# fzi-forschungszentrum-informatik/muvo

Measured on AMD Instinct MI355X. Metric: world-model training samples/sec (seq_len=10), higher is better.
Workload: dtype f32 storage/accumulate; large contractions (convolutions, transformer Linear) as bf16x3 split products

## Files before the change

### include/muvo_hip.h

```cpp
#ifndef MUVO_HIP_H
#define MUVO_HIP_H
#include <stdint.h>

#ifdef __cplusplus
extern "C" {
#endif

#define MUVO_OK 0
#define MUVO_ERR_INVALID_ARG (-1)
#define MUVO_ERR_HIP (-2)

#define MUVO_ACT_NONE 0
#define MUVO_ACT_RELU 1
#define MUVO_ACT_LEAKY 2
#define MUVO_ACT_ELU 3
#define MUVO_ACT_TANH 4
#define MUVO_ACT_SIGMOID 5

const char* muvo_last_error(void);
int muvo_abi_version(void);
int muvo_selftest_mfma(void* stream);
int muvo_set_deterministic(int on);
int muvo_reset_accumulators(void);
int muvo_get_deterministic(void);

typedef struct muvo_conv_desc {
  int32_t nd;
  int32_t transposed;
  int32_t N, Cin, Cout;
  int32_t in_sz[3], out_sz[3];
  int32_t ksz[3], stride[3], pad[3], dil[3];
} muvo_conv_desc;

#define MUVO_CONV_F32 0
#define MUVO_CONV_BF16X3 1
#define MUVO_CONV_MODE_DEFAULT MUVO_CONV_BF16X3
int muvo_conv_set_products(int n);
int muvo_conv_get_products(void);
int muvo_conv_set_mode(int mode);
int muvo_conv_get_mode(void);
int muvo_conv_set_bf16x3_min_gflop(double gflop_per_item);
int muvo_linear_bf16x3_pack_floats(int in_f, int out_f, int64_t* fwd_floats, int64_t* dgrad_floats);
int muvo_linear_bf16x3_pack(int in_f, int out_f, const float* w, float* wp_fwd, float* wp_dgrad, void* stream);
int64_t muvo_linear_bf16x3_workspace_bytes(int64_t rows, int features);
int muvo_linear_bf16x3_split(const float* x, int64_t rows, int features, void* ws, void* stream);
int muvo_linear_bf16x3_forward(int64_t rows, int in_f, int out_f, const void* ws_x, const float* wp_fwd, const float* bias,
                               float* y, int act, float slope, void* stream);
int muvo_linear_bf16x3_dgrad(int64_t rows, int in_f, int out_f, const void* ws_dz, const float* wp_dgrad, float* dx,
                             void* stream);
int muvo_linear_bf16x3_wgrad(int64_t rows, int in_f, int out_f, const void* ws_x, const void* ws_dz, float* scratch,
                             float* dw, void* stream);
int64_t muvo_pack_table_item_bytes(void);
int muvo_conv_pack_table_add(void* host_items, int capacity, int* n_items, int64_t* n_blocks, const muvo_conv_desc* d,
                             const float* w, float* wp_fwd, float* wp_dgrad);
int muvo_linear_bf16x3_pack_table_add(void* host_items, int capacity, int* n_items, int64_t* n_blocks, int in_f, int out_f,
                                      const float* w, float* wp_fwd, float* wp_dgrad);
int muvo_pack_table_run(const void* dev_items, int n_items, int64_t n_blocks, void* stream);
int muvo_conv_pack_sizes(const muvo_conv_desc* d, int64_t* fwd_floats, int64_t* dgrad_floats);
int muvo_conv_pack_weights(const muvo_conv_desc* d, const float* w, float* wp_fwd, float* wp_dgrad, void* stream);
int64_t muvo_conv_workspace_bytes(const muvo_conv_desc* d, int op);
int muvo_conv_kernel_family(const muvo_conv_desc* d, int op);
int muvo_conv_kernel_variant(const muvo_conv_desc* d, int op);
int muvo_conv_forward(const muvo_conv_desc* d, const float* x, const float* wp_fwd, const float* bias, float* y, int act,
                      float slope, void* ws, void* stream);
int muvo_conv_dgrad(const muvo_conv_desc* d, const float* dy, const float* wp_dgrad, float* dx, void* ws, int ws_valid,
                    void* stream);
int muvo_conv_forward_head_supported(const muvo_conv_desc* d, int CO);
int muvo_conv_forward_head(const muvo_conv_desc* d, const float* x, const float* wp_fwd, const float* bias, float* y, int act,
                           float slope, void* ws, const float* head_w, const float* head_b, int CO, float* logits, void* stream);
int muvo_conv_forward_moments_supported(const muvo_conv_desc* d);
int muvo_conv_forward_moments(const muvo_conv_desc* d, const float* x, const float* wp_fwd, const float* bias, float* y, int act,
                              float slope, double* moments, void* stream);
int muvo_adain_fwd_moments(const float* x, const float* style, float* y, float* save_mean, float* save_rstd, double* moments,
                           int N, int C, int64_t S, float eps, void* stream);
int muvo_adain_affine(const float* style, double* moments, float* save_mean, float* save_rstd, float* aff, int N, int C, int64_t S,
                      float eps, void* stream);
int muvo_conv_affine_supported(const muvo_conv_desc* d);
int muvo_conv_forward_affine(const muvo_conv_desc* d, const float* x, const float* aff, const float* wp_fwd, const float* bias,
                             float* y, int act, float slope, double* moments, void* stream);
int muvo_conv_wgrad_affine(const muvo_conv_desc* d, const float* x, const float* aff, const float* dy, float* dw, float* dbias,
                           void* stream);
int muvo_grouped_linear_fwd(const float* x, int M, int K, int L, const float* const* W, const float* const* b, float* const* Y,
                            const int* N, void* stream);
int muvo_grouped_linear_bwd(const float* x, int M, int K, int L, const float* const* W, float* const* dY, float* dx,
                            float* const* dW, float* const* db, const int* N, void* stream);
int muvo_bf3_loop_clock(double* shader_mhz, double* us_per_k_step);
int muvo_adain_head_supported(int C, int CO, int64_t S);
int muvo_adain_head_fwd(const float* x, const float* style, float* save_mean, float* save_rstd, double* moments, const float* head_w,
                        const float* head_b, float* logits, int N, int C, int CO, int64_t S, float eps, void* stream);
int muvo_adain_head_bwd(const float* x, const float* style, const float* save_mean, const float* save_rstd, const float* head_w,
                        const float* dlogits, float* dx, float* dstyle, float* dhead_w, float* dhead_b, double* ws, int N, int C,
                        int CO, int64_t S, int act, float slope, void* stream);
int muvo_conv_dgrad_accumulate(const muvo_conv_desc* d, const float* dy, const float* wp_dgrad, float* dx, void* stream);
int muvo_conv_prepare_dy(const muvo_conv_desc* d, const float* y, const float* dy, int act, float slope, void* ws_dy,
                         float* dbias, void* stream);
int muvo_conv_prepare_dy_head_supported(const muvo_conv_desc* d, int CO);
int muvo_conv_prepare_dy_head(const muvo_conv_desc* d, const float* y, const float* dy, const float* dhead, const float* head_w,
                              int CO, int act, float slope, void* ws_dy, float* dbias, float* dhead_w, float* dhead_b, void* stream);
int64_t muvo_split_planes_bytes(int N, int C, int64_t S);
int muvo_split_planes(const float* x, void* ws, int N, int C, int64_t S, const float* y, int act, float slope, float* dbias,
                      void* stream);
int muvo_conv_wgrad(const muvo_conv_desc* d, const float* x, const float* dy, float* dwp_scratch, float* dw, float* dbias,
                    void* ws_x, void* ws_dy, int flags, void* stream);

int muvo_bias_grad_nchw(const float* dy, float* db, int N, int M, int64_t S, void* stream);

typedef struct muvo_gemm_desc {
  int32_t M, N, K;
  int64_t sam, sak, sbk, sbn, scm;
  int32_t B1, B2;
  int64_t a_b1, a_b2, b_b1, b_b2, c_b1, c_b2;
  float alpha;
  int32_t bias_div;
  int32_t act;
  float slope;
  int32_t mode;
} muvo_gemm_desc;
int muvo_gemm(const muvo_gemm_desc* d, const float* A, const float* B, float* C, const float* bias, void* stream);

int muvo_bn_train_fwd(const float* x, const float* gamma, const float* beta, const float* residual, float* y,
                      float* save_mean, float* save_rstd, float* running_mean, float* running_var, double* ws, int N, int C,
                      int64_t S, float eps, float momentum, int res_mode, int relu, void* stream);
int muvo_bn_train_bwd(const float* x, const float* y, const float* dy, const float* gamma, const float* beta,
                      const float* save_mean, const float* save_rstd, float* dx, float* dres, float* dgamma, float* dbeta,
                      double* ws, int N, int C, int64_t S, int mask_mode, void* stream);
int muvo_adain_fwd(const float* x, const float* style, float* y, float* save_mean, float* save_rstd, double* ws, int N,
                   int C, int64_t S, int64_t x_batch_stride, float eps, void* stream);
int muvo_adain_bwd(const float* x, const float* style, const float* dy, const float* save_mean, const float* save_rstd,
                   float* dx, float* dstyle, double* ws, int N, int C, int64_t S, int64_t x_batch_stride, int act,
                   float slope, void* stream);
int muvo_add_dropout_layernorm_fwd(const float* x, const float* a, const float* gamma, const float* beta, float* y,
                                   float* z, float* mean, float* rstd, int rows, int E, float eps, float p, uint64_t seed,
                                   void* stream);
int muvo_add_dropout_layernorm_bwd(const float* dy, const float* z, const float* mean, const float* rstd,
                                   const float* gamma, float* dx, float* da, float* dgamma, float* dbeta, int rows, int E,
                                   float p, uint64_t seed, void* stream);

int muvo_act_fwd(const float* x, float* y, int64_t n, int act, float slope, void* stream);
int muvo_act_bwd(const float* y, const float* dy, float* dx, int64_t n, int act, float slope, void* stream);
int muvo_dropout(const float* x, float* y, int64_t n, float p, uint64_t seed, void* stream);
int muvo_axpby(const float* a, const float* b, float* out, int64_t n, float alpha, float beta, void* stream);
int muvo_copy2d(const float* src, float* dst, int64_t rows, int64_t cols, int64_t ld_src, int64_t ld_dst, int accumulate,
                void* stream);
int muvo_colsum_acc(const float* x, float* out, int64_t rows, int64_t cols, int64_t ld, void* stream);
int muvo_batchsum(const float* x, float* out, int N, int64_t inner, int accumulate, void* stream);
int muvo_nchw_to_tokens(const float* x, const float* pos, const float* temb, int temb_stride, float* tokens, int N, int C,
                        int L, int l0, void* stream);
int muvo_tokens_to_nchw(const float* tokens, float* x, int N, int C, int L, int l0, void* stream);
int muvo_maxpool2d_fwd(const float* x, float* y, uint8_t* idx, int64_t NC, int H, int W, int OH, int OW, int k, int s, int p,
                       void* stream);
int muvo_maxpool2d_bwd(const float* dy, const uint8_t* idx, float* dx, int64_t NC, int H, int W, int OH, int OW, int k, int s,
                       int p, void* stream);
int muvo_avgpool_fwd(const float* x, float* y, int64_t G, int64_t S, void* stream);
int muvo_avgpool_bwd(const float* dy, float* dx, int64_t G, int64_t S, void* stream);
int muvo_upsample3d_x2_fwd(const float* x, float* y, int64_t NC, int D, int H, int W, void* stream);
int muvo_upsample3d_x2_bwd(const float* dy, float* dx, int64_t NC, int D, int H, int W, void* stream);
int muvo_preprocess_image(const uint8_t* img, float* label, float* norm, int64_t NC, int C, int H, int W, int top, int left,
                          int CH, int CW, const float* mean3, const float* std3, void* stream);
int muvo_preprocess_route(const uint8_t* img, float* norm, int64_t NC, int C, int H, int W, int OH, int OW,
                          const float* mean3, const float* std3, void* stream);
int muvo_attention_supported(int L, int DH);
int muvo_attention_fwd(const float* qkv, float* out, float* lse, int L, int N, int H, int DH, float p, uint64_t seed,
                       void* stream);
int muvo_attention_bwd(const float* qkv, const float* out, const float* dout, const float* lse, float* dqkv, int L, int N, int H,
                       int DH, float p, uint64_t seed, void* stream);
int muvo_attention_stream_supported(int L, int DH);
int muvo_attention_stream_blocks(int* bq, int* bk);
int muvo_attention_stream_fwd(const float* qkv, float* out, float* lse, int L, int N, int H, int DH, float p, uint64_t seed,
                              void* stream);
int muvo_attention_stream_bwd(const float* qkv, const float* out, const float* dout, const float* lse, float* dqkv, float* dws,
                              int L, int N, int H, int DH, float p, uint64_t seed, void* stream);
int muvo_rssm_supported(int B, int T, int H, int S, int E, int A, int AD);
int64_t muvo_rssm_transposed_floats(int H, int S, int E, int A);
int64_t muvo_rssm_scratch_floats(int B, int H, int S, int E, int A);
int muvo_rssm_forward(int B, int T, int H, int S, int E, int A, int AD, const float* const* weights, const float* emb,
                      const float* act, const float* noise, uint64_t use_prior_mask, float* const* out7, float* const* keep12,
                      uint32_t* barrier_word, float min_std, void* stream);
int muvo_rssm_backward(int B, int T, int H, int S, int E, int A, int AD, const float* const* weights, float* wt_scratch,
                       const float* noise, uint64_t use_prior_mask, const float* const* kept5, const float* const* upstream7,
                       float* const* grads10, float* scratch, uint32_t* barrier_word, void* stream);
#define MUVO_PIXAUG_STRIDE 16
#define MUVO_ROUTEAUG_STRIDE 8
int muvo_pixel_augment(float* img, float* norm, float* tmp, const float* params, double* gray_sum, int64_t frames, int H, int W,
                       const float* mean3, const float* std3, void* stream);
int muvo_preprocess_route_aug(const uint8_t* img, float* out, const float* params, int B, int S, int C, int H, int W, int OH,
                              int OW, const float* mean3, const float* std3, void* stream);
int muvo_divide_scalar(const float* x, float* y, int64_t n, float divisor, void* stream);
int muvo_resize_bilinear(const float* x, float* y, int64_t NC, int H, int W, int OH, int OW, void* stream);
int muvo_resize_nearest_f32(const float* x, float* y, int64_t NC, int D, int H, int W, int OD, int OH, int OW, void* stream);
int muvo_resize_nearest_u8(const uint8_t* x, uint8_t* y, int64_t NC, int D, int H, int W, int OD, int OH, int OW,
                           void* stream);
int muvo_softmax_dropout_fwd(const float* S, float* P, float* Pd, int64_t rows, int cols, float p, uint64_t seed, void* stream);
int muvo_softmax_dropout_bwd(const float* P, const float* dPd, float* dS, int64_t rows, int cols, float p, uint64_t seed,
                             void* stream);
int muvo_gru_fwd(const float* gi, const float* gh, const float* h, float* hnew, int B, int H, void* stream);
int muvo_gru_bwd(const float* gi, const float* gh, const float* h, const float* dhnew, float* dgi, float* dgh, float* dh,
                 int B, int H, void* stream);
int muvo_rssm_sample_fwd(const float* mu_logsigma, const float* eps, int64_t eps_ld, float* mu, float* sigma, float* sample,
                         int B, int S, float min_std, void* stream);
int muvo_rssm_sample_bwd(const float* mu_logsigma, const float* eps, int64_t eps_ld, const float* dmu, const float* dsigma,
                         const float* dsample, float* dmls, int B, int S, void* stream);

int muvo_spatial_loss_fwd(const float* pred, const float* target, int64_t F, int Ct, int64_t HW, int c0, int c1, int norm,
                          float ignore, float weight, double* stats2, float* loss, void* stream);
int muvo_spatial_loss_bwd(const float* pred, const float* target, float* dpred, int64_t F, int Ct, int64_t HW, int c0, int c1,
                          int norm, float ignore, float weight, const double* stats2, const float* gout, void* stream);
int muvo_spatial_loss_masked_fwd(const float* pred, const float* target, const uint8_t* mask, int64_t F, int Ct, int64_t HW, int c0,
                                 int c1, int norm, float ignore, float weight, double* stats2, float* loss, void* stream);
int muvo_spatial_loss_masked_bwd(const float* pred, const float* target, const uint8_t* mask, float* dpred, int64_t F, int Ct,
                                 int64_t HW, int c0, int c1, int norm, float ignore, float weight, const double* stats2,
                                 const float* gout, void* stream);
int muvo_voxel_loss_stats_doubles(int C);
int muvo_voxel_loss_coef_floats(int C);
int muvo_voxel_loss_fwd(const float* logits, const uint8_t* target, int64_t F, int C, int64_t V, const float* class_w,
                        float weight, double* stats, float* coef, float* loss3, void* stream);
int muvo_voxel_loss_bwd(const float* logits, const uint8_t* target, float* dlogits, int64_t F, int C, int64_t V,
                        const float* class_w, float weight, const float* coef, const float* gout3, void* stream);
int muvo_seg_ce_fwd(const float* logits, const uint8_t* target, const float* class_w, float* loss, int64_t N, int C, int64_t HW,
                    void* stream);
int muvo_seg_ce_bwd(const float* logits, const uint8_t* target, const float* class_w, const float* gloss, float* dlogits, int64_t N,
                    int C, int64_t HW, void* stream);
int muvo_l1_rows_fwd(const float* p, const float* t, int64_t rows, int cols, float weight, float* loss, void* stream);
int muvo_l1_rows_bwd(const float* p, const float* t, float* dp, int64_t rows, int cols, float weight, const float* gout,
                     void* stream);
int muvo_kl_loss_fwd(const float* prior_mu, const float* prior_sigma, const float* post_mu, const float* post_sigma, int B,
                     int T, int S, float weight, float* loss, void* stream);
int muvo_kl_loss_bwd(const float* prior_mu, const float* prior_sigma, const float* post_mu, const float* post_sigma,
                     float* d_prior_mu, float* d_prior_sigma, float* d_post_mu, float* d_post_sigma, int B, int T, int S,
                     float weight, float alpha, const float* gout, void* stream);
int muvo_adamw_step(float* p, const float* g, float* m, float* v, int64_t n, float lr, float beta1, float beta2, float eps,
                    float weight_decay, int step, float grad_scale, void* stream);

int64_t muvo_chamfer_loss_ws_doubles(int64_t F, int64_t n);
int muvo_chamfer_loss_fwd(const float* pred, const float* target, int64_t F, int Cp, int Ct, int64_t n, float weight, double* ws,
                          int32_t* idx_pt, int32_t* idx_tp, float* loss, void* stream);
int muvo_chamfer_loss_bwd(const float* pred, const float* target, const int32_t* idx_pt, const int32_t* idx_tp, float* dpred, int64_t F,
                          int Cp, int Ct, int64_t n, float weight, const float* gout, void* stream);

int muvo_ssim_frames(const float* pred, const float* target, const float* window, double* sums, int N, int C, int H, int W,
                     float c1, float c2, void* stream);
int muvo_ssim_maps(const float* pred, const float* target, const float* window, double* sums, float* dA, float* dB, float* dC, int N,
                   int C, int H, int W, float c1, float c2, void* stream);
int muvo_ssim_bwd(const float* pred, const float* target, const float* window, const float* dA, const float* dB, const float* dC,
                  float* dpred, int N, int C, int H, int W, float scale, void* stream);
int muvo_sqdiff_frames(const float* pred, const float* target, double* sums, int N, int64_t L, void* stream);
int muvo_chamfer_sums(const float* a, const float* b, double* sums, int N, int P, int Q, void* stream);
// ... 120 lines not shown
```

### muvo_amd/csrc/conv_gemm.hip

```cpp
#include "common.h"
#include "conv_vox.h"
#include "conv_pw.h"
#include "conv_plan.h"
#include "conv_bf3.h"

typedef __bf16 wg_bf16x8 __attribute__((ext_vector_type(8)));
__device__ __forceinline__ void wg_split8(const float (&v)[8], wg_bf16x8& hi, wg_bf16x8& lo) {
  typedef __bf16 b2 __attribute__((ext_vector_type(2)));
  typedef float f2 __attribute__((ext_vector_type(2)));
  unsigned h[4], l[4];
#pragma unroll
  for (int p = 0; p < 4; ++p) {
    const b2 hh = __builtin_convertvector((f2){v[2 * p], v[2 * p + 1]}, b2);
    h[p] = __builtin_bit_cast(unsigned, hh);
    const float h0 = __uint_as_float(h[p] << 16), h1 = __uint_as_float(h[p] & 0xffff0000u);
    const b2 ll = __builtin_convertvector((f2){v[2 * p] - h0, v[2 * p + 1] - h1}, b2);
    l[p] = __builtin_bit_cast(unsigned, ll);
  }
  typedef unsigned u4 __attribute__((ext_vector_type(4)));
  hi = __builtin_bit_cast(wg_bf16x8, (u4){h[0], h[1], h[2], h[3]});
  lo = __builtin_bit_cast(wg_bf16x8, (u4){l[0], l[1], l[2], l[3]});
}

template <int BM, int BN, int WM, int WN, int RUN>
// ... 835 lines not shown
    }
    return pl.nfwd > 0 && bf3_wgrad_uses_pp(pl.fwd[0]) ? 1 : 0;
  }
  if (build_plan(d, &pl)) return 0;
  const ConvPhase* ph = op == 0 ? pl.fwd : pl.dgr;
  const int nph = op == 0 ? pl.nfwd : pl.ndgr;
  return nph > 0 && bf3_fwd_uses_pp(ph[0]) ? 1 : 0;
}

static int run_phases(const ConvPhase* ph, int nph, const float* in, const float* wp, const float* bias, float* out, int act,
                      float slope, void* ws, hipStream_t st, bool ws_valid = false) {
  bool split_done = ws_valid;
  static const int any_rule = getenv("MUVO_KSPLIT_ANY") ? atoi(getenv("MUVO_KSPLIT_ANY")) : 1;
  bool use_ksplit = nph > 0 && !any_rule, any_ks = false;
  for (int i = 0; i < nph; ++i) {
    use_ksplit = use_ksplit && phase_ksplit(ph[i]) > 1;
    any_ks = any_ks || phase_ksplit(ph[i]) > 1;
  }
  if (any_rule) use_ksplit = any_ks;
  const long out_total = nph > 0 ? (long)ph[0].N * ph[0].out_sN : 0;
  if (use_ksplit && hipMemsetAsync(out, 0, sizeof(float) * out_total, st) != hipSuccess) {
    muvo_set_error("conv: memset of the split-K output failed");
    return MUVO_ERR_HIP;
  }
  for (int i = 0; i < nph; ++i) {
    if (ph[i].bf3 && !split_done) {
      MUVO_CHECK_ARG(ws != nullptr, "conv: this shape runs on the bf16x3 kernel and needs muvo_conv_workspace_bytes() of workspace");
      int rc = bf3_split_input(in, ws, ph[i].N, ph[i].C, (long)ph[i].ID * ph[i].IH * ph[i].IW, st);
      if (rc) return rc;
      split_done = true;
    }
    const int ks_i = phase_ksplit(ph[i]);
    int rc = launch_fwd_phase(ph[i], in, wp, bias, out, act, slope, st, ws, use_ksplit ? (ks_i > 1 ? ks_i : 2) : 1);
    if (rc) return rc;
  }
  if (use_ksplit && (bias != nullptr || act != MUVO_ACT_NONE)) {
    hipLaunchKernelGGL(bias_act_kernel, dim3(ew_grid(out_total)), dim3(256), 0, st, out, bias, ph[0].Msub, (long)ph[0].out_sC,
                       out_total, act, slope);
    MUVO_CHECK_LAUNCH("bias_act_kernel");
  }
  return MUVO_OK;
}

int muvo_conv_forward(const muvo_conv_desc* d, const float* x, const float* wp_fwd, const float* bias, float* y,
                      int act, float slope, void* ws, void* stream) {
  ConvPlan pl;
  int rc = build_plan(d, &pl);
  if (rc) return rc;
  MUVO_CHECK_ARG(x && wp_fwd && y, "conv_forward: null pointer");
  if (pw_applicable(d)) return pw_forward(d, x, wp_fwd, bias, y, act, slope, (hipStream_t)stream);
  if (vox_fwd_ok(d)) return vox_forward(d, x, wp_fwd, bias, y, act, slope, (hipStream_t)stream, vox_uses_bf3(d, 0));
  return run_phases(pl.fwd, pl.nfwd, x, wp_fwd, bias, y, act, slope, ws, (hipStream_t)stream);
}

int muvo_conv_forward_planes(const muvo_conv_desc* d, const float* x, const float* wp_fwd, const float* bias, float* y, int act,
                             float slope, void* ws, int ws_valid, void* stream) {
  if (!ws_valid) return muvo_conv_forward(d, x, wp_fwd, bias, y, act, slope, ws, stream);
  ConvPlan pl;
  int rc = build_plan(d, &pl);
  if (rc) return rc;
  MUVO_CHECK_ARG(wp_fwd && y && ws, "conv_forward_planes: null pointer");
  MUVO_CHECK_ARG(!pw_applicable(d) && !vox_fwd_ok(d), "conv_forward_planes: this shape does not read split planes");
  bool all_bf3 = pl.nfwd > 0;
  for (int i = 0; i < pl.nfwd; ++i) all_bf3 = all_bf3 && pl.fwd[i].bf3;
  MUVO_CHECK_ARG(all_bf3, "conv_forward_planes: ws_valid needs every phase on the bf16x3 kernels (muvo_conv_kernel_family == 1)");
  return run_phases(pl.fwd, pl.nfwd, x, wp_fwd, bias, y, act, slope, ws, (hipStream_t)stream, true);
}

int muvo_conv_forward_head_supported(const muvo_conv_desc* d, int CO) {
  if (check_desc(d) || CO < 1 || CO > 4) return 0;
  static const int on = getenv("MUVO_CONV_HEAD_FWD") ? atoi(getenv("MUVO_CONV_HEAD_FWD")) : 1;
  if (!on || muvo_det() || conv_mode() != 1 || pw_applicable(d) || vox_fwd_ok(d)) return 0;
  ConvPlan pl;
  if (build_plan(d, &pl) != MUVO_OK || pl.nfwd < 1) return 0;
  for (int i = 0; i < pl.nfwd; ++i) {
    const ConvPhase& g = pl.fwd[i];
    if (!g.bf3 || !bf3_fwd_uses_pp(g) || phase_ksplit(g) > 1) return 0;
    if (g.Msub != d->Cout || g.Msub % 64 != 0 || g.M % 64 != 0 || (long)CO * g.Msub > 1024) return 0;
    if ((long)g.N * g.out_sN * 4 >= 0x7fffff00L) return 0;
  }
  return 1;
}
int muvo_conv_forward_head(const muvo_conv_desc* d, const float* x, const float* wp_fwd, const float* bias, float* y, int act,
                           float slope, void* ws, const float* head_w, const float* head_b, int CO, float* logits, void* stream) {
  ConvPlan pl;
  int rc = build_plan(d, &pl);
  if (rc) return rc;
  MUVO_CHECK_ARG(x && wp_fwd && y && head_w && logits, "conv_forward_head: null pointer");
  MUVO_CHECK_ARG(muvo_conv_forward_head_supported(d, CO), "conv_forward_head: shape not served by the eight-wave bf16x3 tiles");
  hipStream_t st = (hipStream_t)stream;
  if (d->Cout > 64) {
    const long S_out = (long)d->out_sz[0] * d->out_sz[1] * d->out_sz[2];
    if (hipMemsetAsync(logits, 0, sizeof(float) * (size_t)d->N * CO * S_out, st) != hipSuccess) {
      muvo_set_error("conv_forward_head: memset of the logits failed");
      return MUVO_ERR_HIP;
    }
  }
  bf3_set_fused_head(head_w, head_b, logits, CO);
  rc = run_phases(pl.fwd, pl.nfwd, x, wp_fwd, bias, y, act, slope, ws, st);
  bf3_set_fused_head(nullptr, nullptr, nullptr, 0);
  return rc;
}

int muvo_conv_forward_moments_supported(const muvo_conv_desc* d) {
  if (check_desc(d)) return 0;
  if (muvo_det()) return 0;
  return (!pw_applicable(d) && vox_fwd_ok(d) && vox_uses_bf3(d, 0)) ? 1 : 0;
}
int muvo_conv_forward_moments(const muvo_conv_desc* d, const float* x, const float* wp_fwd, const float* bias, float* y, int act,
                              float slope, double* moments, void* stream) {
  ConvPlan pl;
  int rc = build_plan(d, &pl);
  if (rc) return rc;
  MUVO_CHECK_ARG(x && wp_fwd && y && moments, "conv_forward_moments: null pointer");
  MUVO_CHECK_ARG(muvo_conv_forward_moments_supported(d), "conv_forward_moments: only the bf16x3 voxel kernels produce output moments");
  return vox_forward(d, x, wp_fwd, bias, y, act, slope, (hipStream_t)stream, true, moments);
}

int muvo_conv_affine_supported(const muvo_conv_desc* d) {
  if (check_desc(d)) return 0;
  return (conv_mode() == 1 && !pw_applicable(d) && vox_fwd_ok(d) && vox_uses_bf3(d, 0) && vox_wgrad_applicable(d) &&
          vox_wgrad_uses_bf3(d) && vox_affine_ok(d)) ? 1 : 0;
}
int muvo_conv_forward_affine(const muvo_conv_desc* d, const float* x, const float* aff, const float* wp_fwd, const float* bias,
                             float* y, int act, float slope, double* moments, void* stream) {
  ConvPlan pl;
  int rc = build_plan(d, &pl);
  if (rc) return rc;
  MUVO_CHECK_ARG(x && aff && wp_fwd && y, "conv_forward_affine: null pointer");
  MUVO_CHECK_ARG(muvo_conv_affine_supported(d), "conv_forward_affine: shape not served by the bf16x3 voxel kernels");
  return vox_forward(d, x, wp_fwd, bias, y, act, slope, (hipStream_t)stream, true, moments, aff);
}
int muvo_conv_wgrad_affine(const muvo_conv_desc* d, const float* x, const float* aff, const float* dy, float* dw, float* dbias,
                           void* stream) {
  ConvPlan pl;
  int rc = build_plan(d, &pl, 0, false);
  if (rc) return rc;
  MUVO_CHECK_ARG(x && aff && dy && dw, "conv_wgrad_affine: null pointer");
  MUVO_CHECK_ARG(muvo_conv_affine_supported(d), "conv_wgrad_affine: shape not served by the bf16x3 voxel kernels");
  return vox_wgrad(d, x, dy, dw, dbias, (hipStream_t)stream, true, aff);
}

int muvo_conv_dgrad(const muvo_conv_desc* d, const float* dy, const float* wp_dgrad, float* dx, void* ws, int ws_valid,
                    void* stream) {
  ConvPlan pl;
  int rc = build_plan(d, &pl);
  if (rc) return rc;
  MUVO_CHECK_ARG(dy && wp_dgrad && dx, "conv_dgrad: null pointer");
  if (pw_applicable(d)) return pw_dgrad(d, dy, wp_dgrad, dx, (hipStream_t)stream);
  if (vox_dgrad_ok(d)) return vox_dgrad(d, dy, wp_dgrad, dx, (hipStream_t)stream, vox_uses_bf3(d, 1));
  return run_phases(pl.dgr, pl.ndgr, dy, wp_dgrad, nullptr, dx, MUVO_ACT_NONE, 0.f, ws, (hipStream_t)stream, ws_valid != 0);
}

int muvo_conv_dgrad_accumulate(const muvo_conv_desc* d, const float* dy, const float* wp_dgrad, float* dx, void* stream) {
  int rc = check_desc(d);
  if (rc) return rc;
  MUVO_CHECK_ARG(dy && wp_dgrad && dx, "conv_dgrad_accumulate: null pointer");
  MUVO_CHECK_ARG(pw_applicable(d), "conv_dgrad_accumulate: only the 1x1 head kernels (muvo_conv_kernel_family == 3) accumulate");
  return pw_dgrad_acc(d, dy, wp_dgrad, dx, (hipStream_t)stream);
}

int muvo_conv_prepare_dy(const muvo_conv_desc* d, const float* y, const float* dy, int act, float slope, void* ws_dy,
                         float* dbias, void* stream) {
  int rc = check_desc(d);
  if (rc) return rc;
  MUVO_CHECK_ARG(dy && ws_dy && (y || act == MUVO_ACT_NONE), "conv_prepare_dy: null pointer");
  const long S_out = (long)d->out_sz[0] * d->out_sz[1] * d->out_sz[2];
  return bf3_split_input(dy, ws_dy, d->N, d->Cout, S_out, (hipStream_t)stream, act == MUVO_ACT_NONE ? nullptr : y, act, slope,
                         dbias);
}

int muvo_conv_prepare_dy_head(const muvo_conv_desc* d, const float* y, const float* dy, const float* dhead, const float* head_w,
                              int CO, int act, float slope, void* ws_dy, float* dbias, float* dhead_w, float* dhead_b, void* stream) {
  int rc = check_desc(d);
  if (rc) return rc;
  MUVO_CHECK_ARG(dhead && head_w && ws_dy && CO >= 1 && CO <= 4 && (y || act == MUVO_ACT_NONE), "conv_prepare_dy_head: bad args");
  const long S_out = (long)d->out_sz[0] * d->out_sz[1] * d->out_sz[2];
  MUVO_CHECK_ARG(dhead_w == nullptr || (y != nullptr && act != MUVO_ACT_NONE),
                 "conv_prepare_dy_head: the fused head weight gradient needs the activation output y");
  return bf3_split_input(dy, ws_dy, d->N, d->Cout, S_out, (hipStream_t)stream, act == MUVO_ACT_NONE ? nullptr : y, act, slope,
                         dbias, dhead, head_w, CO, dhead_w, dhead_b);
}
int muvo_conv_prepare_dy_head_supported(const muvo_conv_desc* d, int CO) {
  if (check_desc(d)) return 0;
  const long S_out = (long)d->out_sz[0] * d->out_sz[1] * d->out_sz[2];
  return CO >= 1 && CO <= 4 && S_out % 4 == 0 && S_out >= 1024;
}

static double bf3_wgrad_min_gflop() {
  static const char* e = getenv("MUVO_BF16X3_WGRAD_MIN_GFLOP");
  static const double env_v = e ? atof(e) : -1.0;
  if (env_v >= 0.0) return env_v;
  if (bf3_default_policy()) return 0.05;
  return bf3_min_gflop() < 0.5 ? bf3_min_gflop() : 0.5;
}

static const int g_bf3_wgrad_min_m = getenv("MUVO_BF3_WGRAD_MIN_M") ? atoi(getenv("MUVO_BF3_WGRAD_MIN_M")) : 32;
static bool wgrad_uses_bf3(const ConvPlan& pf) {
  if (conv_mode() != 1) return false;
  const bool dflt = bf3_default_policy() && !getenv("MUVO_BF16X3_WGRAD_MIN_GFLOP");
  double total = 0.0;
  int taps = 0;
  for (int i = 0; i < pf.nfwd; ++i) {
    const ConvPhase& g = pf.fwd[i];
    const double gflop = 2.0 * g.Msub * g.T * g.C * (double)g.SD * g.SH * g.SW * 1e-9;
    if (g.Msub < g_bf3_wgrad_min_m || g.C < 32 || g.Msub % 16 != 0 && g.nmerge > 1) return false;
    static const int allow32 = getenv("MUVO_BF3_WGRAD_32X32") ? atoi(getenv("MUVO_BF3_WGRAD_32X32")) : 1;
    if (g.Msub <= 32 && g.C < 64 && !allow32) return false;
    if (!dflt && gflop < bf3_wgrad_min_gflop()) return false;
    total += gflop * g.nmerge;
    taps += g.T * g.nmerge;
  }
  if (dflt && (total < bf3_wgrad_min_gflop() || taps <= 1)) return false;
  return pf.nfwd > 0;
}

int muvo_conv_wgrad(const muvo_conv_desc* d, const float* x, const float* dy, float* dwp_scratch, float* dw, float* dbias,
                    void* ws_x, void* ws_dy, int flags, void* stream) {
  ConvPlan pl;
  int rc = build_plan(d, &pl, 0, false);
  if (rc) return rc;
  MUVO_CHECK_ARG(x && dy && dwp_scratch && dw, "conv_wgrad: null pointer");
  hipStream_t st = (hipStream_t)stream;
  if (pw_applicable(d)) return pw_wgrad(d, x, dy, dw, dbias, st);
  if (vox_wgrad_ok(d)) return vox_wgrad(d, x, dy, dw, dbias, st, vox_wgrad_uses_bf3(d));
  const long S_out = (long)d->out_sz[0] * d->out_sz[1] * d->out_sz[2];
  if (wgrad_uses_bf3(pl)) {
    ConvPlan pm;
    if (build_plan(d, &pm, 0, true) == MUVO_OK && wgrad_uses_bf3(pm)) pl = pm;
    MUVO_CHECK_ARG(ws_x && ws_dy, "conv_wgrad: this shape runs on the bf16x3 kernel and needs both workspaces");
    const long S_in = (long)d->in_sz[0] * d->in_sz[1] * d->in_sz[2];
    if (!(flags & 1)) { rc = bf3_split_input(x, ws_x, d->N, d->Cin, S_in, st); if (rc) return rc; }
    if (!(flags & 2)) { rc = bf3_split_input(dy, ws_dy, d->N, d->Cout, S_out, st); if (rc) return rc; }
    long off = 0;
    for (int i = 0; i < pl.nfwd; ++i) off += (long)pl.fwd[i].T * pl.fwd[i].M * pl.fwd[i].C;
    off = 0;
    for (int i = 0; i < pl.nfwd; ++i) {
      ConvPhase g = pl.fwd[i];
      g.wp_off = off;
      off += (long)g.T * g.M * g.C;
      rc = bf3_wgrad_phase(g, ws_x, d->Cin, ws_dy, d->Cout, dwp_scratch, dw, st);
      if (rc) return rc;
    }
  } else {
    for (int i = 0; i < pl.nfwd; ++i) {
      rc = launch_wgrad_phase(pl.fwd[i], x, dy, dwp_scratch, st);
      if (rc) return rc;
    }
    for (int i = 0; i < pl.nfwd; ++i) {
      const long total = (long)pl.fwd[i].M * pl.fwd[i].C * pl.fwd[i].T;
      if (total == 0) continue;
      hipLaunchKernelGGL(unpack_wgrad_kernel, dim3(ew_grid(total)), dim3(256), 0, st, pl.fwd[i], dwp_scratch, dw);
    }
    MUVO_CHECK_LAUNCH("unpack_wgrad_kernel");
  }
  if (dbias) {
    int chunks = cdiv((long)d->N * S_out, 65536);
    if (chunks > 64) chunks = 64;
    if (muvo_det()) chunks = 1;
    hipLaunchKernelGGL(bias_grad_kernel, dim3(d->Cout, chunks), dim3(256), 0, st, dy, dbias, d->N, d->Cout, S_out);
    MUVO_CHECK_LAUNCH("bias_grad_kernel");
  }
  return MUVO_OK;
}

int64_t muvo_split_planes_bytes(int N, int C, int64_t S) { return bf3_workspace_bytes(N, C, (long)S); }
int muvo_split_planes(const float* x, void* ws, int N, int C, int64_t S, const float* y, int act, float slope, float* dbias,
                      void* stream) {
  MUVO_CHECK_ARG(x && ws && N > 0 && C > 0 && S > 0, "split_planes: bad args");
  return bf3_split_input(x, ws, N, C, (long)S, (hipStream_t)stream, act == MUVO_ACT_NONE ? nullptr : y, act, slope, dbias);
}
int muvo_bias_grad_nchw(const float* dy, float* db, int N, int M, int64_t S, void* stream) {
  MUVO_CHECK_ARG(dy && db && N > 0 && M > 0 && S > 0, "bias_grad_nchw: bad args");
  int chunks = cdiv((long)N * S, 65536);
  if (chunks > 64) chunks = 64;
  if (muvo_det()) chunks = 1;
  hipLaunchKernelGGL(bias_grad_kernel, dim3(M, chunks), dim3(256), 0, (hipStream_t)stream, dy, db, N, M, (long)S);
  MUVO_CHECK_LAUNCH("bias_grad_kernel");
  return MUVO_OK;
}

static int linear_phase(int rows, int c, int m, long wsm, long wsc, bool token_major_out, ConvPhase* ph) {
  MUVO_CHECK_ARG(rows > 0 && c >= 32 && m > 32 && c % 8 == 0 && m % 4 == 0,
                 "linear_bf16x3: needs in/out features >= 32, reduction features %% 8 == 0, produced features %% 4 == 0");
  muvo_conv_desc d;
  memset(&d, 0, sizeof(d));
  d.nd = 2; d.N = 1; d.Cin = c; d.Cout = m;
  for (int a = 0; a < 3; ++a) { d.in_sz[a] = d.out_sz[a] = d.ksz[a] = d.stride[a] = d.dil[a] = 1; d.pad[a] = 0; }
  d.in_sz[2] = d.out_sz[2] = rows;
  t_plan_mode = 1;
  t_allow_merge = false;
  t_force_family = 1;
  const int rc = build_conv_form(&d, d.in_sz, d.out_sz, c, m, wsm, wsc, ph);
  t_force_family = 0;
  if (rc) return rc;
  ph->wp_off = 0;
  if (token_major_out) { ph->os[2] = m; ph->out_sC = 1; }
  return MUVO_OK;
}

int muvo_linear_bf16x3_pack_floats(int in_f, int out_f, int64_t* fwd_floats, int64_t* dgrad_floats) {
  ConvPhase f, b;
  int rc = linear_phase(1, in_f, out_f, in_f, 1, true, &f);
  if (rc) return rc;
  rc = linear_phase(1, out_f, in_f, 1, in_f, true, &b);
  if (rc) return rc;
// ... 121 lines not shown
```

### muvo_amd/csrc/conv_vox.h

```cpp
#pragma once
#include "common.h"

bool vox_fwd_applicable(const muvo_conv_desc* d);
bool vox_dgrad_applicable(const muvo_conv_desc* d);
bool vox_wgrad_applicable(const muvo_conv_desc* d);
long vox_pack_floats(const muvo_conv_desc* d);
bool vox_bf3_shape_ok(const muvo_conv_desc* d, int dgrad);
int vox_pack(const muvo_conv_desc* d, const float* w, float* wp, int dgrad, hipStream_t st, bool bf3);
int vox_forward(const muvo_conv_desc* d, const float* x, const float* wp, const float* bias, float* y, int act, float slope,
                hipStream_t st, bool bf3, double* moments = nullptr, const float* aff = nullptr);
bool vox_affine_ok(const muvo_conv_desc* d);
int vox_dgrad(const muvo_conv_desc* d, const float* dy, const float* wp, float* dx, hipStream_t st, bool bf3);
bool vox_bf3_wgrad_shape_ok(const muvo_conv_desc* d);
bool vox_wgrad_ps_only(const muvo_conv_desc* d);
int vox_wgrad(const muvo_conv_desc* d, const float* x, const float* dz, float* dw, float* dbias, hipStream_t st, bool bf3,
              const float* aff = nullptr);
```

### muvo_amd/csrc/conv_vox.hip

```cpp
#include "common.h"
#include "conv_vox.h"
#include <type_traits>

struct VoxArgs {
  int N, Cin, Cout, X, Y;
  int ytiles, xgroups;
  int XYZ;
  long sN_in, sN_out;
  double* moments;
  int xcd_order;
  const float* aff;
  unsigned* ticket;
};
static int vox_xcd_order() {
  static const int v = getenv("MUVO_VOX_XCD") ? atoi(getenv("MUVO_VOX_XCD")) : 1;
  return v;
}

__device__ __forceinline__ float dpp_wave_shr1(float v) {
  return __int_as_float(__builtin_amdgcn_update_dpp(0, __float_as_int(v), 0x138, 0xf, 0xf, true));
}
__device__ __forceinline__ float dpp_wave_shl1(float v) {
  return __int_as_float(__builtin_amdgcn_update_dpp(0, __float_as_int(v), 0x130, 0xf, 0xf, true));
}
// ... 170 lines not shown
    }
  };
  auto fetch_dz = [&](int xx) {
#pragma unroll
    for (int k = 0; k < NDZ; ++k) {
      const int item = tid + k * NT;
      const int i = item & 3, zz = (item >> 2) % Z, r = (item >> 2) / Z;
      const int y = y0 + r;
      const bool ok = xx < xb && r < TYB && y < a.Y;
      const int off = xx * YZ + y * Z + zz;
#pragma unroll
      for (int e = 0; e < CQB; ++e) pdz[k][e] = ok ? dzn[(size_t)(4 * e + i) * a.XYZ + off] : 0.f;
    }
  };
  auto store_dz = [&](int buf) {
    float* S = D + buf * DBUF;
#pragma unroll
    for (int k = 0; k < NDZ; ++k) {
      const int item = tid + k * NT;
      const int i = item & 3, zz = (item >> 2) % Z, r = (item >> 2) / Z;
      if (r < TYB) {
#pragma unroll
        for (int e = 0; e < CQB; ++e) S[e * DPL + (r * Z + zz) * 4 + i] = pdz[k][e];
      }
    }
  };
  auto slot_of = [](int xx) { return (xx + 3) % 3; };

  f32x4 acc[CQR][9];
#pragma unroll
  for (int q = 0; q < CQR; ++q)
#pragma unroll
    for (int t = 0; t < 9; ++t) acc[q][t] = (f32x4){0.f, 0.f, 0.f, 0.f};
  float db[CQR];
#pragma unroll
  for (int q = 0; q < CQR; ++q) db[q] = 0.f;

  fetch_in(xa - 1); store_in(slot_of(xa - 1));
  fetch_in(xa);     store_in(slot_of(xa));
  fetch_in(xa + 1); store_in(slot_of(xa + 1));
  fetch_dz(xa);     store_dz(xa & 1);
  __syncthreads();

  const int b = lane >> 2, lj = lane & 3;
  const bool bias_role = tx == 1 && rr == 0;
  for (int x = xa; x < xb; ++x) {
    const bool more = x + 1 < xb;
    if (more) { fetch_in(x + 2); fetch_dz(x + 1); }
    const float* S = P + slot_of(x + tx - 1) * SLOT + rr * PLANE;
    const float* Dz = D + (x & 1) * DBUF + (qg * CQR) * DPL;
#pragma unroll 1
    for (int row = 0; row < TYB; ++row) {
#pragma unroll
      for (int zs = 0; zs < ZS; ++zs) {
        const int zz = zs * 16 + b;
        float av[CQR];
#pragma unroll
        for (int q = 0; q < CQR; ++q) av[q] = Dz[q * DPL + (row * Z + zz) * 4 + lj];
        float bv[9];
#pragma unroll
        for (int ty = 0; ty < 3; ++ty)
#pragma unroll
          for (int tz = 0; tz < 3; ++tz) bv[ty * 3 + tz] = S[((row + ty) * ZP + zz + tz) * 4 + lj];
#pragma unroll
        for (int t = 0; t < 9; ++t)
#pragma unroll
          for (int q = 0; q < CQR; ++q) acc[q][t] = __builtin_amdgcn_mfma_f32_4x4x1f32(av[q], bv[t], acc[q][t], 0, 0, 0);
        if (bias_role) {
#pragma unroll
          for (int q = 0; q < CQR; ++q) db[q] += av[q];
        }
      }
    }
    __syncthreads();
    if (more) { store_in(slot_of(x + 2)); store_dz((x + 1) & 1); }
    __syncthreads();
  }

  det_turn_wait(a.ticket);
#pragma unroll
  for (int q = 0; q < CQR; ++q)
#pragma unroll
    for (int t = 0; t < 9; ++t)
#pragma unroll
      for (int i = 0; i < 4; ++i) {
        float v = acc[q][t][i];
        v += __shfl_xor(v, 4, 64);
        v += __shfl_xor(v, 8, 64);
        v += __shfl_xor(v, 16, 64);
        v += __shfl_xor(v, 32, 64);
        if (lane < 4) {
          const int co = (qc * CQB + qg * CQR + q) * 4 + i, ci = (rc * RQB + rr) * 4 + lane;
          atomicAdd(dw + ((size_t)co * a.Cin + ci) * 27 + tx * 9 + t, v);
        }
      }
  if (bias_role && rc == 0 && dbias != nullptr) {
#pragma unroll
    for (int q = 0; q < CQR; ++q) {
      float v = db[q];
      v += __shfl_xor(v, 4, 64);
      v += __shfl_xor(v, 8, 64);
      v += __shfl_xor(v, 16, 64);
      v += __shfl_xor(v, 32, 64);
      if (lane < 4) atomicAdd(dbias + (qc * CQB + qg * CQR + q) * 4 + lane, v);
    }
  }
  det_turn_done(a.ticket);
}

__global__ void __launch_bounds__(256) vox_pack_kernel(const float* __restrict__ w, float* __restrict__ wp, int Cin, int Cout,
                                                       int dgrad) {
  const int total = 27 * Cin * Cout;
  for (int idx = blockIdx.x * 256 + threadIdx.x; idx < total; idx += gridDim.x * 256) {
    const int ci_k = dgrad ? Cout : Cin;
    const int co_k = dgrad ? Cin : Cout;
    const int cq = co_k / 4;
    const int q = idx % cq;
    int r = idx / cq;
    const int i = r & 3; r >>= 2;
    const int ck = r % ci_k, tap = r / ci_k;
    const int cp = 4 * q + i;
    float v;
    if (!dgrad) v = w[((size_t)cp * Cin + ck) * 27 + tap];
    else v = w[((size_t)ck * Cin + cp) * 27 + (26 - tap)];
    wp[idx] = v;
  }
}

typedef __bf16 vbf16x8 __attribute__((ext_vector_type(8)));
typedef float vf32x4 __attribute__((ext_vector_type(4)));
typedef unsigned vu32x4 __attribute__((ext_vector_type(4)));

__device__ __forceinline__ float vox_act_simple(float v, int act, float slope) {
  const float neg = act == MUVO_ACT_RELU ? 0.f : v * slope;
  return (act == MUVO_ACT_NONE || v > 0.f) ? v : neg;
}

template <int N>
__device__ __forceinline__ void vox_dummy_stores(__amdgpu_buffer_rsrc_t rs) {
#pragma unroll
  for (int k = 0; k < N; ++k) __builtin_amdgcn_raw_buffer_store_b32(0u, rs, 0x7fffff00u + 32u * k, 0, 0);
}

__device__ __forceinline__ void vox_split2(float a, float b, unsigned& hi, unsigned& lo) {
  typedef __bf16 vbf16x2 __attribute__((ext_vector_type(2)));
  typedef float vf32x2 __attribute__((ext_vector_type(2)));
  const vbf16x2 h = __builtin_convertvector((vf32x2){a, b}, vbf16x2);
  hi = __builtin_bit_cast(unsigned, h);
  const float h0 = __uint_as_float(hi << 16), h1 = __uint_as_float(hi & 0xffff0000u);
  const vbf16x2 l = __builtin_convertvector((vf32x2){a - h0, b - h1}, vbf16x2);
  lo = __builtin_bit_cast(unsigned, l);
}

template <int CK, int Z, int TY, bool GENERIC>
__global__ void __launch_bounds__(64 * TY)
vox_bf3_kernel(const VoxArgs a, const float* __restrict__ in, const vu32x4* __restrict__ wp, const float* __restrict__ bias,
               float* __restrict__ out, int act, float slope, int xseg, int accum) {
  static_assert(CK == 8 && TY == 8, "8 reduction channels (one channel group), 8 rows per workgroup");
  constexpr int CG = 1, TPS = 4, NSTEP = (27 + TPS - 1) / TPS, ZT = Z / 16;
  constexpr int ROWS = TY + 2, COLS = Z + 2;
  constexpr int PLANE = 2 * CG * ROWS * COLS;
  constexpr int NTASK = CG * ROWS * Z, TPT = (NTASK + 64 * TY - 1) / (64 * TY);
  extern __shared__ vu32x4 vsm[];
  const int tid = threadIdx.x, lane = tid & 63, wave = tid >> 6;
  const int nseg = (a.X + xseg - 1) / xseg;
  int bid = a.xcd_order ? xcd_swizzle(blockIdx.x, gridDim.x) : (int)blockIdx.x;
  const int seg = bid % nseg; bid /= nseg;
  const int ytile = bid % a.ytiles, n = bid / a.ytiles;
  const int y0 = ytile * TY, xs = seg * xseg, xe = xs + xseg < a.X ? xs + xseg : a.X;
  const long YZ = (long)a.Y * Z;
  const float* inb = in + (long)n * a.sN_in;
  const int co0 = blockIdx.y * 16;

  vbf16x8 wh[NSTEP], wl[NSTEP];
  const vu32x4* wpb = wp + (size_t)blockIdx.y * NSTEP * 2 * 64;
#pragma unroll
  for (int s = 0; s < NSTEP; ++s) {
    wh[s] = __builtin_bit_cast(vbf16x8, wpb[(s * 2) * 64 + lane]);
    wl[s] = __builtin_bit_cast(vbf16x8, wpb[(s * 2 + 1) * 64 + lane]);
  }
  for (int i = tid; i < 3 * PLANE; i += 64 * TY) vsm[i] = vu32x4{0u, 0u, 0u, 0u};
  __syncthreads();

  float stg[TPT][8];
  unsigned stg_ok = 0u;
  float afs[8], afb[8];
  if (a.aff) {
#pragma unroll
    for (int e = 0; e < 8; ++e) {
      afs[e] = a.aff[((long)n * a.Cin + e) * 2];
      afb[e] = a.aff[((long)n * a.Cin + e) * 2 + 1];
    }
  }
  const __amdgpu_buffer_rsrc_t rs_in = __builtin_amdgcn_make_buffer_rsrc((void*)inb, 0, (int)((long)CK * a.XYZ * 4), 0x00020000);
  const unsigned xyz4 = (unsigned)a.XYZ * 4u;
  auto stage_load = [&](int x) {
#pragma unroll
    for (int k = 0; k < TPT; ++k) {
      const int t = tid + k * 64 * TY;
      const int z = t % Z, r = (t / Z) % ROWS, cg = t / (Z * ROWS);
      const int gy = y0 - 1 + r;
      const bool ok = t < NTASK && x >= 0 && x < a.X && gy >= 0 && gy < a.Y;
      stg_ok = k == 0 ? (unsigned)ok : stg_ok | ((unsigned)ok << k);
      const unsigned off = ok ? (unsigned)(((long)(cg * 8) * a.XYZ + (long)x * YZ + (long)gy * Z + z) * 4) : 0x7fffff00u;
#pragma unroll
      for (int e = 0; e < 8; ++e)
        stg[k][e] = __uint_as_float(__builtin_amdgcn_raw_buffer_load_b32(rs_in, off + (unsigned)e * xyz4, 0, 0));
    }
  };
  auto stage_store = [&](int slot) {
    vu32x4* P = vsm + slot * PLANE;
#pragma unroll
    for (int k = 0; k < TPT; ++k) {
      const int t = tid + k * 64 * TY;
      if (t >= NTASK) continue;
      const int z = t % Z, r = (t / Z) % ROWS, cg = t / (Z * ROWS);
      if (a.aff) {
        const bool ok = (stg_ok >> k) & 1u;
#pragma unroll
        for (int e = 0; e < 8; ++e) stg[k][e] = ok ? stg[k][e] * afs[e] + afb[e] : 0.f;
      }
      unsigned h[4], l[4];
#pragma unroll
      for (int q = 0; q < 4; ++q) vox_split2(stg[k][2 * q], stg[k][2 * q + 1], h[q], l[q]);
      P[(cg * ROWS + r) * COLS + z + 1] = vu32x4{h[0], h[1], h[2], h[3]};
      P[((CG + cg) * ROWS + r) * COLS + z + 1] = vu32x4{l[0], l[1], l[2], l[3]};
    }
  };

  const int v = lane & 15, g = lane >> 4;
  float msum[4] = {0.f, 0.f, 0.f, 0.f}, msq[4] = {0.f, 0.f, 0.f, 0.f};
  float bv[4];
#pragma unroll
  for (int i = 0; i < 4; ++i) bv[i] = (bias != nullptr && co0 + 4 * g + i < a.Cout) ? bias[co0 + 4 * g + i] : 0.f;
  const __amdgpu_buffer_rsrc_t rs_out = __builtin_amdgcn_make_buffer_rsrc((void*)(out + (long)n * a.sN_out), 0,
                                                                          (int)((long)a.Cout * a.XYZ * 4), 0x00020000);

  int fdx[NSTEP], foff[NSTEP];
#pragma unroll
  for (int s = 0; s < NSTEP; ++s) {
    int tap = s * TPS + g;
    if (tap > 26) tap = 26;
    const int dx = tap / 9 - 1, dy = (tap / 3) % 3 - 1, dz = tap % 3 - 1;
    fdx[s] = dx;
    foff[s] = (wave + 1 + dy) * COLS + (v + 1 + dz);
  }

  stage_load(xs - 1); stage_store((xs - 1 + 3) % 3);
  stage_load(xs); stage_store(xs % 3);
  stage_load(xs + 1);
  vox_dummy_stores<4 * ZT>(rs_out);
  __syncthreads();
  for (int x = xs; x < xe; ++x) {
    stage_store((x + 1) % 3);
    __syncthreads();
    if (x + 1 < xe) stage_load(x + 2);
    const vu32x4* P[3] = {vsm + ((x - 1 + 3) % 3) * PLANE, vsm + (x % 3) * PLANE, vsm + ((x + 1) % 3) * PLANE};
    const vu32x4* fb[NSTEP];
#pragma unroll
    for (int s = 0; s < NSTEP; ++s) fb[s] = (fdx[s] < 0 ? P[0] : (fdx[s] == 0 ? P[1] : P[2])) + foff[s];
    const int gy = y0 + wave;
#pragma unroll
    for (int zt = 0; zt < ZT; ++zt) {
      vf32x4 acc = {0.f, 0.f, 0.f, 0.f};
#pragma unroll
      for (int s = 0; s < NSTEP; ++s) {
        const vbf16x8 bh = __builtin_bit_cast(vbf16x8, fb[s][zt * 16]);
        const vbf16x8 bl = __builtin_bit_cast(vbf16x8, fb[s][zt * 16 + CG * ROWS * COLS]);
        acc = __builtin_amdgcn_mfma_f32_16x16x32_bf16(wl[s], bh, acc, 0, 0, 0);
        acc = __builtin_amdgcn_mfma_f32_16x16x32_bf16(wh[s], bl, acc, 0, 0, 0);
        acc = __builtin_amdgcn_mfma_f32_16x16x32_bf16(wh[s], bh, acc, 0, 0, 0);
      }
      const unsigned ooff = (unsigned)(((long)x * YZ + (long)gy * Z + zt * 16 + v) * 4);
#pragma unroll
      for (int i = 0; i < 4; ++i) {
        const int co = co0 + 4 * g + i;
        const bool ok = gy < a.Y && co < a.Cout;
        const unsigned off = ok ? ooff + (unsigned)co * xyz4 : 0x7fffff00u;
        float r = acc[i] + bv[i];
        if constexpr (GENERIC) {
          if (accum) r += __uint_as_float(__builtin_amdgcn_raw_buffer_load_b32(rs_out, off, 0, 0));
          r = act_apply(r, act, slope);
        } else {
          r = vox_act_simple(r, act, slope);
        }
        __builtin_amdgcn_raw_buffer_store_b32(__float_as_uint(r), rs_out, off, 0, 0);
        r = ok ? r : 0.f;
        msum[i] += r;
        msq[i] += r * r;
      }
    }
    __syncthreads();
  }
  if (a.moments) {
#pragma unroll
    for (int i = 0; i < 4; ++i)
#pragma unroll
      for (int o = 1; o < 16; o <<= 1) { msum[i] += __shfl_xor(msum[i], o, 64); msq[i] += __shfl_xor(msq[i], o, 64); }
    float* red = (float*)vsm;
    if (v == 0)
#pragma unroll
      for (int i = 0; i < 4; ++i) { red[((wave * 4 + g) * 4 + i) * 2] = msum[i]; red[((wave * 4 + g) * 4 + i) * 2 + 1] = msq[i]; }
    __syncthreads();
    if (tid < 32) {
      const int c = tid >> 1, k = tid & 1;
      double t = 0.0;
      for (int w = 0; w < TY; ++w) t += (double)red[((w * 4 + (c >> 2)) * 4 + (c & 3)) * 2 + k];
      if (co0 + c < a.Cout) atomicAdd(&a.moments[((long)n * a.Cout + co0 + c) * 2 + k], t);
    }
  }
}

constexpr int VOX_PS_TY = 8;
template <int Z, int TY, bool CO8, bool GENERIC>
__global__ void __launch_bounds__(64 * TY, 1)
vox_bf3_ps_kernel(const VoxArgs a, const float* __restrict__ in, const vu32x4* __restrict__ wp, const float* __restrict__ bias,
                  float* __restrict__ out, int act, float slope, int xseg, int accum) {
  static_assert(TY == VOX_PS_TY, "one workgroup of eight waves per CU");
  constexpr int CK = 16, CG = 2, PSTEPS = 5, ZT = Z / 16, NF = CO8 ? 2 * PSTEPS : 3 * PSTEPS, NACC = CO8 ? 2 : 3;
  constexpr int ROWS = TY + 2, COLS = Z + 2;
  constexpr int PLANE = 2 * CG * ROWS * COLS;
  constexpr int NTASK = CG * ROWS * Z, TPT = (NTASK + 64 * TY - 1) / (64 * TY);
  extern __shared__ vu32x4 vsm[];
  const int tid = threadIdx.x, lane = tid & 63, wave = tid >> 6;
  const int nseg = (a.X + xseg - 1) / xseg;
  int bid = a.xcd_order ? xcd_swizzle(blockIdx.x, gridDim.x) : (int)blockIdx.x;
  const int seg = bid % nseg; bid /= nseg;
  const int ytile = bid % a.ytiles, n = bid / a.ytiles;
  const int y0 = ytile * TY, xs = seg * xseg, xe = xs + xseg < a.X ? xs + xseg : a.X;
  const long YZ = (long)a.Y * Z;
  const float* inb = in + (long)n * a.sN_in;
  const int co0 = blockIdx.y * 16;

  vbf16x8 wh[NF], wl[NF];
  const vu32x4* wpb = wp + (size_t)blockIdx.y * NF * 2 * 64;
#pragma unroll
  for (int f = 0; f < NF; ++f) {
    wh[f] = __builtin_bit_cast(vbf16x8, wpb[(f * 2) * 64 + lane]);
    wl[f] = __builtin_bit_cast(vbf16x8, wpb[(f * 2 + 1) * 64 + lane]);
  }
  for (int i = tid; i < 2 * PLANE; i += 64 * TY) vsm[i] = vu32x4{0u, 0u, 0u, 0u};
  __syncthreads();

  float stg[TPT][8];
  unsigned stg_ok = 0u;
  __shared__ float s_aff[2 * CK];
  if (a.aff) {
    if (tid < 2 * CK) s_aff[tid] = a.aff[(long)n * a.Cin * 2 + tid];
    __syncthreads();
  }
  const __amdgpu_buffer_rsrc_t rs_in = __builtin_amdgcn_make_buffer_rsrc((void*)inb, 0, (int)((long)CK * a.XYZ * 4), 0x00020000);
  const unsigned xyz4 = (unsigned)a.XYZ * 4u;
  auto stage_load_task = [&](int k, int x) {
    const int t = tid + k * 64 * TY;
    const int z = t % Z, r = (t / Z) % ROWS, cg = t / (Z * ROWS);
    const int gy = y0 - 1 + r;
    const bool ok = t < NTASK && x >= 0 && x < a.X && gy >= 0 && gy < a.Y;
    stg_ok = (stg_ok & ~(1u << k)) | ((unsigned)ok << k);
    const unsigned off = ok ? (unsigned)(((long)(cg * 8) * a.XYZ + (long)x * YZ + (long)gy * Z + z) * 4) : 0x7fffff00u;
#pragma unroll
    for (int e = 0; e < 8; ++e)
      stg[k][e] = __uint_as_float(__builtin_amdgcn_raw_buffer_load_b32(rs_in, off + (unsigned)e * xyz4, 0, 0));
  };
  auto stage_load = [&](int x) {
#pragma unroll
    for (int k = 0; k < TPT; ++k) stage_load_task(k, x);
  };
  auto stage_store_task = [&](int k, int slot) {
    vu32x4* P = vsm + slot * PLANE;
    {
      const int t = tid + k * 64 * TY;
      if (t >= NTASK) return;
      const int z = t % Z, r = (t / Z) % ROWS, cg = t / (Z * ROWS);
      if (a.aff) {
        const bool ok = (stg_ok >> k) & 1u;
#pragma unroll
        for (int e = 0; e < 8; ++e) {
          const float sc = s_aff[(cg * 8 + e) * 2], sh = s_aff[(cg * 8 + e) * 2 + 1];
          stg[k][e] = ok ? stg[k][e] * sc + sh : 0.f;
        }
      }
      unsigned h[4], l[4];
#pragma unroll
      for (int q = 0; q < 4; ++q) vox_split2(stg[k][2 * q], stg[k][2 * q + 1], h[q], l[q]);
      P[(cg * ROWS + r) * COLS + z + 1] = vu32x4{h[0], h[1], h[2], h[3]};
      P[((CG + cg) * ROWS + r) * COLS + z + 1] = vu32x4{l[0], l[1], l[2], l[3]};
    }
  };
  auto stage_store = [&](int slot) {
#pragma unroll
    for (int k = 0; k < TPT; ++k) stage_store_task(k, slot);
  };

  const int v = lane & 15, g = lane >> 4;
  float msum[4] = {0.f, 0.f, 0.f, 0.f}, msq[4] = {0.f, 0.f, 0.f, 0.f};
  float bv[4];
#pragma unroll
  for (int i = 0; i < 4; ++i) bv[i] = (bias != nullptr && co0 + 4 * g + i < a.Cout) ? bias[co0 + 4 * g + i] : 0.f;
  const __amdgpu_buffer_rsrc_t rs_out = __builtin_amdgcn_make_buffer_rsrc((void*)(out + (long)n * a.sN_out), 0,
                                                                          (int)((long)a.Cout * a.XYZ * 4), 0x00020000);
  int foff[PSTEPS];
#pragma unroll
  for (int s = 0; s < PSTEPS; ++s) {
    int tp = s * 2 + (g >> 1);
    if (tp > 8) tp = 8;
    const int dy = tp / 3 - 1, dz = tp % 3 - 1;
    foff[s] = ((g & 1) * ROWS + (wave + 1 + dy)) * COLS + (v + 1 + dz);
  }
  vf32x4 acc[NACC][ZT];
#pragma unroll
  for (int j = 0; j < NACC; ++j)
#pragma unroll
    for (int zt = 0; zt < ZT; ++zt) acc[j][zt] = vf32x4{0.f, 0.f, 0.f, 0.f};

  stage_load(xs - 1); stage_store((xs - 1) & 1);
  stage_load(xs);
  vox_dummy_stores<4 * ZT>(rs_out);
  __syncthreads();
  const int gy = y0 + wave;
  for (int p = xs - 1; p <= xe; ++p) {
    constexpr bool ACC_PRE = GENERIC && (CO8 || Z <= 32);
    float accv[ZT][4];
    if constexpr (ACC_PRE) {
      if (accum) {
        const int xo = p - 1;
        const bool xok = xo >= xs && xo < xe;
#pragma unroll
        for (int zt = 0; zt < ZT; ++zt) {
          const unsigned ooff = (unsigned)(((long)xo * YZ + (long)gy * Z + zt * 16 + v) * 4);
#pragma unroll
          for (int i = 0; i < 4; ++i) {
            const int co = co0 + 4 * g + i;
            const bool ok = xok && gy < a.Y && co < a.Cout && (!CO8 || g < 2);
            accv[zt][i] = __uint_as_float(__builtin_amdgcn_raw_buffer_load_b32(rs_out, ok ? ooff + (unsigned)co * xyz4 : 0x7fffff00u, 0, 0));
          }
        }
      }
    }
    constexpr bool PIPE = CO8 || Z <= 32;
    if constexpr (!PIPE) {
      stage_store((p + 1) & 1);
      if (p + 2 <= xe) stage_load(p + 2);
    }
    const vu32x4* P = vsm + (p & 1) * PLANE;
#pragma unroll
    for (int zt = 0; zt < ZT; ++zt) {
#pragma unroll
      for (int s = 0; s < PSTEPS; ++s) {
        const vbf16x8 bh = __builtin_bit_cast(vbf16x8, P[foff[s] + zt * 16]);
        const vbf16x8 bl = __builtin_bit_cast(vbf16x8, P[foff[s] + zt * 16 + CG * ROWS * COLS]);
        if constexpr (CO8) {
          acc[1][zt] = __builtin_amdgcn_mfma_f32_16x16x32_bf16(wl[s], bh, acc[1][zt], 0, 0, 0);
          acc[1][zt] = __builtin_amdgcn_mfma_f32_16x16x32_bf16(wh[s], bl, acc[1][zt], 0, 0, 0);
          acc[1][zt] = __builtin_amdgcn_mfma_f32_16x16x32_bf16(wh[s], bh, acc[1][zt], 0, 0, 0);
          acc[0][zt] = __builtin_amdgcn_mfma_f32_16x16x32_bf16(wl[PSTEPS + s], bh, acc[0][zt], 0, 0, 0);
          acc[0][zt] = __builtin_amdgcn_mfma_f32_16x16x32_bf16(wh[PSTEPS + s], bl, acc[0][zt], 0, 0, 0);
          acc[0][zt] = __builtin_amdgcn_mfma_f32_16x16x32_bf16(wh[PSTEPS + s], bh, acc[0][zt], 0, 0, 0);
        } else {
#pragma unroll
          for (int dxi = 0; dxi < 3; ++dxi) {
            const int f = dxi * PSTEPS + s, j = 2 - dxi;
            acc[j][zt] = __builtin_amdgcn_mfma_f32_16x16x32_bf16(wl[f], bh, acc[j][zt], 0, 0, 0);
            acc[j][zt] = __builtin_amdgcn_mfma_f32_16x16x32_bf16(wh[f], bl, acc[j][zt], 0, 0, 0);
            acc[j][zt] = __builtin_amdgcn_mfma_f32_16x16x32_bf16(wh[f], bh, acc[j][zt], 0, 0, 0);
          }
        }
      }
      if constexpr (PIPE) {
#pragma unroll
        for (int k = 0; k < TPT; ++k)
          if ((k < ZT ? k : ZT - 1) == zt) {
            stage_store_task(k, (p + 1) & 1);
            if (p + 2 <= xe) stage_load_task(k, p + 2);
          }
        __builtin_amdgcn_sched_barrier(0);
      }
    }
    const int xo = p - 1;
    const bool xok = xo >= xs && xo < xe;
#pragma unroll
    for (int zt = 0; zt < ZT; ++zt) {
      const unsigned ooff = (unsigned)(((long)xo * YZ + (long)gy * Z + zt * 16 + v) * 4);
#pragma unroll
      for (int i = 0; i < 4; ++i) {
        const int co = co0 + 4 * g + i;
        const bool ok = xok && gy < a.Y && co < a.Cout && (!CO8 || g < 2);
        const unsigned off = ok ? ooff + (unsigned)co * xyz4 : 0x7fffff00u;
        float r = acc[0][zt][i] + bv[i];
        if constexpr (GENERIC) {
          if constexpr (ACC_PRE) { if (accum) r += accv[zt][i]; }
          else if (accum) r += __uint_as_float(__builtin_amdgcn_raw_buffer_load_b32(rs_out, off, 0, 0));
          r = act_apply(r, act, slope);
        } else {
          r = vox_act_simple(r, act, slope);
        }
        __builtin_amdgcn_raw_buffer_store_b32(__float_as_uint(r), rs_out, off, 0, 0);
        r = ok ? r : 0.f;
        msum[i] += r;
        msq[i] += r * r;
      }
    }
#pragma unroll
    for (int zt = 0; zt < ZT; ++zt) {
      if constexpr (CO8) {
        acc[0][zt] = acc[1][zt];
#pragma unroll
        for (int i = 0; i < 4; ++i) {
          const float up = __shfl(acc[1][zt][i], (lane + 32) & 63, 64);
          acc[1][zt][i] = lane < 32 ? up : 0.f;
        }
      } else {
        acc[0][zt] = acc[1][zt];
        acc[1][zt] = acc[2][zt];
        acc[2][zt] = vf32x4{0.f, 0.f, 0.f, 0.f};
      }
    }
    __syncthreads();
  }
  if (a.moments) {
#pragma unroll
    for (int i = 0; i < 4; ++i)
#pragma unroll
      for (int o = 1; o < 16; o <<= 1) { msum[i] += __shfl_xor(msum[i], o, 64); msq[i] += __shfl_xor(msq[i], o, 64); }
    float* red = (float*)vsm;
    if (v == 0)
#pragma unroll
      for (int i = 0; i < 4; ++i) { red[((wave * 4 + g) * 4 + i) * 2] = msum[i]; red[((wave * 4 + g) * 4 + i) * 2 + 1] = msq[i]; }
    __syncthreads();
    if (tid < 32) {
      const int c = tid >> 1, k = tid & 1;
      double t = 0.0;
      for (int w = 0; w < TY; ++w) t += (double)red[((w * 4 + (c >> 2)) * 4 + (c & 3)) * 2 + k];
      if (co0 + c < a.Cout) atomicAdd(&a.moments[((long)n * a.Cout + co0 + c) * 2 + k], t);
    }
  }
}

template <int Z, int CI, bool CO8>
__global__ void __launch_bounds__(512)
vox_bf3_wgrad_kernel(const VoxArgs a, const float* __restrict__ x, const float* __restrict__ dz, float* __restrict__ dw,
                     float* __restrict__ dbias, int xseg) {
  static_assert(CI == 8 && !CO8, "8 input channels, 16 produced channels");
  constexpr int ZH = Z / 32, WROWS = 8 / ZH, ROWS = WROWS + 2;
  constexpr int XROW = (Z + 16) * 2;
  constexpr int XCI = ROWS * XROW + 16;
  constexpr int XHL = CI * XCI, XSLOT = 2 * XHL;
  constexpr int DCH = 16;
  constexpr int DROW = Z * 2, DCO = WROWS * DROW + 16, DHL = DCH * DCO, DBUF = 2 * DHL;
  constexpr int XT = CI * ROWS * (Z / 8), DT = DCH * WROWS * (Z / 8);
  constexpr int NCOMB = 5, TPC = 3;
  constexpr int NT = NCOMB * TPC;
  constexpr int XPT = (XT + 511) / 512, DPT = (DT + 511) / 512;
  extern __shared__ char wsm[];
  char* xring = wsm;
  char* dzb = wsm + 4 * XSLOT;
  float* dbsum = (float*)(dzb + 2 * DBUF);
  const int tid = threadIdx.x, lane = tid & 63, wave = tid >> 6;
  const int nseg = (a.X + xseg - 1) / xseg;
  int bid = a.xcd_order ? xcd_swizzle(blockIdx.x, gridDim.x) : (int)blockIdx.x;
  const int seg = bid % nseg; bid /= nseg;
  const int ytile = bid % a.ytiles, n = bid / a.ytiles;
  const int y0 = ytile * WROWS, xs = seg * xseg, xe = xs + xseg < a.X ? xs + xseg : a.X;
  const int ci0 = blockIdx.y * CI;
  const long YZ = (long)a.Y * Z;
  const float* xb = x + (long)n * a.sN_in + (long)ci0 * a.XYZ;
  const float* db = dz + (long)n * a.sN_out;
  for (int i = tid; i < (4 * XSLOT + 2 * DBUF + 64) / 16; i += 512) ((uint4*)wsm)[i] = uint4{0u, 0u, 0u, 0u};
  __syncthreads();

  float xst[XPT][8], dst[DPT][8];
  unsigned xok = 0u;
  float xas[XPT], xab[XPT];
#pragma unroll
  for (int k = 0; k < XPT; ++k) {
    const int t = tid + k * 512;
    const int ci = t < XT ? t / ((Z / 8) * ROWS) : 0;
    const bool have = a.aff != nullptr && ci0 + ci < a.Cin;
    xas[k] = have ? a.aff[((long)n * a.Cin + ci0 + ci) * 2] : 1.f;
    xab[k] = have ? a.aff[((long)n * a.Cin + ci0 + ci) * 2 + 1] : 0.f;
  }
  auto split_store = [&](const float (&v)[8], char* hi_addr, int hl_stride) {
    unsigned h[4], l[4];
#pragma unroll
    for (int q = 0; q < 4; ++q) vox_split2(v[2 * q], v[2 * q + 1], h[q], l[q]);
    *(vu32x4*)hi_addr = vu32x4{h[0], h[1], h[2], h[3]};
    *(vu32x4*)(hi_addr + hl_stride) = vu32x4{l[0], l[1], l[2], l[3]};
  };
  constexpr unsigned OOB = 0x7fffff00u;
  auto load8b = [&](const __amdgpu_buffer_rsrc_t& rs, unsigned off, float (&v)[8]) {
    const vu32x4 u0 = __builtin_amdgcn_raw_buffer_load_b128(rs, off, 0, 0);
    const vu32x4 u1 = __builtin_amdgcn_raw_buffer_load_b128(rs, off + 16u, 0, 0);
    v[0] = __uint_as_float(u0.x); v[1] = __uint_as_float(u0.y); v[2] = __uint_as_float(u0.z); v[3] = __uint_as_float(u0.w);
    v[4] = __uint_as_float(u1.x); v[5] = __uint_as_float(u1.y); v[6] = __uint_as_float(u1.z); v[7] = __uint_as_float(u1.w);
  };
  const int nci = a.Cin - ci0 < CI ? a.Cin - ci0 : CI;
  const __amdgpu_buffer_rsrc_t rs_x = __builtin_amdgcn_make_buffer_rsrc((void*)xb, 0, (int)((long)nci * a.XYZ * 4), 0x00020000);
  const __amdgpu_buffer_rsrc_t rs_d = __builtin_amdgcn_make_buffer_rsrc((void*)db, 0, (int)((long)a.Cout * a.XYZ * 4), 0x00020000);
  auto xload = [&](int px) {
#pragma unroll
    for (int k = 0; k < XPT; ++k) {
      const int t = tid + k * 512;
      const int z8 = t % (Z / 8), rr = (t / (Z / 8)) % ROWS, ci = t / ((Z / 8) * ROWS);
      const int gy = y0 - 1 + rr;
      const bool ok = t < XT && px >= 0 && px < a.X && gy >= 0 && gy < a.Y;
      xok = k == 0 ? (unsigned)ok : xok | ((unsigned)ok << k);
      const long eoff = (long)ci * a.XYZ + (long)px * YZ + (long)gy * Z + z8 * 8;
      load8b(rs_x, ok ? (unsigned)(eoff * 4) : OOB, xst[k]);
    }
  };
  auto xstore_task = [&](int k, int slot) {
    const int t = tid + k * 512;
    if (t >= XT) return;
    const int z8 = t % (Z / 8), rr = (t / (Z / 8)) % ROWS, ci = t / ((Z / 8) * ROWS);
    if (a.aff) {
      const bool ok = (xok >> k) & 1u;
#pragma unroll
      for (int e = 0; e < 8; ++e) xst[k][e] = ok ? xst[k][e] * xas[k] + xab[k] : 0.f;
    }
    split_store(xst[k], xring + slot * XSLOT + ci * XCI + rr * XROW + 16 + z8 * 16, XHL);
  };
  auto xstore = [&](int slot) {
#pragma unroll
    for (int k = 0; k < XPT; ++k) xstore_task(k, slot);
  };
  auto dload = [&](int px) {
#pragma unroll
    for (int k = 0; k < DPT; ++k) {
      const int t = tid + k * 512;
      const int z8 = t % (Z / 8), r = (t / (Z / 8)) % WROWS, co = t / ((Z / 8) * WROWS);
      const int gy = y0 + r;
      const bool ok = t < DT && px < xe && gy < a.Y && co < a.Cout;
      const long eoff = (long)co * a.XYZ + (long)px * YZ + (long)gy * Z + z8 * 8;
      load8b(rs_d, ok ? (unsigned)(eoff * 4) : OOB, dst[k]);
    }
  };
  auto dstore_task = [&](int k, int buf) {
    const int t = tid + k * 512;
    if (t >= DT) return;
    const int z8 = t % (Z / 8), r = (t / (Z / 8)) % WROWS, co = t / ((Z / 8) * WROWS);
    split_store(dst[k], dzb + buf * DBUF + co * DCO + r * DROW + z8 * 16, DHL);
    if (blockIdx.y == 0 && dbias) {
      float sdz = 0.f;
#pragma unroll
      for (int e = 0; e < 8; ++e) sdz += dst[k][e];
      if (sdz != 0.f) atomicAdd(dbsum + co, sdz);
    }
  };
  auto dstore = [&](int buf) {
#pragma unroll
    for (int k = 0; k < DPT; ++k) dstore_task(k, buf);
  };

  vf32x4 acc[NT];
#pragma unroll
  for (int t = 0; t < NT; ++t) acc[t] = vf32x4{0.f, 0.f, 0.f, 0.f};
  const int row = wave / ZH, z0 = (wave % ZH) * 32;
  const int j = lane & 15, kg = lane >> 4;
  const int a_off = j * DCO + row * DROW + (z0 + kg * 8) * 2;
  const int b_off = (j & (CI - 1)) * XCI + 16 + (z0 + kg * 8) * 2;
  const int sel = j >> 3;

  xload(xs - 1); xstore((xs - 1 + 4) & 3);
  xload(xs); xstore(xs & 3);
  xload(xs + 1); xstore((xs + 1) & 3);
  dload(xs); dstore(xs & 1);
  xload(xs + 2);
  dload(xs + 1);
  __syncthreads();
  for (int px = xs; px < xe; ++px) {
    const char* A = dzb + (px & 1) * DBUF + a_off;
// ... 618 lines not shown
  a.sN_in = (long)(cin_total ? cin_total : Cin) * a.XYZ; a.sN_out = (long)Cout * a.XYZ;
  return a;
}

static int vox_blocks_target(int wgrad) {
  static const int f = getenv("MUVO_VOX_BLOCKS") ? atoi(getenv("MUVO_VOX_BLOCKS")) : 128;
  static const int w = getenv("MUVO_VOX_WGRAD_BLOCKS") ? atoi(getenv("MUVO_VOX_WGRAD_BLOCKS")) : 128;
  return wgrad ? w : f;
}
static int vox_xseg(const VoxArgs& a, int factor, int wgrad) {
  int xseg = a.X;
  while ((long)a.N * a.ytiles * cdiv(a.X, xseg) * factor < vox_blocks_target(wgrad) && xseg > 12) xseg = cdiv(xseg, 2);
  return xseg;
}

template <class... K>
static int vox_raise_lds(bool& done, const char* what, size_t lds, K... kernels) {
  if (done) return MUVO_OK;
  if (((hipFuncSetAttribute((const void*)kernels, hipFuncAttributeMaxDynamicSharedMemorySize, (int)lds) != hipSuccess) || ...)) {
    muvo_set_error("%s: cannot raise the dynamic LDS limit to %zu bytes", what, lds);
    return MUVO_ERR_HIP;
  }
  done = true;
  return MUVO_OK;
}

template <bool Z16 = false, class F>
static int vox_with_z(int Z, F&& f) {
  if (Z == 64) return f(std::integral_constant<int, 64>{});
  if (Z == 32) return f(std::integral_constant<int, 32>{});
  if constexpr (Z16) {
    if (Z == 16) return f(std::integral_constant<int, 16>{});
  }
  muvo_set_error("vox_conv: no kernel for z lines of %d voxels", Z);
  return MUVO_ERR_INVALID_ARG;
}
template <class F>
static int vox_with_bool(bool b, F&& f) { return b ? f(std::true_type{}) : f(std::false_type{}); }

template <int CQ, int TY, int Z>
static int launch_vox_conv(const muvo_conv_desc* d, int Cin, int Cout, const float* in, const float* wp, const float* bias,
                           float* out, int act, float slope, hipStream_t st) {
  VoxArgs a = vox_args(d, Cin, Cout, TY, Z, 0, nullptr);
  a.xgroups = cdiv(a.X, 64 / Z);
  const long nwaves = (long)a.N * a.xgroups * a.ytiles;
  const size_t lds = (size_t)27 * Cin * Cout * sizeof(float);
  hipLaunchKernelGGL((vox_conv_kernel<CQ, TY, Z>), dim3(cdiv(nwaves, 4)), dim3(256), lds, st, a, in, wp, bias, out, act, slope);
  MUVO_CHECK_LAUNCH("vox_conv_kernel");
  return MUVO_OK;
}

template <int Z>
static int launch_vox_bf3(const muvo_conv_desc* d, int Cout, const float* in, const float* wp, const float* bias, float* out, int act,
                          float slope, hipStream_t st, double* moments, const float* aff) {
  constexpr int CK = 8, TY = 8;
  VoxArgs a = vox_args(d, CK, Cout, TY, Z, 0, aff);
  a.moments = moments;
  const int xseg = vox_xseg(a, 1, 0);
  constexpr size_t lds = (size_t)3 * 2 * (TY + 2) * (Z + 2) * 16;
  static bool lds_raised = false;
  if (int rc = vox_raise_lds(lds_raised, "vox_bf3", lds, vox_bf3_kernel<CK, Z, TY, false>, vox_bf3_kernel<CK, Z, TY, true>)) return rc;
  const dim3 grid((unsigned)((long)a.N * a.ytiles * cdiv(a.X, xseg)), cdiv(Cout, 16));
  return vox_with_bool(act > MUVO_ACT_LEAKY, [&](auto generic) -> int {
    hipLaunchKernelGGL((vox_bf3_kernel<CK, Z, TY, decltype(generic)::value>), grid, dim3(64 * TY), lds, st, a, in, (const vu32x4*)wp, bias, out,
                       act, slope, xseg,  0);
    MUVO_CHECK_LAUNCH("vox_bf3_kernel");
    return MUVO_OK;
  });
}

template <int Z>
static int launch_vox_bf3_2row(const muvo_conv_desc* d, const float* in, const float* wp, const float* bias, float* out, int act,
                               float slope, hipStream_t st, double* moments, const float* aff) {
  constexpr int CK = 8, TY = 16;
  VoxArgs a = vox_args(d, CK, 8, TY, Z, 0, aff);
  a.moments = moments;
  const int xseg = vox_xseg(a, 1, 0);
  constexpr size_t lds = (size_t)3 * 2 * (TY + 2) * (Z + 2) * 16;
  static_assert(lds <= 160 * 1024, "LDS budget");
  static bool lds_raised = false;
  if (int rc = vox_raise_lds(lds_raised, "vox_bf3_2row", lds, vox_bf3_2row_kernel<Z, CK, false>, vox_bf3_2row_kernel<Z, CK, true>)) return rc;
  const dim3 grid((unsigned)((long)a.N * a.ytiles * cdiv(a.X, xseg)));
  return vox_with_bool(act > MUVO_ACT_LEAKY, [&](auto generic) -> int {
    hipLaunchKernelGGL((vox_bf3_2row_kernel<Z, CK, decltype(generic)::value>), grid, dim3(32 * TY), lds, st, a, in, (const vu32x4*)wp, bias, out,
                       act, slope, xseg);
    MUVO_CHECK_LAUNCH("vox_bf3_2row_kernel");
    return MUVO_OK;
  });
}

template <int Z, bool CO8>
static int launch_vox_bf3_ps(const muvo_conv_desc* d, int Cout, const float* in, const float* wp, const float* bias, float* out, int act,
                             float slope, hipStream_t st, int cin_total, int accum, double* moments, const float* aff) {
  constexpr int TY = VOX_PS_TY;
  VoxArgs a = vox_args(d, 16, Cout, TY, Z, cin_total, aff);
  a.moments = moments;
  const int xseg = vox_xseg(a, 1, 0);
  constexpr size_t lds = (size_t)2 * 2 * 2 * (TY + 2) * (Z + 2) * 16;
  static bool lds_raised = false;
  if (int rc = vox_raise_lds(lds_raised, "vox_bf3_ps", lds, vox_bf3_ps_kernel<Z, TY, CO8, false>, vox_bf3_ps_kernel<Z, TY, CO8, true>)) return rc;
  const dim3 grid((unsigned)((long)a.N * a.ytiles * cdiv(a.X, xseg)), cdiv(Cout, 16));
  return vox_with_bool(accum || act > MUVO_ACT_LEAKY, [&](auto generic) -> int {
    hipLaunchKernelGGL((vox_bf3_ps_kernel<Z, TY, CO8, decltype(generic)::value>), grid, dim3(64 * TY), lds, st, a, in, (const vu32x4*)wp, bias, out,
                       act, slope, xseg, accum);
    MUVO_CHECK_LAUNCH("vox_bf3_ps_kernel");
    return MUVO_OK;
  });
}

static int vox_conv_dispatch(const muvo_conv_desc* d, int Cin, int Cout, const float* in, const float* wp, const float* bias,
                             float* out, int act, float slope, hipStream_t st, bool bf3, double* moments, const float* aff) {
  if (moments && !bf3) { muvo_set_error("vox_conv: output moments need the bf16x3 kernels"); return MUVO_ERR_INVALID_ARG; }
  const int Z = d->in_sz[2];
  if (bf3 && vox_bf3_ps(Cin, Cout)) {
    const long XYZ = (long)d->in_sz[0] * d->in_sz[1] * Z;
    const size_t wstep = (size_t)cdiv(Cout, 16) * (Cout <= 8 ? 10 : 15) * 2 * 64 * 4;
    const int npass = Cin / 16, cin_total = npass > 1 ? Cin : 0;
    return vox_with_z<true>(Z, [&](auto z) -> int {
      constexpr int ZC = decltype(z)::value;
      return vox_with_bool(Cout <= 8, [&](auto co8) -> int {
        for (int ps = 0; ps < npass; ++ps) {
          const bool last = ps == npass - 1;
          const int rc = launch_vox_bf3_ps<ZC, decltype(co8)::value>(d, Cout, in + (size_t)ps * 16 * XYZ, wp + ps * wstep, last ? bias : nullptr, out,
                                                                     last ? act : MUVO_ACT_NONE, last ? slope : 0.f, st, cin_total, ps > 0,
                                                                     last ? moments : nullptr, aff);
          if (rc) return rc;
        }
        return MUVO_OK;
      });
    });
  }
  if (bf3 && vox_bf3_two_rows(Cin, Cout))
    return vox_with_z(Z, [&](auto z) -> int { return launch_vox_bf3_2row<decltype(z)::value>(d, in, wp, bias, out, act, slope, st, moments, aff); });
  if (bf3 && Cin == 8)
    return vox_with_z(Z, [&](auto z) -> int { return launch_vox_bf3<decltype(z)::value>(d, Cout, in, wp, bias, out, act, slope, st, moments, aff); });
  if (Cout == 8) return vox_with_z(Z, [&](auto z) -> int { return launch_vox_conv<2, 6, decltype(z)::value>(d, Cin, Cout, in, wp, bias, out, act, slope, st); });
  if (Cout == 16) return vox_with_z(Z, [&](auto z) -> int { return launch_vox_conv<4, 4, decltype(z)::value>(d, Cin, Cout, in, wp, bias, out, act, slope, st); });
  muvo_set_error("vox_conv: unsupported shape Cout=%d Z=%d", Cout, Z);
  return MUVO_ERR_INVALID_ARG;
}

int vox_forward(const muvo_conv_desc* d, const float* x, const float* wp, const float* bias, float* y, int act, float slope,
                hipStream_t st, bool bf3, double* moments, const float* aff) {
  if (aff && !vox_affine_ok(d)) { muvo_set_error("vox_forward: no affine staging for this shape"); return MUVO_ERR_INVALID_ARG; }
  return vox_conv_dispatch(d, d->Cin, d->Cout, x, wp, bias, y, act, slope, st, bf3 || aff != nullptr, moments, aff);
}
bool vox_affine_ok(const muvo_conv_desc* d) {
  return vox_fwd_applicable(d) && vox_bf3_shape_ok(d, 0) && vox_bf3_wgrad_shape_ok(d) && (d->Cin == 8 || d->Cin == 16);
}
int vox_dgrad(const muvo_conv_desc* d, const float* dy, const float* wp, float* dx, hipStream_t st, bool bf3) {
  return vox_conv_dispatch(d, d->Cout, d->Cin, dy, wp, nullptr, dx, MUVO_ACT_NONE, 0.f, st, bf3, nullptr, nullptr);
}

template <int RQB, int CQR, int Z, int TYB>
static int launch_vox_wgrad(const muvo_conv_desc* d, const float* x, const float* dz, float* dw, float* dbias,
                            hipStream_t st) {
  constexpr int CQB = 2;
  VoxArgs a = vox_args(d, d->Cin, d->Cout, TYB, Z, 0, nullptr);
  const int nqc = d->Cout / (4 * CQB), nrc = d->Cin / (4 * RQB);
  int xsplit = 1;
  while ((long)a.N * a.ytiles * xsplit * nqc * nrc < 1536 && a.X / (xsplit * 2) >= 8) xsplit *= 2;
  constexpr size_t lds = sizeof(float) * (3 * RQB * (TYB + 2) * (Z + 2) * 4 + 2 * CQB * TYB * Z * 4);
  static bool lds_raised = false;
  if (int rc = vox_raise_lds(lds_raised, "vox_wgrad", lds, vox_wgrad_kernel<RQB, CQR, Z, TYB>)) return rc;
  dim3 grid(a.N * a.ytiles * xsplit, nqc * nrc);
  a.ticket = muvo_det_ticket(st);
  hipLaunchKernelGGL((vox_wgrad_kernel<RQB, CQR, Z, TYB>), grid, dim3(768), lds, st, a, x, dz, dw, dbias, xsplit, nqc);
  MUVO_CHECK_LAUNCH("vox_wgrad_kernel");
  return MUVO_OK;
}

bool vox_wgrad_ps_only(const muvo_conv_desc* d) {
  return vox_geometry_ok(d, true) && (d->in_sz[2] == 16 || d->Cout == 32) && d->Cin % 16 == 0 && d->Cin <= 64 &&
         (d->Cout == 8 || d->Cout == 16 || d->Cout == 32);
}
bool vox_bf3_wgrad_shape_ok(const muvo_conv_desc* d) {
  if (vox_wgrad_ps_only(d)) return true;
  return vox_wgrad_applicable(d) && (d->Cin == 8 || d->Cin % 16 == 0) && d->Cin <= 64 && (d->Cout == 8 || d->Cout == 16);
}

template <int Z>
static int launch_vox_bf3_wgrad(const muvo_conv_desc* d, const float* x, const float* dz, float* dw, float* dbias, hipStream_t st,
                                const float* aff) {
  constexpr int CI = 8;
  constexpr int ZH = Z / 32, WROWS = 8 / ZH, ROWS = WROWS + 2;
  constexpr size_t lds = (size_t)4 * 2 * CI * (ROWS * (Z + 16) * 2 + 16) + (size_t)2 * 2 * 16 * (WROWS * Z * 2 + 16) + 64;
  static_assert(lds <= 160 * 1024, "LDS budget");
  static_assert(lds >= 15 * 256 * 4 + 64, "the reduction reuses the rings");
  const VoxArgs a = vox_args(d, d->Cin, d->Cout, WROWS, Z, 0, aff);
  const int xseg = vox_xseg(a, a.Cin / CI, 1);
  static bool lds_raised = false;
  if (int rc = vox_raise_lds(lds_raised, "vox_bf3_wgrad", lds, vox_bf3_wgrad_kernel<Z, CI, false>)) return rc;
  dim3 grid((unsigned)((long)a.N * a.ytiles * cdiv(a.X, xseg)), a.Cin / CI);
  hipLaunchKernelGGL((vox_bf3_wgrad_kernel<Z, CI, false>), grid, dim3(512), lds, st, a, x, dz, dw, dbias, xseg);
  MUVO_CHECK_LAUNCH("vox_bf3_wgrad_kernel");
  return MUVO_OK;
}

template <int Z, int CI, bool CO8>
static int launch_vox_bf3_wgrad_ps(const muvo_conv_desc* d, const float* x, const float* dz, float* dw, float* dbias, hipStream_t st,
                                   const float* aff) {
  constexpr int SW = (CI == 16 && CO8) ? VOX_WGPS_SW : 0;
  constexpr int ZH = Z >= 32 ? Z / 32 : 1, RW = Z >= 32 ? 1 : 32 / Z, WROWS = 8 / ZH * RW, ROWS = WROWS + 2;
  constexpr size_t lds = (size_t)2 * 2 * CI * (ROWS * (Z + 16) * 2 + 16) + 64;
  const VoxArgs a = vox_args(d, d->Cin, d->Cout, WROWS, Z, 0, aff);
  const int xseg = vox_xseg(a, (a.Cin / CI) * cdiv(a.Cout, 16), 1);
  static bool lds_raised = false;
  if (int rc = vox_raise_lds(lds_raised, "vox_bf3_wgrad_ps", lds, vox_bf3_wgrad_ps_kernel<Z, CI, CO8, SW>)) return rc;
  dim3 grid((unsigned)((long)a.N * a.ytiles * cdiv(a.X, xseg)), a.Cin / CI, cdiv(a.Cout, 16));
  hipLaunchKernelGGL((vox_bf3_wgrad_ps_kernel<Z, CI, CO8, SW>), grid, dim3(512 + 64 * SW), lds, st, a, x, dz, dw, dbias, xseg);
  MUVO_CHECK_LAUNCH("vox_bf3_wgrad_ps_kernel");
  return MUVO_OK;
}

int vox_wgrad(const muvo_conv_desc* d, const float* x, const float* dz, float* dw, float* dbias, hipStream_t st, bool bf3,
              const float* aff) {
  if (aff && !vox_affine_ok(d)) { muvo_set_error("vox_wgrad: no affine staging for this shape"); return MUVO_ERR_INVALID_ARG; }
  if (aff) bf3 = true;
  const int Z = d->in_sz[2];
  if (bf3) {
    if (Z == 16 && !vox_wgrad_ps_only(d)) { muvo_set_error("vox_wgrad: 16-voxel z lines need the plane-streaming kernel"); return MUVO_ERR_INVALID_ARG; }
    const bool co8 = d->Cout <= 8;
    if (d->Cin != 8)
      return vox_with_z<true>(Z, [&](auto z) -> int {
        constexpr int ZC = decltype(z)::value;
        return vox_with_bool(co8, [&](auto c) -> int { return launch_vox_bf3_wgrad_ps<ZC, 16, decltype(c)::value>(d, x, dz, dw, dbias, st, aff); });
      });
    if (co8) return vox_with_z(Z, [&](auto z) -> int { return launch_vox_bf3_wgrad_ps<decltype(z)::value, 8, true>(d, x, dz, dw, dbias, st, aff); });
    return vox_with_z(Z, [&](auto z) -> int { return launch_vox_bf3_wgrad<decltype(z)::value>(d, x, dz, dw, dbias, st, aff); });
  }
  const bool r4 = d->Cin % 16 == 0;
  return vox_with_z(Z, [&](auto z) -> int {
    constexpr int ZC = decltype(z)::value, TYB = ZC == 64 ? 4 : 8;
    return r4 ? launch_vox_wgrad<4, 2, ZC, TYB>(d, x, dz, dw, dbias, st) : launch_vox_wgrad<2, 1, ZC, TYB>(d, x, dz, dw, dbias, st);
  });
}
```

### muvo_amd/models/common.py

```python
import math

import torch
import torch.nn as nn

from muvo_amd import nn as hnn
from muvo_amd import ops
from muvo_amd.models.resnet import ResNet18Features


class RouteEncode(nn.Module):
    def __init__(self, out_channels, backbone='resnet18'):
        super().__init__()
        assert backbone == 'resnet18'
        self.backbone = ResNet18Features(in_chans=3, out_indices=(4,))
        self.out_channels = out_channels
        self.fc = hnn.Linear(512, out_channels)

    def forward(self, route):
        x = self.backbone(route)[0]
        return self.fc(ops.global_avg_pool(x))


class Policy(nn.Module):
    def __init__(self, in_channels):
        super().__init__()
        c = in_channels
        self.fc = nn.Sequential(hnn.Linear(c, c), hnn.Placeholder(), hnn.Linear(c, c), hnn.Placeholder(),
                                hnn.Linear(c, c // 2), hnn.Placeholder(), hnn.Linear(c // 2, 2), hnn.Placeholder())

    def forward(self, x):
        x = self.fc[0](x, act=ops.ACT_RELU)
        x = self.fc[2](x, act=ops.ACT_RELU)
        x = self.fc[4](x, act=ops.ACT_RELU)
        return self.fc[6](x, act=ops.ACT_TANH)


def _conv_bn_relu(cin, cout):
    return nn.Sequential(hnn.Conv2d(cin, cout, 3, 1, 1, bias=False), hnn.BatchNorm2d(cout), hnn.Placeholder())


class DecoderDS(nn.Module):
    def __init__(self, feature_info, out_channels):
        super().__init__()
        self.conv1 = _conv_bn_relu(feature_info[0]['num_chs'], out_channels)
        self.downsample_skip_convs = nn.ModuleList(
            _conv_bn_relu(feature_info[i]['num_chs'], out_channels) for i in range(1, len(feature_info)))
        self.out_channels = out_channels

    def feat_consumers(self):
        return [(self.conv1[0],)] + [(c[0],) for c in self.downsample_skip_convs]

    def forward(self, xs):
        x = self.conv1[1](self.conv1[0](xs[0]), relu=True, from_conv=True)
        for i, conv in enumerate(self.downsample_skip_convs):
            stride = xs[i].shape[-1] // xs[i + 1].shape[-1]
            pooled = ops.max_pool2d(x, stride)
            x = conv[1](conv[0](xs[i + 1]), residual=pooled, res_mode=2, relu=True, from_conv=True)
        return x


class Decoder(nn.Module):

    def __init__(self, feature_info, out_channels):
        super().__init__()
        n_upsample_skip_convs = len(feature_info) - 1
        self.conv1 = _conv_bn_relu(feature_info[-1]['num_chs'], out_channels)
        self.upsample_skip_convs = nn.ModuleList(
            _conv_bn_relu(feature_info[-i]['num_chs'], out_channels) for i in range(2, n_upsample_skip_convs + 2))
        self.out_channels = out_channels

    def forward(self, xs):
        x = self.conv1[1](self.conv1[0](xs[-1]), relu=True)
        for i, conv in enumerate(self.upsample_skip_convs):
            up = ops.interpolate_bilinear(x, xs[-(i + 2)].shape[-2:])
            x = conv[1](conv[0](xs[-(i + 2)]), residual=up, res_mode=2, relu=True)
        return x


class StyleBank:

    def __init__(self, latent, modules, styles):
        self.latent = latent
        self.shape = latent.shape
        self._styles = {id(m): s for m, s in zip(modules, styles)}

    def style_of(self, norm):
        return self._styles[id(norm)]

    @staticmethod
    def build(decoder, w):
        if isinstance(w, StyleBank):
            return w
        norms = decoder.__dict__.get('_adain_layers')
        if norms is None:
            norms = [m for m in decoder.modules() if isinstance(m, (AdaptiveInstanceNorm3d, AdaptiveInstanceNorm))]
            decoder.__dict__['_adain_layers'] = norms
        linears = [m.latent_affine for m in norms]
        if not norms or not ops.grouped_linear_supported(w, linears):
            return w
        return StyleBank(w, norms, ops.grouped_linear(w, linears))


def _style(norm, style):
    return style.style_of(norm) if isinstance(style, StyleBank) else norm.latent_affine(style)


class AdaptiveInstanceNorm3d(nn.Module):
    def __init__(self, latent_n_channels, out_channels, epsilon=1e-8):
        super().__init__()
        self.out_channels = out_channels
        self.epsilon = epsilon
        self.latent_affine = hnn.Linear(latent_n_channels, 2 * out_channels)

    def forward(self, x, style, pre_act=ops.ACT_NONE, pre_slope=0.0, moments=None):
        return ops.adain(x, _style(self, style), self.epsilon, style.shape[0], pre_act, pre_slope, moments)


class ConvInstanceNorm3d(nn.Module):
    def __init__(self, in_channels, out_channels, latent_n_channels):
        super().__init__()
        self.conv_act = nn.Sequential(hnn.Conv3d(in_channels, out_channels, 3, 1, 1), hnn.Placeholder())
        self.adaptive_norm = AdaptiveInstanceNorm3d(latent_n_channels, out_channels)

    def forward(self, x, w, lazy=None, next_conv=None):
        moments = ops.conv_moments_buffer(x, self.conv_act[0].geom)
        x = self.conv_act[0](x, act=ops.ACT_LEAKY, slope=0.2, act_bwd_fused=True, moments=moments, lazy=lazy)
        if next_conv is not None and ops.conv_affine_supported(x, next_conv.geom, moments):
            an = self.adaptive_norm
            y, raw, aff = ops.adain_lazy(x, _style(an, w), an.epsilon, ops.ACT_LEAKY, 0.2, moments)
            return y, (raw, aff)
        y = self.adaptive_norm(x, w, pre_act=ops.ACT_LEAKY, pre_slope=0.2, moments=moments)
        return y if next_conv is None else (y, None)

    def forward_with_head(self, x, w, head_conv, lazy=None):
        moments = ops.conv_moments_buffer(x, self.conv_act[0].geom)
        x = self.conv_act[0](x, act=ops.ACT_LEAKY, slope=0.2, act_bwd_fused=True, moments=moments, lazy=lazy)
        if ops.adain_head_supported(x, head_conv.weight, moments):
            an = self.adaptive_norm
            return ops.adain_head(x, _style(an, w), head_conv.weight, head_conv.bias, an.epsilon, moments, ops.ACT_LEAKY, 0.2)
        return head_conv(self.adaptive_norm(x, w, pre_act=ops.ACT_LEAKY, pre_slope=0.2, moments=moments))


class AdaptiveInstanceNorm(nn.Module):

    def __init__(self, latent_n_channels, out_channels, epsilon=1e-8):
        super().__init__()
        self.out_channels = out_channels
        self.epsilon = epsilon
        self.latent_affine = hnn.Linear(latent_n_channels, 2 * out_channels)

    def forward(self, x, style, pre_act=ops.ACT_NONE, pre_slope=0.0):
        x5 = x.unsqueeze(-3)
        y = ops.adain(x5, _style(self, style), self.epsilon, style.shape[0], pre_act, pre_slope)
        return y.squeeze(2)


class ConvInstanceNorm(nn.Module):

    def __init__(self, in_channels, out_channels, latent_n_channels):
        super().__init__()
        self.conv_act = nn.Sequential(hnn.Conv2d(in_channels, out_channels, 3, 1, 1), hnn.Placeholder())
        self.adaptive_norm = AdaptiveInstanceNorm(latent_n_channels, out_channels)

    def forward(self, x, w):
        x = self.conv_act[0](x, act=ops.ACT_LEAKY, slope=0.2, act_bwd_fused=True)
        return self.adaptive_norm(x, w, pre_act=ops.ACT_LEAKY, pre_slope=0.2)


class DecoderBlock(nn.Module):

    def __init__(self, in_channels, out_channels, latent_n_channels, upsample=False):
        super().__init__()
        self.upsample = upsample
        self.conv1 = ConvInstanceNorm(in_channels, out_channels, latent_n_channels)
        self.conv2 = ConvInstanceNorm(out_channels, out_channels, latent_n_channels)

    def forward(self, x, w):
        if self.upsample:
            x = ops.interpolate_bilinear(x, (2 * x.shape[-2], 2 * x.shape[-1]))
        return self.conv2(self.conv1(x, w), w)


class SegmentationHead(nn.Module):

    def __init__(self, in_channels, n_classes, downsample_factor):
        super().__init__()
        self.downsample_factor = downsample_factor
        self.segmentation_head = nn.Sequential(hnn.Conv2d(in_channels, n_classes, 1, 1, 0))
        self.instance_offset_head = nn.Sequential(hnn.Conv2d(in_channels, 2, 1, 1, 0))
        self.instance_center_head = nn.Sequential(hnn.Conv2d(in_channels, 1, 1, 1, 0), hnn.Placeholder())

    def forward(self, x):
        f = self.downsample_factor
        return {f'bev_segmentation_{f}': self.segmentation_head[0](x),
                f'bev_instance_offset_{f}': self.instance_offset_head[0](x),
                f'bev_instance_center_{f}': self.instance_center_head[0](x, act=ops.ACT_SIGMOID)}


class BevDecoder(nn.Module):

    def __init__(self, latent_n_channels, semantic_n_channels, constant_size=(3, 3), head='bev'):
        super().__init__()
        assert head == 'bev'
        n = 512
        self.constant_tensor = nn.Parameter(torch.randn((n, *constant_size), dtype=torch.float32))
        self.first_norm = AdaptiveInstanceNorm(latent_n_channels, out_channels=n)
        self.first_conv = ConvInstanceNorm(n, n, latent_n_channels)
        self.middle_conv = nn.ModuleList(DecoderBlock(n, n, latent_n_channels, upsample=True) for _ in range(3))
        self.conv1 = DecoderBlock(n, 256, latent_n_channels, upsample=True)
        self.head_4 = SegmentationHead(256, semantic_n_channels, downsample_factor=4)
        self.conv2 = DecoderBlock(256, 128, latent_n_channels, upsample=True)
        self.head_2 = SegmentationHead(128, semantic_n_channels, downsample_factor=2)
        self.conv3 = DecoderBlock(128, 64, latent_n_channels, upsample=True)
        self.head_1 = SegmentationHead(64, semantic_n_channels, downsample_factor=1)

    def forward(self, w):
        w = StyleBank.build(self, w)
        x = self.first_norm(self.constant_tensor, w)
        x = self.first_conv(x, w)
        for module in self.middle_conv:
            x = module(x, w)
        x = self.conv1(x, w)
        output_4 = self.head_4(x)
        x = self.conv2(x, w)
        output_2 = self.head_2(x)
        x = self.conv3(x, w)
        output_1 = self.head_1(x)
        return {**output_4, **output_2, **output_1}


class DecoderBlock3d(nn.Module):
    def __init__(self, in_channels, out_channels, latent_n_channels, upsample=False):
        super().__init__()
        self.upsample = upsample
        self.conv1 = ConvInstanceNorm3d(in_channels, out_channels, latent_n_channels)
        self.conv2 = ConvInstanceNorm3d(out_channels, out_channels, latent_n_channels)

    def forward(self, x, w, head_conv=None):
        if self.upsample:
            x = ops.upsample3d_x2(x)
        y, lazy = self.conv1(x, w, next_conv=self.conv2.conv_act[0])
        if head_conv is not None:
            return self.conv2.forward_with_head(y, w, head_conv, lazy=lazy)
        return self.conv2(y, w, lazy=lazy)


class _Head(nn.Module):

    def __init__(self, attr, key, conv, downsample_factor):
        super().__init__()
        self.downsample_factor = downsample_factor
        self._attr, self._key = attr, key
        setattr(self, attr, nn.Sequential(conv))

    def forward(self, x):
        return {f'{self._key}_{self.downsample_factor}': getattr(self, self._attr)[0](x)}

    def branch(self, x):
        m = getattr(self, self._attr)[0]
        x, y = ops.head_branch(x, m.weight, m.bias, m.geom, m._packed)
        return x, {f'{self._key}_{self.downsample_factor}': y}


def RGBHead(in_channels, n_classes, downsample_factor):
    return _Head('rgb_head', 'rgb', hnn.Conv2d(in_channels, n_classes, 1, 1, 0), downsample_factor)


def LidarReHead(in_channels, n_classes, downsample_factor):
    return _Head('lidar_re_head', 'lidar_reconstruction', hnn.Conv2d(in_channels, n_classes, 1, 1, 0), downsample_factor)


def LidarSegHead(in_channels, n_classes, downsample_factor):
    return _Head('seg_head', 'lidar_segmentation', hnn.Conv2d(in_channels, n_classes, 1, 1, 0), downsample_factor)


def SemHead(in_channels, n_classes, downsample_factor):
    return _Head('sem_head', 'semantic_image', hnn.Conv2d(in_channels, n_classes, 1, 1, 0), downsample_factor)


def DepthHead(in_channels, n_classes, downsample_factor):
    return _Head('depth_head', 'depth', hnn.Conv2d(in_channels, n_classes, 1, 1, 0), downsample_factor)


def VoxelSemHead(in_channels, n_classes, downsample_factor):
    return _Head('segmentation_head', 'voxel', hnn.Conv3d(in_channels, n_classes, 1, 1, 0), downsample_factor)


class VoxelDecoder1(nn.Module):
    def __init__(self, latent_n_channels, semantic_n_channels, feature_channels=512, constant_size=(3, 3, 1)):
        super().__init__()
        n = feature_channels
        self.constant_tensor = nn.Parameter(torch.randn((2 * n, *constant_size), dtype=torch.float32))
        self.first_norm = AdaptiveInstanceNorm3d(latent_n_channels, out_channels=2 * n)
        self.first_conv = ConvInstanceNorm3d(2 * n, n, latent_n_channels)
        self.middle_conv = nn.ModuleList(DecoderBlock3d(n, n, latent_n_channels, upsample=True) for _ in range(3))
        self.conv1 = DecoderBlock3d(n, n // 2, latent_n_channels, upsample=True)
        self.head_4 = VoxelSemHead(n // 2, semantic_n_channels, downsample_factor=4)
        self.conv2 = DecoderBlock3d(n // 2, n // 4, latent_n_channels, upsample=True)
        self.head_2 = VoxelSemHead(n // 4, semantic_n_channels, downsample_factor=2)
        self.conv3 = DecoderBlock3d(n // 4, n // 8, latent_n_channels, upsample=True)
        self.head_1 = VoxelSemHead(n // 8, semantic_n_channels, downsample_factor=1)

    def forward(self, w):
        w = StyleBank.build(self, w)
        x = self.first_norm(self.constant_tensor, w)
        x = self.first_conv(x, w)
        for module in self.middle_conv:
            x = module(x, w)
        x = self.conv1(x, w)
        x, output_4 = self.head_4.branch(x)
        x = self.conv2(x, w)
        x, output_2 = self.head_2.branch(x)
        h1 = self.head_1
        output_1 = {f'{h1._key}_{h1.downsample_factor}': self.conv3(x, w, head_conv=getattr(h1, h1._attr)[0])}
        return {**output_4, **output_2, **output_1}


class _Seed1x1ConvTFn(torch.autograd.Function):

    @staticmethod
    def forward(ctx, x, weight, bias, act):
        x = x.contiguous()
        n, ci = x.shape[0], x.shape[1]
        co, kh, kw = weight.shape[1:]
        ncol = co * kh * kw
        y = torch.empty(n, co, kh, kw, device=x.device, dtype=torch.float32)
        ops.gemm(x, weight, y, n, ncol, ci, ci, 1, ncol, 1, ncol, bias=bias, bias_div=kh * kw, act=act)
        ctx.weight, ctx.bias, ctx.act = weight, bias, act
        ctx.save_for_backward(x, y)
        return y

    @staticmethod
    def backward(ctx, dy):
        import ctypes as C
        x, y = ctx.saved_tensors
        weight, bias = ctx.weight, ctx.bias
        n, ci = x.shape[0], x.shape[1]
        co, kh, kw = weight.shape[1:]
        ncol = co * kh * kw
        dy = dy.contiguous()
        dz = torch.empty_like(dy)
        L = ops.lib()
        ops._ck(L.muvo_act_bwd(ops._f(y), ops._f(dy), ops._f(dz), ops._i64(dy.numel()), ctx.act, ops._fl(0.0), ops._st()))
        dx = None
        if ctx.needs_input_grad[0]:
            dx = torch.empty_like(x)
            ops.gemm(dz, weight, dx, n, ci, ncol, ncol, 1, 1, ncol, ci)
        ops.gemm(x, dz, ops.grad_of(weight), ci, ncol, n, 1, ci, ncol, 1, ncol, mode=1)
        if bias is not None:
            ops._ck(L.muvo_bias_grad_nchw(ops._f(dz), ops._f(ops.grad_of(bias)), n, co, ops._i64(kh * kw), ops._st()))
        return dx, None, None, None


class ConvDecoder(nn.Module):
    def __init__(self, latent_n_channels, out_channels, constant_size=(5, 13), head='rgb'):
        super().__init__()
        n_channels = 512
        self.linear = nn.Sequential(hnn.Linear(latent_n_channels, n_channels), hnn.Placeholder())
        P = hnn.Placeholder
        self.pre_transpose_conv = nn.Sequential(
            hnn.ConvTranspose2d(n_channels, n_channels, constant_size), P(),
            hnn.ConvTranspose2d(n_channels, n_channels, 5, 2, 2, 1), P(),
            hnn.ConvTranspose2d(n_channels, n_channels, 5, 2, 2, 1), P(),
            hnn.ConvTranspose2d(n_channels, n_channels, 6, 2, 2), P())
        head_module = {'rgb': RGBHead, 'lidar_re': LidarReHead, 'lidar_seg': LidarSegHead, 'sem_image': SemHead,
                       'depth': DepthHead}[head]
        self.trans_conv1 = nn.Sequential(hnn.ConvTranspose2d(n_channels, 256, 6, 2, 2), P())
        self.head_4 = head_module(256, out_channels, downsample_factor=4)
        self.trans_conv2 = nn.Sequential(hnn.ConvTranspose2d(256, 128, 6, 2, 2), P())
        self.head_2 = head_module(128, out_channels, downsample_factor=2)
        self.trans_conv3 = nn.Sequential(hnn.ConvTranspose2d(128, 64, 6, 2, 2), P())
        self.head_1 = head_module(64, out_channels, downsample_factor=1)

    def forward(self, x):
        x = self.linear[0](x)
        seed = self.pre_transpose_conv[0]
        x = _Seed1x1ConvTFn.apply(x.view(x.shape[0], -1, 1, 1), seed.weight, seed.bias, ops.ACT_ELU)
        for i in (2, 4, 6):
            x = self.pre_transpose_conv[i](x, act=ops.ACT_ELU)
        x, output_4 = self._stage(self.trans_conv1[0], self.head_4, x)
        x, output_2 = self._stage(self.trans_conv2[0], self.head_2, x)
        _, output_1 = self._stage(self.trans_conv3[0], self.head_1, x)
        return {**output_4, **output_2, **output_1}

    @staticmethod
    def _stage(conv, head, x):
        hc = getattr(head, head._attr)[0]
        if ops.conv_head_supported(x, conv.geom, hc.geom):
            y, logits = ops.conv_head(x, conv.weight, conv.bias, conv.geom, conv._packed, ops.ACT_ELU, 0.0,
                                      hc.weight, hc.bias, hc.geom, hc._packed)
            return y, {f'{head._key}_{head.downsample_factor}': logits}
        return head.branch(conv(x, act=ops.ACT_ELU))


# ... 16 lines not shown
```

### muvo_amd/nn.py

```python
import math

import torch
import torch.nn as nn

from muvo_amd import ops


def _uniform_(t, bound):
    with torch.no_grad():
        t.uniform_(-bound, bound)


class _ConvNd(nn.Module):
    def __init__(self, nd, transposed, cin, cout, ksz, stride=1, pad=0, dil=1, out_pad=0, bias=True):
        super().__init__()
        self.geom = ops.ConvGeom(nd, transposed, cin, cout, ksz, stride, pad, dil, out_pad)
        k = self.geom.ksz[3 - nd:]
        shape = (cin, cout, *k) if transposed else (cout, cin, *k)
        self.weight = nn.Parameter(torch.empty(shape))
        self.bias = nn.Parameter(torch.empty(cout)) if bias else None
        self._packed = ops._PackedWeights()
        fan_in = shape[1] * math.prod(k)
        _uniform_(self.weight, 1.0 / math.sqrt(fan_in))
        if bias:
            _uniform_(self.bias, 1.0 / math.sqrt(fan_in))

    def forward(self, x, act=ops.ACT_NONE, slope=0.0, act_bwd_fused=False, moments=None, lazy=None):
        return ops.conv(x, self.weight, self.bias, self.geom, self._packed, act, slope, act_bwd_fused, moments, lazy)


class Conv2d(_ConvNd):
    def __init__(self, cin, cout, ksz, stride=1, pad=0, bias=True):
        super().__init__(2, False, cin, cout, ksz, stride, pad, 1, 0, bias)


class Conv3d(_ConvNd):
    def __init__(self, cin, cout, ksz, stride=1, pad=0, bias=True):
        super().__init__(3, False, cin, cout, ksz, stride, pad, 1, 0, bias)


class ConvTranspose2d(_ConvNd):
    def __init__(self, cin, cout, ksz, stride=1, pad=0, out_pad=0, bias=True):
        super().__init__(2, True, cin, cout, ksz, stride, pad, 1, out_pad, bias)


class Linear(nn.Module):
    def __init__(self, cin, cout, bias=True):
        super().__init__()
        self.weight = nn.Parameter(torch.empty(cout, cin))
        self.bias = nn.Parameter(torch.empty(cout)) if bias else None
        _uniform_(self.weight, 1.0 / math.sqrt(cin))
        if bias:
            _uniform_(self.bias, 1.0 / math.sqrt(cin))

    def forward(self, x, act=ops.ACT_NONE, slope=0.0):
        return ops.linear(x, self.weight, self.bias, act, slope)


class BatchNorm2d(nn.Module):

    def __init__(self, c, eps=1e-5, momentum=0.1):
        super().__init__()
        self.eps, self.momentum = eps, momentum
        self.weight = nn.Parameter(torch.ones(c))
        self.bias = nn.Parameter(torch.zeros(c))
        self.register_buffer('running_mean', torch.zeros(c))
        self.register_buffer('running_var', torch.ones(c))
        self.register_buffer('num_batches_tracked', torch.tensor(0, dtype=torch.long))

    def forward(self, x, residual=None, res_mode=1, relu=False, consumers=(), sole_consumer=False, from_conv=False):
        return ops.bn_act(x, self, residual, res_mode, relu, consumers, sole_consumer, from_conv)

    def _save_to_state_dict(self, destination, prefix, keep_vars):
        ops.flush_bn_counters()
        super()._save_to_state_dict(destination, prefix, keep_vars)

    def _load_from_state_dict(self, state_dict, prefix, *args, **kwargs):
        ops.flush_bn_counters()
        super()._load_from_state_dict(state_dict, prefix, *args, **kwargs)


class LayerNorm(nn.Module):
    def __init__(self, e, eps=1e-5):
        super().__init__()
        self.eps = eps
        self.weight = nn.Parameter(torch.ones(e))
        self.bias = nn.Parameter(torch.zeros(e))


class Placeholder(nn.Module):

    def forward(self, x):
        return x


class _MHAParams(nn.Module):
    def __init__(self, e):
        super().__init__()
        self.in_proj_weight = nn.Parameter(torch.empty(3 * e, e))
        self.in_proj_bias = nn.Parameter(torch.zeros(3 * e))
        self.out_proj = Linear(e, e)
        bound = math.sqrt(6.0 / (e + 3 * e))
        _uniform_(self.in_proj_weight, bound)
        with torch.no_grad():
            self.out_proj.bias.zero_()


class TransformerEncoderLayer(nn.Module):

    def __init__(self, e, nhead, dim_ff=2048, dropout=0.1):
        super().__init__()
        self.nhead, self.p = nhead, dropout
        self.self_attn = _MHAParams(e)
        self.linear1 = Linear(e, dim_ff)
        self.linear2 = Linear(dim_ff, e)
        self.norm1 = LayerNorm(e)
        self.norm2 = LayerNorm(e)

    def forward(self, x, seed):
        p = self.p if self.training else 0.0
        pm = 0.0 if getattr(self, 'module_dropout_off', False) else p
        sa = self.self_attn
        qkv = ops.linear(x, sa.in_proj_weight, sa.in_proj_bias)
        o = ops.attention(qkv, self.nhead, p, seed)
        a = sa.out_proj(o)
        x = ops.add_dropout_layernorm(x, a, self.norm1, pm, seed + 1)
        f = self.linear1(x, act=ops.ACT_RELU)
        f = ops.dropout(f, pm, seed + 2)
        f = self.linear2(f)
        return ops.add_dropout_layernorm(x, f, self.norm2, pm, seed + 3)


class TransformerEncoder(nn.Module):
    def __init__(self, e, nhead, num_layers, dropout=0.1):
        super().__init__()
        self.layers = nn.ModuleList(TransformerEncoderLayer(e, nhead, dropout=dropout) for _ in range(num_layers))

    def forward(self, x, seed):
        for i, layer in enumerate(self.layers):
            x = layer(x, seed + 16 * i)
        return x


class GRUCell(nn.Module):

    def __init__(self, cin, hid):
        super().__init__()
        self.hid = hid
        b = 1.0 / math.sqrt(hid)
        self.weight_ih = nn.Parameter(torch.empty(3 * hid, cin))
        self.weight_hh = nn.Parameter(torch.empty(3 * hid, hid))
        self.bias_ih = nn.Parameter(torch.empty(3 * hid))
        self.bias_hh = nn.Parameter(torch.empty(3 * hid))
        for p in self.parameters():
            _uniform_(p, b)

    def forward(self, x, h):
        gi = ops.linear(x, self.weight_ih, self.bias_ih)
        gh = ops.linear(h, self.weight_hh, self.bias_hh)
        return ops.gru_pointwise(gi, gh, h)
```

### muvo_amd/ops.py

```python
import collections
import contextlib
import ctypes as C
import math
import os
import threading
import weakref

import torch

_HERE = os.path.dirname(os.path.abspath(__file__))
_LIB_PATH = os.environ.get('MUVO_HIP_LIB') or os.path.join(_HERE, 'libmuvo_hip.so')
_lib = None
_lock = threading.Lock()

ACT_NONE, ACT_RELU, ACT_LEAKY, ACT_ELU, ACT_TANH, ACT_SIGMOID = 0, 1, 2, 3, 4, 5


class ConvDesc(C.Structure):
    _fields_ = [('nd', C.c_int32), ('transposed', C.c_int32), ('N', C.c_int32), ('Cin', C.c_int32), ('Cout', C.c_int32),
                ('in_sz', C.c_int32 * 3), ('out_sz', C.c_int32 * 3), ('ksz', C.c_int32 * 3), ('stride', C.c_int32 * 3),
                ('pad', C.c_int32 * 3), ('dil', C.c_int32 * 3)]


class GemmDesc(C.Structure):
    _fields_ = [('M', C.c_int32), ('N', C.c_int32), ('K', C.c_int32),
                ('sam', C.c_int64), ('sak', C.c_int64), ('sbk', C.c_int64), ('sbn', C.c_int64), ('scm', C.c_int64),
                ('B1', C.c_int32), ('B2', C.c_int32),
                ('a_b1', C.c_int64), ('a_b2', C.c_int64), ('b_b1', C.c_int64), ('b_b2', C.c_int64),
                ('c_b1', C.c_int64), ('c_b2', C.c_int64),
                ('alpha', C.c_float), ('bias_div', C.c_int32), ('act', C.c_int32), ('slope', C.c_float),
                ('mode', C.c_int32)]


EXPORTS = [
    'muvo_last_error', 'muvo_abi_version', 'muvo_selftest_mfma', 'muvo_set_deterministic', 'muvo_get_deterministic', 'muvo_reset_accumulators',
    'muvo_conv_set_products', 'muvo_conv_get_products',
    'muvo_conv_set_mode', 'muvo_conv_get_mode', 'muvo_conv_set_bf16x3_min_gflop', 'muvo_conv_pack_sizes', 'muvo_conv_workspace_bytes', 'muvo_conv_kernel_family', 'muvo_conv_kernel_variant', 'muvo_conv_pack_weights', 'muvo_conv_forward', 'muvo_conv_dgrad', 'muvo_conv_prepare_dy', 'muvo_conv_wgrad', 'muvo_bias_grad_nchw',
    'muvo_gemm',
    'muvo_pack_table_item_bytes', 'muvo_conv_pack_table_add', 'muvo_linear_bf16x3_pack_table_add', 'muvo_pack_table_run',
    'muvo_linear_bf16x3_pack_floats', 'muvo_linear_bf16x3_pack', 'muvo_linear_bf16x3_workspace_bytes', 'muvo_linear_bf16x3_split',
    'muvo_linear_bf16x3_forward', 'muvo_linear_bf16x3_dgrad', 'muvo_linear_bf16x3_wgrad',
    'muvo_bn_train_fwd', 'muvo_bn_train_bwd', 'muvo_adain_fwd', 'muvo_adain_bwd',
    'muvo_add_dropout_layernorm_fwd', 'muvo_add_dropout_layernorm_bwd',
    'muvo_act_fwd', 'muvo_act_bwd', 'muvo_dropout', 'muvo_axpby', 'muvo_copy2d', 'muvo_colsum_acc', 'muvo_batchsum',
    'muvo_nchw_to_tokens', 'muvo_tokens_to_nchw', 'muvo_maxpool2d_fwd', 'muvo_maxpool2d_bwd', 'muvo_avgpool_fwd',
    'muvo_avgpool_bwd', 'muvo_upsample3d_x2_fwd', 'muvo_upsample3d_x2_bwd', 'muvo_preprocess_image',
    'muvo_preprocess_route', 'muvo_divide_scalar', 'muvo_resize_bilinear', 'muvo_resize_nearest_f32',
    'muvo_resize_nearest_u8', 'muvo_softmax_dropout_fwd', 'muvo_softmax_dropout_bwd', 'muvo_gru_fwd', 'muvo_gru_bwd',
    'muvo_rssm_sample_fwd', 'muvo_rssm_sample_bwd',
    'muvo_spatial_loss_fwd', 'muvo_spatial_loss_bwd', 'muvo_spatial_loss_masked_fwd', 'muvo_spatial_loss_masked_bwd', 'muvo_voxel_loss_stats_doubles', 'muvo_voxel_loss_coef_floats',
    'muvo_voxel_loss_fwd', 'muvo_voxel_loss_bwd', 'muvo_l1_rows_fwd', 'muvo_l1_rows_bwd', 'muvo_kl_loss_fwd',
    'muvo_kl_loss_bwd', 'muvo_adamw_step', 'muvo_chamfer_loss_ws_doubles', 'muvo_chamfer_loss_fwd', 'muvo_chamfer_loss_bwd',
    'muvo_ssim_frames', 'muvo_sqdiff_frames', 'muvo_chamfer_sums', 'muvo_ssc_counts', 'muvo_seg_confusion', 'muvo_seg_confusion_index',
    'muvo_frustum_cells', 'muvo_frustum_pool_fwd', 'muvo_frustum_pool_bwd', 'muvo_depth_expectation',
    'muvo_resize_bilinear_bwd', 'muvo_softmax_channel_fwd', 'muvo_softmax_channel_bwd',
    'muvo_range_projection', 'muvo_voxel_grid', 'muvo_seg_ce_fwd', 'muvo_seg_ce_bwd', 'muvo_ssim_maps', 'muvo_ssim_bwd',
    'muvo_instance_labels', 'muvo_pixel_augment', 'muvo_preprocess_route_aug',
    'muvo_split_planes_bytes', 'muvo_split_planes', 'muvo_attention_supported', 'muvo_attention_fwd', 'muvo_attention_bwd',
    'muvo_conv_dgrad_accumulate', 'muvo_conv_forward_moments_supported', 'muvo_conv_forward_moments', 'muvo_adain_fwd_moments',
    'muvo_adain_head_supported', 'muvo_adain_head_fwd', 'muvo_adain_head_bwd', 'muvo_bf3_loop_clock',
    'muvo_grouped_linear_fwd', 'muvo_grouped_linear_bwd', 'muvo_conv_prepare_dy_head', 'muvo_conv_prepare_dy_head_supported',
    'muvo_conv_forward_head_supported', 'muvo_conv_forward_head',
    'muvo_adain_affine', 'muvo_conv_affine_supported', 'muvo_conv_forward_affine', 'muvo_conv_wgrad_affine',
    'muvo_fake_allreduce', 'muvo_resize_bilinear_aa', 'muvo_bn_train_fwd_planes', 'muvo_bn_train_bwd_planes', 'muvo_conv_forward_planes',
    'muvo_stem_conv_supported', 'muvo_stem_conv_forward', 'muvo_stem_conv_wgrad',
    'muvo_rssm_supported', 'muvo_rssm_transposed_floats', 'muvo_rssm_scratch_floats', 'muvo_rssm_forward', 'muvo_rssm_backward',
    'muvo_voxelize_scratch_bytes', 'muvo_voxelize_frames',
    'muvo_birdview_decode_frames', 'muvo_label_components_frames', 'muvo_depth_semantic_decode_frames',
    'muvo_range_projection_frames', 'muvo_voxel_grid_frames',
    'muvo_attention_stream_supported', 'muvo_attention_stream_blocks', 'muvo_attention_stream_fwd', 'muvo_attention_stream_bwd',
    'muvo_voxel_rows_scratch_bytes', 'muvo_voxel_rows_logits', 'muvo_voxel_rows_grid', 'muvo_voxel_rows_write', 'muvo_image_u8',
    'muvo_panel_image', 'muvo_panel_logits', 'muvo_panel_labels', 'muvo_panel_fill', 'muvo_panel_bars', 'muvo_panel_scatter',
    'muvo_panel_voxel_top_logits', 'muvo_panel_voxel_top_grid',
    'muvo_icp_state_doubles', 'muvo_icp_ws_doubles', 'muvo_icp_init', 'muvo_icp_iterate',
]


def lib():
    global _lib
    if _lib is None:
        with _lock:
            if _lib is None:
                if not os.path.exists(_LIB_PATH):
                    raise RuntimeError(f'{_LIB_PATH} not found: build it with `python -m muvo_amd.build` '
                                       '(there is no fallback path)')
                L = C.CDLL(_LIB_PATH)
                L.muvo_last_error.restype = C.c_char_p
                L.muvo_conv_workspace_bytes.restype = C.c_int64
                L.muvo_linear_bf16x3_workspace_bytes.restype = C.c_int64
                L.muvo_pack_table_item_bytes.restype = C.c_int64
                L.muvo_split_planes_bytes.restype = C.c_int64
                L.muvo_rssm_transposed_floats.restype = C.c_int64
                L.muvo_rssm_scratch_floats.restype = C.c_int64
                L.muvo_voxelize_scratch_bytes.restype = C.c_int64
                L.muvo_voxel_rows_scratch_bytes.restype = C.c_int64
                L.muvo_chamfer_loss_ws_doubles.restype = C.c_int64
                L.muvo_icp_state_doubles.restype = C.c_int64
                L.muvo_icp_ws_doubles.restype = C.c_int64
                for name in EXPORTS:
                    getattr(L, name)
                _lib = L
    return _lib


def _ck(rc):
    if rc != 0:
        msg = lib().muvo_last_error().decode()
        reset_accumulators()
        raise RuntimeError(f'muvo_hip error {rc}: {msg}')


_MOMENT_BUFS = []


def reset_accumulators():
    try:
        if _lib is not None:
            _lib.muvo_reset_accumulators()
        live = []
        for r in _MOMENT_BUFS:
            t = r()
            if t is not None:
                t.zero_()
                live.append(r)
        _MOMENT_BUFS[:] = live
    except Exception:
        pass


def _st():
    return C.c_void_p(torch._C._cuda_getCurrentRawStream(torch.cuda.current_device()))


def _p(t):
    if t is None:
        return C.c_void_p(0)
    assert t.is_cuda and t.is_contiguous(), 'muvo_hip ops need contiguous device tensors'
    return C.c_void_p(t.data_ptr())


def _f(t):
    assert t is None or t.dtype == torch.float32
    return _p(t)


def _i64(v):
    return C.c_int64(int(v))


def _fl(v):
    return C.c_float(float(v))


_weight_epoch = [0]


def bump_weight_epoch():
    _weight_epoch[0] += 1


CONV_F32, CONV_BF16X3, CONV_BF16 = 0, 1, 2


def set_conv_mode(mode, min_gflop=None):
    _ck(lib().muvo_conv_set_mode(CONV_BF16X3 if int(mode) == CONV_BF16 else int(mode)))
    _ck(lib().muvo_conv_set_products(1 if int(mode) == CONV_BF16 else 3))
    if min_gflop is not None:
        _ck(lib().muvo_conv_set_bf16x3_min_gflop(C.c_double(min_gflop)))
    bump_weight_epoch()
    _plan_epoch[0] += 1


def get_conv_mode():
    m = lib().muvo_conv_get_mode()
    return CONV_BF16 if (m == CONV_BF16X3 and lib().muvo_conv_get_products() == 1) else m


_plan_epoch = [0]


def set_deterministic(on=True):
    global GROUPED_LINEAR
    _ck(lib().muvo_set_deterministic(1 if on else 0))
    GROUPED_LINEAR = (not on) and os.environ.get('MUVO_GROUPED_LINEAR', '1') != '0'
    bump_weight_epoch()
    _plan_epoch[0] += 1


def get_deterministic():
    return bool(lib().muvo_get_deterministic())


_join_queued = [False]


def _queue_final_join():
    def cb():
        _join_queued[0] = False
        join_side_streams()
    try:
        torch.autograd.Variable._execution_engine.queue_callback(cb)
        _join_queued[0] = True
    except RuntimeError:
        pass


def grad_of(p):
    if not p.requires_grad:
        return scratch('frozen_grad_dump', p.numel(), p.device).view(-1)[:p.numel()].view(p.shape)
    if _side_streams and not _join_queued[0]:
        _queue_final_join()
    if p.grad is None:
        view = getattr(p, '_muvo_flat_grad', None)
        if view is not None:
            view.zero_()
            p.grad = view
        else:
            p.grad = torch.zeros_like(p)
    return p.grad


_scratch = {}


def _stream_key(device):
    device = torch.device(device)
    if device.type != 'cuda':
        return 0
    return torch._C._cuda_getCurrentRawStream(device.index if device.index is not None else torch.cuda.current_device())


def scratch_zeroed(name, nfloats, device):
    key = (name, device, torch.float32, _stream_key(device))
    t = _scratch.get(key)
    if t is None or t.numel() < nfloats:
        t = torch.zeros(int(nfloats), device=device, dtype=torch.float32)
        _scratch[key] = t
    return t


def scratch(name, nfloats, device, dtype=torch.float32):
    key = (name, device, dtype, _stream_key(device))
    t = _scratch.get(key)
    if t is None or t.numel() < nfloats:
        t = torch.empty(int(nfloats), device=device, dtype=dtype)
        _scratch[key] = t
    return t


STREAMS = os.environ.get('MUVO_STREAMS', '1') != '0'
_side_streams = {}
# ... 574 lines not shown
        self.fwd_plan = self.dgr_plan = None


def _wkey(w):
    return (w._version, _weight_epoch[0], w.data_ptr())


def _is_alias(buf, weight):
    return buf is not None and buf.data_ptr() == weight.data_ptr()


_PACKED_ATTRS = (('fwd', 'fwd_key', 'fwd_plan'), ('dgr', 'dgr_key', 'dgr_plan'))


def _packed_weight(plan, packed, weight, dgrad):
    a_buf, a_key, a_plan = _PACKED_ATTRS[dgrad]
    buf, key, k = getattr(packed, a_buf), getattr(packed, a_key), _wkey(weight)
    if (plan.fam_dgrad if dgrad else plan.fam_fwd) == 3 and weight.is_contiguous():
        buf = weight.detach().view(-1)
    else:
        size = plan.pack_dgrad if dgrad else plan.pack_fwd
        if buf is None or buf.numel() < size or _is_alias(buf, weight):
            buf, key = torch.empty(size, device=weight.device, dtype=torch.float32), None
        if key == k and getattr(packed, a_plan) == plan.pack_key:
            return buf
        _ck(lib().muvo_conv_pack_weights(C.byref(plan.desc), _f(weight), None if dgrad else _f(buf), _f(buf) if dgrad else None,
                                         _st()))
        if not dgrad:
            _PACKS.register(_PackEntry('conv', plan.desc, weight, weakref.ref(packed), plan.pack_key, plan.pack_key[1]))
    setattr(packed, a_buf, buf)
    setattr(packed, a_key, k)
    setattr(packed, a_plan, plan.pack_key)
    return buf


_PackEntry = collections.namedtuple('_PackEntry', 'kind desc weight holder pack_key epoch')


class _PackRegistry:
    def __init__(self):
        self.entries, self.seen = [], set()
        self.sig, self.dev, self.n, self.nblk, self.batched = None, None, 0, 0, []

    def register(self, entry):
        key = (id(entry.holder()), entry.pack_key)
        if key not in self.seen:
            self.seen.add(key)
            self.entries.append(entry)


_PACKS = _PackRegistry()
_PACK_BATCH = os.environ.get('MUVO_PACK_BATCH', '1') != '0'


def repack_all():
    flush_bn_counters()
    R = _PACKS
    if not R.entries or not _PACK_BATCH:
        return
    L = lib()
    ptr = lambda t: 0 if t is None else t.data_ptr()
    live = [(e, e.holder()) for e in R.entries]
    live = [(e, pk) for e, pk in live if pk is not None and e.epoch == _plan_epoch[0]]
    if len(live) != len(R.entries):
        R.entries = [e for e, _ in live]
        R.seen = {(id(pk), e.pack_key) for e, pk in live}
        R.sig = None
    if not R.entries:
        return
    sig = tuple((ptr(pk.fwd), ptr(pk.dgr), e.weight.data_ptr()) for e, pk in live)
    if sig != R.sig:
        item = L.muvo_pack_table_item_bytes()
        cap = 16 * len(live) + 8
        host = torch.zeros(cap * item, dtype=torch.uint8)
        n, nblk = C.c_int(0), C.c_int64(0)
        R.batched = []
        for e, pk in live:
            if pk.fwd is None and pk.dgr is None:
                continue
            if _is_alias(pk.fwd, e.weight) or _is_alias(pk.dgr, e.weight):
                continue
            if e.kind == 'conv':
                rc = L.muvo_conv_pack_table_add(C.c_void_p(host.data_ptr()), cap, C.byref(n), C.byref(nblk), C.byref(e.desc),
                                                _f(e.weight), _f(pk.fwd), _f(pk.dgr))
            else:
                rc = L.muvo_linear_bf16x3_pack_table_add(C.c_void_p(host.data_ptr()), cap, C.byref(n), C.byref(nblk),
                                                         e.desc[0], e.desc[1], _f(e.weight), _f(pk.fwd), _f(pk.dgr))
            if rc == 0:
                R.batched.append(e)
            elif rc != 1:
                _ck(rc)
        R.n, R.nblk = n.value, nblk.value
        R.dev = host[:max(R.n, 1) * item].to(live[0][0].weight.device)
        R.sig = sig
    if R.n:
        _ck(L.muvo_pack_table_run(C.c_void_p(R.dev.data_ptr()), R.n, _i64(R.nblk), _st()))
        for e in R.batched:
            pk = e.holder()
            if pk is None:
                continue
            k = _wkey(e.weight)
            if pk.fwd is not None:
                pk.fwd_key = k
            if pk.dgr is not None:
                pk.dgr_key = k
            if e.kind == 'conv':
                pk.fwd_plan = e.pack_key if pk.fwd is not None else pk.fwd_plan
                pk.dgr_plan = e.pack_key if pk.dgr is not None else pk.dgr_plan


_KEEP_WS = os.environ.get('MUVO_KEEP_WS', '1') != '0'


def _bracket(plan, direction):
    e0, e1 = KERNEL_TIMING.bracket(*plan.timing[direction])
    e0.record()
    return e1


@contextlib.contextmanager
def _on_wgrad_stream(wst, device, reads, dy_slot=None):
    cur = torch.cuda.current_stream(device)
    if wst is None or wst == cur:
        yield
        return
    wst.wait_stream(cur)
    for t in reads:
        if t is not None:
            t.record_stream(wst)
    with torch.cuda.stream(wst):
        yield
        if dy_slot is not None:
            dy_slot.done = torch.cuda.Event()
            dy_slot.done.record(wst)


class _DyWorkspace:
    __slots__ = ('wst', 'device', 'slot')

    def __init__(self, wst, device):
        self.wst, self.device, self.slot = wst, device, None

    def get(self, nfloats):
        if self.wst is None:
            return scratch('conv_ws_dy', nfloats, self.device)
        if self.slot is None:
            self.slot = _dy_ws_acquire(nfloats, self.device)
        assert self.slot.t.numel() >= nfloats
        return self.slot.t


class ConvFn(torch.autograd.Function):
    @staticmethod
    def forward(ctx, x, weight, bias, geom, packed, act, slope, act_bwd_fused=False, moments=None, aff_src=None, aff=None):
        ctx.aff = aff
        if aff is not None:
            x = aff_src
        xp = getattr(x, '_muvo_planes', None)
        x_ph = getattr(x, '_muvo_planes_only', False)
        if not x_ph:
            x = x.contiguous()
        plan = geom.plan_for(x)
        hf = getattr(ctx, '_head_fwd', None)
        ctx.geom, ctx.packed, ctx.act, ctx.slope, ctx.act_bwd_fused = geom, packed, act, slope, act_bwd_fused
        ctx.weight, ctx.bias = weight, bias
        ctx.stem = bool(plan.supports('muvo_stem_conv_supported') and get_conv_mode() != CONV_F32 and bias is None
                        and act == ACT_NONE and moments is None and aff is None and not x_ph and not ctx.needs_input_grad[0]
                        and hf is None and weight.is_contiguous())
        if ctx.stem:
            return ConvFn._stem_forward(ctx, plan, x, weight)
        wp = _packed_weight(plan, packed, weight, 0)
        y = torch.empty(plan.oshape, device=x.device, dtype=torch.float32)
        e1 = _bracket(plan, 'fwd') if KERNEL_TIMING is not None else None
        use_xp = (xp is not None and plan.ws_fwd_x > 0 and plan.fam_fwd == 1 and hf is None and aff is None
                  and moments is None and xp[1] == _stream_key(x.device) and xp[0].numel() * 4 >= plan.ws_fwd_x)
        ws = ConvFn._forward_workspace(ctx, plan, x, xp[0] if use_xp else None, x_ph)
        L, d = lib(), C.byref(plan.desc)
        if hf is not None:
            _ck(L.muvo_conv_forward_head(d, _f(x), _f(wp), _f(bias), _f(y), act, _fl(slope), _p(ws),
                                         _f(hf[0]), _f(hf[1]), hf[0].shape[0], _f(hf[2]), _st()))
        elif aff is not None:
            _ck(L.muvo_conv_forward_affine(d, _f(x), _f(aff), _f(wp), _f(bias), _f(y), act, _fl(slope), _p(moments), _st()))
        elif moments is not None:
            _ck(L.muvo_conv_forward_moments(d, _f(x), _f(wp), _f(bias), _f(y), act, _fl(slope), _p(moments), _st()))
        elif use_xp:
            _ck(L.muvo_conv_forward_planes(d, None if x_ph else _f(x), _f(wp), _f(bias), _f(y), act, _fl(slope), _p(ws), 1, _st()))
        else:
            _ck(L.muvo_conv_forward(d, _f(x), _f(wp), _f(bias), _f(y), act, _fl(slope), _p(ws), _st()))
        if e1 is not None:
            e1.record()
        ctx.save_for_backward(x, y if (act != ACT_NONE and not act_bwd_fused) else None)
        return y

    @staticmethod
    def _forward_workspace(ctx, plan, x, planes, x_ph):
        wgrad_follows = ctx.needs_input_grad[1]
        if x_ph and not (planes is not None and (plan.ws_wgrad_x > 0 or not wgrad_follows)):
            raise RuntimeError('muvo_hip: a planes-only tensor (BNActFn keep_f32=False) reached a convolution that needs its fp32 values')
        if planes is not None:
            ws = planes
            keep_ws = plan.ws_wgrad_x > 0 and wgrad_follows and (_KEEP_WS or x_ph)
        else:
            keep_ws = plan.ws_fwd_x > 0 and plan.ws_wgrad_x > 0 and wgrad_follows and _KEEP_WS
            if keep_ws:
                ws = torch.empty((plan.ws_fwd_x + 3) // 4, device=x.device, dtype=torch.float32)
            else:
                ws = scratch('conv_ws', (plan.ws_fwd_x + 3) // 4, x.device) if plan.ws_fwd_x else None
        ctx.ws_x = ws if keep_ws else None
        ctx.x_is_placeholder = x_ph
        return ws

    @staticmethod
    def _stem_forward(ctx, plan, x, weight):
        y = torch.empty(plan.oshape, device=x.device, dtype=torch.float32)
        e1 = _bracket(plan, 'stem_fwd') if KERNEL_TIMING is not None else None
        _ck(lib().muvo_stem_conv_forward(C.byref(plan.desc), _f(x), _f(weight), None, _f(y), 0, _st()))
        if e1 is not None:
            e1.record()
        ctx.ws_x, ctx.x_is_placeholder = None, False
        ctx.save_for_backward(x, None)
        return y

    @staticmethod
    def _stem_backward(ctx, plan, x, dy):
        weight = ctx.weight
        if not (weight.requires_grad and dy is not None):
            return
        dy = dy.contiguous()
        gw = grad_of(weight)
        with _on_wgrad_stream(wgrad_stream(x.device), x.device, (x, dy)):
            e1 = _bracket(plan, 'stem_wgrad') if KERNEL_TIMING is not None else None
            _ck(lib().muvo_stem_conv_wgrad(C.byref(plan.desc), _f(x), _f(dy), _f(gw), _st()))
            if e1 is not None:
                e1.record()

    @staticmethod
    def backward(ctx, dy):
        return ConvFn._backward(ctx, dy, None)

    @staticmethod
    def _backward(ctx, dy, head):
        x, y = ctx.saved_tensors
        plan = ctx.geom.plan_for(x)
        if getattr(ctx, 'stem', False):
            ConvFn._stem_backward(ctx, plan, x, dy)
            return (None,) * 11
        need_dx, need_dw = ctx.needs_input_grad[0], ctx.weight.requires_grad
        fused_dy = plan.dy_planes and need_dx and need_dw
        dy_ws = _DyWorkspace(wgrad_stream(x.device) if need_dw else None, x.device)
        dz, planes = ConvFn._resolve_dy(ctx, plan, x, y, dy, head, fused_dy, dy_ws)
        dx = None
        if need_dx:
            dx, planes = ConvFn._data_grad(ctx, plan, x, dz, planes, fused_dy, dy_ws)
        if need_dw:
            ConvFn._weight_grad(ctx, plan, x, y, dz, planes, need_dx and plan.ws_dgrad_dy > 0, fused_dy, dy_ws)
        return (dx,) + (None,) * 10

    @staticmethod
    def _resolve_dy(ctx, plan, x, y, dy, head, fused_dy, dy_ws):
        dyp = getattr(dy, '_muvo_planes', None) if dy is not None else None
        if dy is not None and dyp is None:
            dy = dy.contiguous()
        use_act = ctx.act != ACT_NONE and not ctx.act_bwd_fused
        if head is not None and not (fused_dy and plan.supports('muvo_conv_prepare_dy_head_supported', head[1].shape[0])):
            gl, head_w, _, head_wgrad = head
            hd = torch.einsum('nk...,kc->nc...', gl, head_w.view(head_w.shape[0], -1))
            dy = hd.contiguous() if dy is None else dy + hd
            head_wgrad()
            head = None
        if dyp is not None:
            if not (fused_dy and head is None and ctx.bias is None and not use_act
                    and dyp[0].numel() >= plan.dy_planes_floats and dyp[1] == _stream_key(x.device)):
                raise RuntimeError('muvo_hip: a gradient that exists only as split planes reached a convolution backward that cannot read them')
            return dyp[0], dyp[0]
        if fused_dy:
            return ConvFn._split_dy(ctx, plan, x, y, dy, head, use_act, dy_ws.get(plan.dy_planes_floats))
        if use_act:
            dz = torch.empty_like(dy)
            _ck(lib().muvo_act_bwd(_f(y), _f(dy), _f(dz), _i64(dy.numel()), ctx.act, _fl(ctx.slope), _st()))
            return dz, None
        return dy, None

    @staticmethod
    def _split_dy(ctx, plan, x, y, dy, head, use_act, planes):
        L, d, bias = lib(), C.byref(plan.desc), ctx.bias
        act = ctx.act if use_act else ACT_NONE
        if head is None:
            _ck(L.muvo_conv_prepare_dy(d, _f(y) if use_act else None, _f(dy), act, _fl(ctx.slope), _p(planes),
                                       _f(grad_of(bias)) if bias is not None else None, _st()))
            return dy, planes
        gl, head_w, head_b, head_wgrad = head
        co = head_w.shape[0]
        ride = use_act and head_w.requires_grad
        if not ride:
            head_wgrad()
        _ck(L.muvo_conv_prepare_dy_head(d, _f(y) if use_act else None, _f(dy) if dy is not None else None,
                                        _f(gl.contiguous()), _f(head_w.contiguous().view(co, -1)), co, act, _fl(ctx.slope),
                                        _p(planes), _f(grad_of(bias)) if bias is not None else None,
                                        _f(grad_of(head_w)) if ride else None,
                                        _f(grad_of(head_b)) if (ride and head_b is not None) else None, _st()))
        if dy is None:
            dy = y if y is not None else x
        return dy, planes

    @staticmethod
    def _data_grad(ctx, plan, x, dz, planes, fused_dy, dy_ws):
        wp = _packed_weight(plan, ctx.packed, ctx.weight, 1)
        dx = torch.empty(x.shape, device=dz.device, dtype=torch.float32)
        e1 = _bracket(plan, 'dgrad') if KERNEL_TIMING is not None else None
        if planes is None and (plan.ws_dgrad_dy > 0 or plan.ws_wgrad_dy > 0):
            planes = dy_ws.get(plan.dy_planes_floats)
        _ck(lib().muvo_conv_dgrad(C.byref(plan.desc), _f(dz), _f(wp), _f(dx), _p(planes), 1 if fused_dy else 0, _st()))
        if e1 is not None:
            e1.record()
        return dx, planes

    @staticmethod
    def _weight_grad(ctx, plan, x, y, dz, ws_dy, dy_is_split, fused_dy, dy_ws):
        bias = ctx.bias
        gw = grad_of(ctx.weight)
        db = grad_of(bias) if (bias is not None and not fused_dy) else None
        ws_x = ctx.ws_x
        x_ph = getattr(ctx, 'x_is_placeholder', False)
        xptr = ws_x if x_ph else x
        flags = (1 if ws_x is not None else 0) | (2 if (dy_is_split and plan.ws_wgrad_dy > 0) else 0)
        with _on_wgrad_stream(dy_ws.wst, x.device, (xptr, y, dz, ws_x, ctx.aff), dy_ws.slot):
            ws = scratch_zeroed('wgrad', plan.pack_fwd, x.device)
            e1 = _bracket(plan, 'wgrad') if KERNEL_TIMING is not None else None
            if ws_x is None and plan.ws_wgrad_x:
                ws_x = scratch('conv_ws', (plan.ws_wgrad_x + 3) // 4, x.device)
            if plan.ws_wgrad_dy and ws_dy is None:
                ws_dy = scratch('conv_ws_dy', (plan.ws_wgrad_dy + 3) // 4, x.device)
            if ctx.aff is not None:
                _ck(lib().muvo_conv_wgrad_affine(C.byref(plan.desc), _f(x), _f(ctx.aff), _f(dz), _f(gw), _f(db), _st()))
            else:
                assert not x_ph or (flags & 1)
                _ck(lib().muvo_conv_wgrad(C.byref(plan.desc), _f(xptr), _f(dz), _f(ws), _f(gw), _f(db), _p(ws_x), _p(ws_dy),
                                          flags, _st()))
            if e1 is not None:
                e1.record()


def conv(x, weight, bias, geom, packed, act=ACT_NONE, slope=0.0, act_bwd_fused=False, moments=None, lazy=None):
    if lazy is not None:
        return ConvFn.apply(x, weight, bias, geom, packed, act, slope, act_bwd_fused, moments, lazy[0], lazy[1])
    y = ConvFn.apply(x, weight, bias, geom, packed, act, slope, act_bwd_fused, moments)
    if (BN_PLANES and bias is None and act == ACT_NONE and moments is None and x.requires_grad and weight.requires_grad
            and torch.is_grad_enabled() and geom.plan_for(x).dy_planes):
        y._muvo_dy_planes_ok = True
    return y


CONV_AFFINE = os.environ.get('MUVO_CONV_AFFINE', '1') != '0'


def conv_affine_supported(x, geom, moments):
    if not CONV_AFFINE or moments is None or x.dim() != 5 or not (x.requires_grad and torch.is_grad_enabled()):
        return False
    return geom.plan_for(x).supports('muvo_conv_affine_supported')


CONV_MOMENTS = os.environ.get('MUVO_CONV_MOMENTS', '1') != '0'


def conv_moments_buffer(x, geom):
    if not CONV_MOMENTS or not geom.plan_for(x).supports('muvo_conv_forward_moments_supported'):
        return None
    n = x.shape[0]
    cache = geom.__dict__.setdefault('_moments', {})
    buf = cache.get((n, x.device))
    if buf is None:
        buf = cache[(n, x.device)] = torch.zeros(n, geom.cout, 2, device=x.device, dtype=torch.float64)
        _MOMENT_BUFS.append(weakref.ref(buf))
    return buf


def _grad_is_private(g):
    return g._base is None and g._use_count() <= 2


class HeadBranchFn(torch.autograd.Function):

    @staticmethod
    def forward(ctx, x, weight, bias, geom, packed):
        y = ConvFn.forward(ctx, x, weight, bias, geom, packed, ACT_NONE, 0.0)
        return x.view_as(x), y

    @staticmethod
    def backward(ctx, gx, gy):
        x, _ = ctx.saved_tensors
        weight, bias = ctx.weight, ctx.bias
        if gy is None:
            return (gx,) + (None,) * 4
        plan = ctx.geom.plan_for(x)
        L, d = lib(), C.byref(plan.desc)
        gy = gy.contiguous()
        dx = None
        if ctx.needs_input_grad[0]:
            wp = _packed_weight(plan, ctx.packed, weight, 1)
            if gx is not None and gx.is_contiguous() and _grad_is_private(gx):
                dx = gx
                _ck(L.muvo_conv_dgrad_accumulate(d, _f(gy), _f(wp), _f(dx), _st()))
            else:
                dx = torch.empty_like(x)
                _ck(L.muvo_conv_dgrad(d, _f(gy), _f(wp), _f(dx), None, 0, _st()))
                if gx is not None:
                    dx = dx + gx
        if weight.requires_grad:
            ws = scratch_zeroed('wgrad', plan.pack_fwd, x.device)
            _ck(L.muvo_conv_wgrad(d, _f(x), _f(gy), _f(ws), _f(grad_of(weight)), _f(grad_of(bias)) if bias is not None else None,
                                  None, None, 0, _st()))
        return (dx,) + (None,) * 4


class ConvHeadFn(torch.autograd.Function):

    @staticmethod
    def forward(ctx, x, weight, bias, geom, packed, act, slope, head_w, head_b, head_geom, head_packed):
        plan = geom.plan_for(x)
        co = head_geom.cout
        fused = plan.supports('muvo_conv_forward_head_supported', co)
        logits = None
        if fused:
            logits = torch.empty((plan.n, co) + plan.oshape[2:], device=x.device, dtype=torch.float32)
            ctx._head_fwd = (head_w.contiguous().view(co, -1), head_b, logits)
        y = ConvFn.forward(ctx, x, weight, bias, geom, packed, act, slope)
        ctx._head_fwd = None
        ctx.save_for_backward(x, y)
        ctx.head = (head_w, head_b, head_geom)
        ctx.set_materialize_grads(False)
        if not fused:
            hplan = head_geom.plan_for(y)
            hwp = _packed_weight(hplan, head_packed, head_w, 0)
            logits = torch.empty(hplan.oshape, device=x.device, dtype=torch.float32)
            _ck(lib().muvo_conv_forward(C.byref(hplan.desc), _f(y), _f(hwp), _f(head_b), _f(logits), ACT_NONE, _fl(0.0), None, _st()))
        return y, logits

    @staticmethod
    def backward(ctx, gy, gl):
        if gl is None:
            if gy is None:
                return (None,) * 11
            return ConvFn._backward(ctx, gy, None)[:7] + (None,) * 4
        x, y = ctx.saved_tensors
        head_w, head_b, head_geom = ctx.head
        hplan = head_geom.plan_for(y)
        gl = gl.contiguous()

        def head_wgrad():
            if head_w.requires_grad:
                ws = scratch_zeroed('wgrad', hplan.pack_fwd, x.device)
                _ck(lib().muvo_conv_wgrad(C.byref(hplan.desc), _f(y), _f(gl), _f(ws), _f(grad_of(head_w)),
                                          _f(grad_of(head_b)) if head_b is not None else None, None, None, 0, _st()))
        return ConvFn._backward(ctx, gy, (gl, head_w, head_b, head_wgrad))[:7] + (None,) * 4


def conv_head_supported(x, geom, head_geom, act_bwd_fused=False):
    if not CONV_HEAD or not (x.requires_grad and torch.is_grad_enabled()) or act_bwd_fused:
        return False
    plan = geom.plan_for(x)
    if not (plan.fam_dgrad == 1 and plan.fam_wgrad == 1):
        return False
    hplan = head_geom.plan(plan.n, plan.out_sz)
    return (hplan.fam_fwd == 3 and hplan.fam_wgrad == 3
            and plan.supports('muvo_conv_prepare_dy_head_supported', head_geom.cout))


CONV_HEAD = os.environ.get('MUVO_CONV_HEAD', '1') != '0'


def conv_head(x, weight, bias, geom, packed, act, slope, head_w, head_b, head_geom, head_packed):
    return ConvHeadFn.apply(x, weight, bias, geom, packed, act, slope, head_w, head_b, head_geom, head_packed)


def head_branch(x, weight, bias, geom, packed):
    plan = geom.plan_for(x)
    if plan.fam_fwd == 3 and plan.fam_dgrad == 3 and plan.fam_wgrad == 3 and x.requires_grad and torch.is_grad_enabled():
        return HeadBranchFn.apply(x, weight, bias, geom, packed)
    return x, conv(x, weight, bias, geom, packed)


BN_PLANES = os.environ.get('MUVO_BN_PLANES', '1') != '0'


_NAN_SCALAR = {}


def _nan_placeholder(shape, device):
    device = torch.device(device)
    src = _NAN_SCALAR.get(device)
    if src is None:
        src = _NAN_SCALAR[device] = torch.full((1,), float('nan'), device=device, dtype=torch.float32)
    return src.expand(shape)


class BNActFn(torch.autograd.Function):

    @staticmethod
    def forward(ctx, x, residual, bn, res_mode, relu, training, planes=False, keep_f32=True, dx_planes=False):
        x = x.contiguous()
        n, c = x.shape[:2]
        s = x.numel() // (n * c)
        mean = torch.empty(c, device=x.device, dtype=torch.float32)
        rstd = torch.empty(c, device=x.device, dtype=torch.float32)
        if residual is not None:
            residual = residual.contiguous()
        if not training:
            raise RuntimeError('eval-mode BatchNorm is not part of the training hot path (reference keeps train() mode '
                               'even in validation, trainer.py:405)')
        mask_mode = 0 if not relu else (1 if (residual is not None and res_mode == 1) else 2)
        keep_f32 = keep_f32 or not planes or mask_mode == 1
        y = torch.empty_like(x) if keep_f32 else _nan_placeholder(x.shape, x.device)
        if planes:
            pl = torch.empty((lib().muvo_split_planes_bytes(n, c, _i64(s)) + 3) // 4, device=x.device, dtype=torch.float32)
            _ck(lib().muvo_bn_train_fwd_planes(_f(x), _f(bn.weight), _f(bn.bias), _f(residual), _f(y) if keep_f32 else None, _f(mean),
                                               _f(rstd), _f(bn.running_mean), _f(bn.running_var), n, c, _i64(s), _fl(bn.eps),
                                               _fl(bn.momentum), res_mode if residual is not None else 0, int(relu), _p(pl), _st()))
            _BN_PLANES_OUT.append((pl, _stream_key(x.device), not keep_f32))
        else:
            ws = torch.empty(2 * c, device=x.device, dtype=torch.float64)
            _ck(lib().muvo_bn_train_fwd(_f(x), _f(bn.weight), _f(bn.bias), _f(residual), _f(y), _f(mean), _f(rstd),
                                        _f(bn.running_mean), _f(bn.running_var), _p(ws), n, c, _i64(s), _fl(bn.eps),
                                        _fl(bn.momentum), res_mode if residual is not None else 0, int(relu), _st()))
        _BN_PENDING.append(bn)
        ctx.bn, ctx.dims = bn, (n, c, s)
# ... 290 lines not shown
            else:
                outs.append(None)
            off += w
        return tuple(outs)


def cat_last(xs):
    return CatLastFn.apply(*xs)


class SliceLastFn(torch.autograd.Function):

    @staticmethod
    def forward(ctx, x, a, b):
        x = x.contiguous()
        rows, tot = x.shape
        y = torch.empty(rows, b - a, device=x.device, dtype=torch.float32)
        _ck(lib().muvo_copy2d(C.c_void_p(x.data_ptr() + 4 * a), _f(y), _i64(rows), _i64(b - a), _i64(tot), _i64(b - a), 0,
                              _st()))
        ctx.a, ctx.b, ctx.tot, ctx.rows = a, b, tot, rows
        return y

    @staticmethod
    def backward(ctx, dy):
        dy = dy.contiguous()
        dx = torch.zeros(ctx.rows, ctx.tot, device=dy.device, dtype=torch.float32)
        _ck(lib().muvo_copy2d(_f(dy), C.c_void_p(dx.data_ptr() + 4 * ctx.a), _i64(ctx.rows), _i64(ctx.b - ctx.a),
                              _i64(ctx.b - ctx.a), _i64(ctx.tot), 0, _st()))
        return dx, None, None


def slice_last(x, a, b):
    return SliceLastFn.apply(x, a, b)


class TokensFn(torch.autograd.Function):

    @staticmethod
    def forward(ctx, xi, xl, pos_i, pos_l, type_emb):
        xi, xl = xi.contiguous(), xl.contiguous()
        n, c = xi.shape[:2]
        li, ll = xi.shape[2] * xi.shape[3], xl.shape[2] * xl.shape[3]
        tok = torch.empty(li + ll, n, c, device=xi.device, dtype=torch.float32)
        L = lib()
        te = type_emb.contiguous()
        _ck(L.muvo_nchw_to_tokens(_f(xi), _f(pos_i), _f(te), 2, _f(tok), n, c, li, 0, _st()))
        _ck(L.muvo_nchw_to_tokens(_f(xl), _f(pos_l), C.c_void_p(te.data_ptr() + 4), 2, _f(tok), n, c, ll, li, _st()))
        ctx.shapes = (xi.shape, xl.shape, li, ll, n, c)
        ctx.type_emb = type_emb
        return tok

    @staticmethod
    def backward(ctx, dtok):
        dtok = dtok.contiguous()
        si, sl, li, ll, n, c = ctx.shapes
        L = lib()
        dxi = torch.empty(si, device=dtok.device, dtype=torch.float32)
        dxl = torch.empty(sl, device=dtok.device, dtype=torch.float32)
        _ck(L.muvo_tokens_to_nchw(_f(dtok), _f(dxi), n, c, li, 0, _st()))
        _ck(L.muvo_tokens_to_nchw(_f(dtok), _f(dxl), n, c, ll, li, _st()))
        te = ctx.type_emb
        if te.requires_grad:
            tmp = torch.zeros(2, c, device=dtok.device, dtype=torch.float32)
            _ck(L.muvo_colsum_acc(_f(dtok), _f(tmp[0]), _i64(li * n), _i64(c), _i64(c), _st()))
            _ck(L.muvo_colsum_acc(C.c_void_p(dtok.data_ptr() + 4 * li * n * c), _f(tmp[1]), _i64(ll * n), _i64(c),
                                  _i64(c), _st()))
            g = grad_of(te)
            for k in range(2):
                _ck(L.muvo_copy2d(_f(tmp[k]), C.c_void_p(g.data_ptr() + 4 * k), _i64(c), _i64(1), _i64(1), _i64(2), 1,
                                  _st()))
        return dxi, dxl, None, None, None


def make_tokens(xi, xl, pos_i, pos_l, type_emb):
    return TokensFn.apply(xi, xl, pos_i, pos_l, type_emb)


class UntokenFn(torch.autograd.Function):

    @staticmethod
    def forward(ctx, tok, l0, h, w):
        tok = tok.contiguous()
        ltot, n, c = tok.shape
        x = torch.empty(n, c, h, w, device=tok.device, dtype=torch.float32)
        _ck(lib().muvo_tokens_to_nchw(_f(tok), _f(x), n, c, h * w, l0, _st()))
        ctx.dims = (ltot, n, c, l0, h * w)
        return x

    @staticmethod
    def backward(ctx, dx):
        dx = dx.contiguous()
        ltot, n, c, l0, l = ctx.dims
        dtok = torch.zeros(ltot, n, c, device=dx.device, dtype=torch.float32)
        _ck(lib().muvo_nchw_to_tokens(_f(dx), None, None, 0, _f(dtok), n, c, l, l0, _st()))
        return dtok, None, None, None


def untoken(tok, l0, h, w):
    return UntokenFn.apply(tok, l0, h, w)


class MaxPool2dFn(torch.autograd.Function):
    @staticmethod
    def forward(ctx, x, k, s, p):
        x = x.contiguous()
        n, c, h, w = x.shape
        oh, ow = (h + 2 * p - k) // s + 1, (w + 2 * p - k) // s + 1
        y = torch.empty(n, c, oh, ow, device=x.device, dtype=torch.float32)
        idx = torch.empty(n, c, oh, ow, device=x.device, dtype=torch.uint8)
        _ck(lib().muvo_maxpool2d_fwd(_f(x), _f(y), _p(idx), _i64(n * c), h, w, oh, ow, k, s, p, _st()))
        ctx.dims = (n, c, h, w, oh, ow, k, s, p)
        ctx.save_for_backward(idx)
        return y

    @staticmethod
    def backward(ctx, dy):
        (idx,) = ctx.saved_tensors
        n, c, h, w, oh, ow, k, s, p = ctx.dims
        dy = dy.contiguous()
        dx = torch.empty(n, c, h, w, device=dy.device, dtype=torch.float32)
        _ck(lib().muvo_maxpool2d_bwd(_f(dy), _p(idx), _f(dx), _i64(n * c), h, w, oh, ow, k, s, p, _st()))
        return dx, None, None, None


def max_pool2d(x, k, s=None, p=0):
    return MaxPool2dFn.apply(x, k, s or k, p)


class GlobalAvgPoolFn(torch.autograd.Function):
    @staticmethod
    def forward(ctx, x):
        x = x.contiguous()
        n, c = x.shape[:2]
        s = x.numel() // (n * c)
        y = torch.empty(n, c, device=x.device, dtype=torch.float32)
        _ck(lib().muvo_avgpool_fwd(_f(x), _f(y), _i64(n * c), _i64(s), _st()))
        ctx.shape = x.shape
        return y

    @staticmethod
    def backward(ctx, dy):
        dy = dy.contiguous()
        shape = ctx.shape
        dx = torch.empty(shape, device=dy.device, dtype=torch.float32)
        g = shape[0] * shape[1]
        _ck(lib().muvo_avgpool_bwd(_f(dy), _f(dx), _i64(g), _i64(dx.numel() // g), _st()))
        return dx


def global_avg_pool(x):
    return GlobalAvgPoolFn.apply(x)


class Upsample3dFn(torch.autograd.Function):
    @staticmethod
    def forward(ctx, x):
        x = x.contiguous()
        n, c, d, h, w = x.shape
        y = torch.empty(n, c, 2 * d, 2 * h, 2 * w, device=x.device, dtype=torch.float32)
        _ck(lib().muvo_upsample3d_x2_fwd(_f(x), _f(y), _i64(n * c), d, h, w, _st()))
        ctx.shape = x.shape
        return y

    @staticmethod
    def backward(ctx, dy):
        dy = dy.contiguous()
        n, c, d, h, w = ctx.shape
        dx = torch.empty(ctx.shape, device=dy.device, dtype=torch.float32)
        _ck(lib().muvo_upsample3d_x2_bwd(_f(dy), _f(dx), _i64(n * c), d, h, w, _st()))
        return dx


def upsample3d_x2(x):
    return Upsample3dFn.apply(x)


class AttentionFn(torch.autograd.Function):

    @staticmethod
    def forward(ctx, qkv, nheads, p, seed):
        qkv = qkv.contiguous()
        l, n, e3 = qkv.shape
        e = e3 // 3
        dh = e // nheads
        scale = 1.0 / (dh ** 0.5)
        dev = qkv.device
        S = torch.empty(n, nheads, l, l, device=dev, dtype=torch.float32)
        gemm(qkv, qkv, S, l, l, dh, n * e3, 1, 1, n * e3, l, alpha=scale, B1=n, B2=nheads,
             a_b=(e3, dh), b_b=(e3, dh), c_b=(nheads * l * l, l * l), b_off=e)
        P = torch.empty_like(S)
        Pd = torch.empty_like(S) if p > 0 else None
        _ck(lib().muvo_softmax_dropout_fwd(_f(S), _f(P), _f(Pd), _i64(n * nheads * l), l, _fl(p), C.c_uint64(seed),
                                           _st()))
        del S
        o = torch.empty(l, n, e, device=dev, dtype=torch.float32)
        pa = Pd if Pd is not None else P
        gemm(pa, qkv, o, l, dh, l, l, 1, n * e3, 1, n * e, B1=n, B2=nheads, a_b=(nheads * l * l, l * l),
             b_b=(e3, dh), c_b=(e, dh), b_off=2 * e)
        ctx.dims = (l, n, e, nheads, dh, scale, p, seed)
        ctx.save_for_backward(qkv, P)
        return o

    @staticmethod
    def backward(ctx, do):
        qkv, P = ctx.saved_tensors
        l, n, e, nheads, dh, scale, p, seed = ctx.dims
        e3 = 3 * e
        do = do.contiguous()
        dev = do.device
        dqkv = torch.empty_like(qkv)
        if p > 0:
            Pd = torch.empty_like(P)
            _ck(lib().muvo_dropout(_f(P), _f(Pd), _i64(P.numel()), _fl(p), C.c_uint64(seed), _st()))
        else:
            Pd = P
        bP = (nheads * l * l, l * l)
        gemm(Pd, do, dqkv, l, dh, l, 1, l, n * e, 1, n * e3, B1=n, B2=nheads, a_b=bP, b_b=(e, dh), c_b=(e3, dh),
             c_off=2 * e)
        dPd = torch.empty_like(P)
        gemm(do, qkv, dPd, l, l, dh, n * e, 1, 1, n * e3, l, B1=n, B2=nheads, a_b=(e, dh), b_b=(e3, dh), c_b=bP,
             b_off=2 * e)
        dS = dPd
        _ck(lib().muvo_softmax_dropout_bwd(_f(P), _f(dPd), _f(dS), _i64(n * nheads * l), l, _fl(p), C.c_uint64(seed),
                                           _st()))
        gemm(dS, qkv, dqkv, l, dh, l, l, 1, n * e3, 1, n * e3, alpha=scale, B1=n, B2=nheads, a_b=bP, b_b=(e3, dh),
             c_b=(e3, dh), b_off=e)
        gemm(dS, qkv, dqkv, l, dh, l, 1, l, n * e3, 1, n * e3, alpha=scale, B1=n, B2=nheads, a_b=bP, b_b=(e3, dh),
             c_b=(e3, dh), c_off=e)
        return dqkv, None, None, None


class FlashAttentionFn(torch.autograd.Function):

    @staticmethod
    def forward(ctx, qkv, nheads, p, seed):
        qkv = qkv.contiguous()
        l, n, e3 = qkv.shape
        e = e3 // 3
        o = torch.empty(l, n, e, device=qkv.device, dtype=torch.float32)
        lse = torch.empty(n * nheads, l, device=qkv.device, dtype=torch.float32)
        _ck(lib().muvo_attention_fwd(_f(qkv), _f(o), _f(lse), l, n, nheads, e // nheads, _fl(p), C.c_uint64(seed), _st()))
        ctx.dims = (l, n, nheads, e // nheads, p, seed)
        ctx.save_for_backward(qkv, o, lse)
        return o

    @staticmethod
    def backward(ctx, do):
        qkv, o, lse = ctx.saved_tensors
        l, n, nheads, dh, p, seed = ctx.dims
        dqkv = torch.empty_like(qkv)
        _ck(lib().muvo_attention_bwd(_f(qkv), _f(o), _f(do.contiguous()), _f(lse), _f(dqkv), l, n, nheads, dh, _fl(p),
                                     C.c_uint64(seed), _st()))
        return dqkv, None, None, None


class StreamAttentionFn(torch.autograd.Function):

    @staticmethod
    def forward(ctx, qkv, nheads, p, seed):
        qkv = qkv.contiguous()
        l, n, e3 = qkv.shape
        e = e3 // 3
        o = torch.empty(l, n, e, device=qkv.device, dtype=torch.float32)
        lse = torch.empty(n * nheads, l, device=qkv.device, dtype=torch.float32)
        _ck(lib().muvo_attention_stream_fwd(_f(qkv), _f(o), _f(lse), l, n, nheads, e // nheads, _fl(p), C.c_uint64(seed), _st()))
        ctx.dims = (l, n, nheads, e // nheads, p, seed)
        ctx.save_for_backward(qkv, o, lse)
        return o

    @staticmethod
    def backward(ctx, do):
        qkv, o, lse = ctx.saved_tensors
        l, n, nheads, dh, p, seed = ctx.dims
        dqkv = torch.empty_like(qkv)
        dws = torch.empty_like(lse)
        _ck(lib().muvo_attention_stream_bwd(_f(qkv), _f(o), _f(do.contiguous()), _f(lse), _f(dqkv), _f(dws), l, n, nheads, dh,
                                            _fl(p), C.c_uint64(seed), _st()))
        return dqkv, None, None, None


FLASH_ATTENTION = os.environ.get('MUVO_FLASH_ATTN', '1') != '0'
STREAM_MIN_L = 385


def attention_path(l, dh):
    if FLASH_ATTENTION:
        if lib().muvo_attention_supported(l, dh):
            return 'fused'
        if l >= STREAM_MIN_L and lib().muvo_attention_stream_supported(l, dh):
            return 'stream'
    return 'unfused'


_ATTENTION_FNS = {'fused': FlashAttentionFn, 'stream': StreamAttentionFn, 'unfused': AttentionFn}


def attention(qkv, nheads, p, seed):
    l, _, e3 = qkv.shape
    return _ATTENTION_FNS[attention_path(l, e3 // 3 // nheads)].apply(qkv, nheads, p, seed)


class GRUPointwiseFn(torch.autograd.Function):
    @staticmethod
    def forward(ctx, gi, gh, h):
        gi, gh, h = gi.contiguous(), gh.contiguous(), h.contiguous()
        b, hd = h.shape
        hn = torch.empty_like(h)
        _ck(lib().muvo_gru_fwd(_f(gi), _f(gh), _f(h), _f(hn), b, hd, _st()))
        ctx.save_for_backward(gi, gh, h)
        return hn

    @staticmethod
    def backward(ctx, dhn):
        gi, gh, h = ctx.saved_tensors
        b, hd = h.shape
        dhn = dhn.contiguous()
        dgi, dgh, dh = torch.empty_like(gi), torch.empty_like(gh), torch.empty_like(h)
        _ck(lib().muvo_gru_bwd(_f(gi), _f(gh), _f(h), _f(dhn), _f(dgi), _f(dgh), _f(dh), b, hd, _st()))
        return dgi, dgh, dh


def gru_pointwise(gi, gh, h):
    return GRUPointwiseFn.apply(gi, gh, h)
# ... 892 lines not shown
```

Before: 25.64.

## Fuse trilinear upsample adjoint into voxel conv dgrad epilogue

Adds an UP2 epilogue to the bf16x3 voxel dgrad kernels. It applies the x2 trilinear upsample backward in registers: z is reduced with DPP lane shuffles and x is carried across planes, so the kernel writes a half-resolution partial result. A small finish kernel then reduces y and merges the segment boundaries. The upsampling decoder block now routes through the conv with up2_src, so the full-resolution dx tensor is never materialised and the separate upsample-backward pass is skipped. The cost is extra epilogue complexity, a workspace allocation, and the risk of boundary and segment-merge errors.

```diff
diff --git a/include/muvo_hip.h b/include/muvo_hip.h
--- a/include/muvo_hip.h
+++ b/include/muvo_hip.h
@@ -92,6 +92,9 @@
                         const float* dlogits, float* dx, float* dstyle, float* dhead_w, float* dhead_b, double* ws, int N, int C,
                         int CO, int64_t S, int act, float slope, void* stream);
 int muvo_conv_dgrad_accumulate(const muvo_conv_desc* d, const float* dy, const float* wp_dgrad, float* dx, void* stream);
+int64_t muvo_conv_dgrad_up2_ws_floats(const muvo_conv_desc* d);
+int muvo_conv_dgrad_up2(const muvo_conv_desc* d, const float* dy, const float* wp_dgrad, float* dx_low, float* ws, int64_t ws_floats,
+                        void* stream);
 int muvo_conv_prepare_dy(const muvo_conv_desc* d, const float* y, const float* dy, int act, float slope, void* ws_dy,
                          float* dbias, void* stream);
 int muvo_conv_prepare_dy_head_supported(const muvo_conv_desc* d, int CO);
diff --git a/muvo_amd/csrc/conv_gemm.hip b/muvo_amd/csrc/conv_gemm.hip
--- a/muvo_amd/csrc/conv_gemm.hip
+++ b/muvo_amd/csrc/conv_gemm.hip
@@ -1011,6 +1011,20 @@
   return run_phases(pl.dgr, pl.ndgr, dy, wp_dgrad, nullptr, dx, MUVO_ACT_NONE, 0.f, ws, (hipStream_t)stream, ws_valid != 0);
 }
 
+int64_t muvo_conv_dgrad_up2_ws_floats(const muvo_conv_desc* d) {
+  if (check_desc(d) || pw_applicable(d) || !vox_dgrad_ok(d) || !vox_uses_bf3(d, 1)) return 0;
+  return vox_dgrad_up2_ws_floats(d);
+}
+
+int muvo_conv_dgrad_up2(const muvo_conv_desc* d, const float* dy, const float* wp_dgrad, float* dx_low, float* ws, int64_t ws_floats,
+                        void* stream) {
+  int rc = check_desc(d);
+  if (rc) return rc;
+  MUVO_CHECK_ARG(dy && wp_dgrad && dx_low && ws, "conv_dgrad_up2: null pointer");
+  MUVO_CHECK_ARG(muvo_conv_dgrad_up2_ws_floats(d) > 0, "conv_dgrad_up2: shape not served (muvo_conv_dgrad_up2_ws_floats == 0)");
+  return vox_dgrad_up2(d, dy, wp_dgrad, dx_low, ws, (long)ws_floats, (hipStream_t)stream);
+}
+
 int muvo_conv_dgrad_accumulate(const muvo_conv_desc* d, const float* dy, const float* wp_dgrad, float* dx, void* stream) {
   int rc = check_desc(d);
   if (rc) return rc;
diff --git a/muvo_amd/csrc/conv_vox.h b/muvo_amd/csrc/conv_vox.h
--- a/muvo_amd/csrc/conv_vox.h
+++ b/muvo_amd/csrc/conv_vox.h
@@ -11,6 +11,9 @@
                 hipStream_t st, bool bf3, double* moments = nullptr, const float* aff = nullptr);
 bool vox_affine_ok(const muvo_conv_desc* d);
 int vox_dgrad(const muvo_conv_desc* d, const float* dy, const float* wp, float* dx, hipStream_t st, bool bf3);
+bool vox_dgrad_up2_shape_ok(const muvo_conv_desc* d);
+long vox_dgrad_up2_ws_floats(const muvo_conv_desc* d);
+int vox_dgrad_up2(const muvo_conv_desc* d, const float* dy, const float* wp, float* dx_low, float* ws, long ws_floats, hipStream_t st);
 bool vox_bf3_wgrad_shape_ok(const muvo_conv_desc* d);
 bool vox_wgrad_ps_only(const muvo_conv_desc* d);
 int vox_wgrad(const muvo_conv_desc* d, const float* x, const float* dz, float* dw, float* dbias, hipStream_t st, bool bf3,
diff --git a/muvo_amd/csrc/conv_vox.hip b/muvo_amd/csrc/conv_vox.hip
--- a/muvo_amd/csrc/conv_vox.hip
+++ b/muvo_amd/csrc/conv_vox.hip
@@ -346,11 +346,155 @@
   lo = __builtin_bit_cast(unsigned, l);
 }
 
-template <int CK, int Z, int TY, bool GENERIC>
+__device__ __forceinline__ float vox_dpp_row_ror1(float v) {
+  return __int_as_float(__builtin_amdgcn_update_dpp(0, __float_as_int(v), 0x121, 0xf, 0xf, false));
+}
+__device__ __forceinline__ float vox_dpp_row_rol1(float v) {
+  return __int_as_float(__builtin_amdgcn_update_dpp(0, __float_as_int(v), 0x12f, 0xf, 0xf, false));
+}
+__device__ __forceinline__ float vox_dpp_swap1(float v) {
+  return __int_as_float(__builtin_amdgcn_update_dpp(0, __float_as_int(v), 0xb1, 0xf, 0xf, false));
+}
+
+template <int Z>
+struct VoxUp2 {
+  static constexpr int ZT = Z / 16, ZP = ZT / 2, NSTORE = ZP * 4;
+  static_assert(ZT % 2 == 0, "z lines of 32 or 64 voxels");
+  static constexpr unsigned OOB = 0x7fffff00u;
+  float part[ZP][4], carry[ZP][4];
+  const float* rp;
+  const float* sp;
+  long s_which;
+  int r_bytes, s_bytes;
+  unsigned rbase, sbase;
+  unsigned cs_r, cs_s;
+  int xs, xe, X, src4;
+  bool rowok;
+
+  __device__ __forceinline__ void init(float* out, int N, int C, int X_, int Y, int n, int seg, int xs_, int xe_, int co0, int gy,
+                                       int lane) {
+    const int v = lane & 15, g = lane >> 4, Zh = Z / 2;
+    const long plane = (long)Y * Zh, rn = (long)C * (X_ / 2) * plane, sn = (long)C * plane;
+    rp = out + (long)n * rn;
+    sp = out + (long)N * rn + ((long)(seg * 2) * N + n) * sn;
+    s_which = (long)N * sn;
+    r_bytes = (int)(rn * 4); s_bytes = (int)(sn * 4);
+    cs_s = (unsigned)(plane * 4); cs_r = (unsigned)((X_ / 2) * plane * 4);
+    rowok = gy < Y;
+    rbase = (unsigned)(co0 + 4 * g) * cs_r + (unsigned)(gy * Zh + v) * 4u;
+    sbase = (unsigned)(co0 + 4 * g) * cs_s + (unsigned)(gy * Zh + v) * 4u;
+    xs = xs_; xe = xe_; X = X_;
+    src4 = ((lane & 48) + 2 * (v & 7) + (v >> 3)) * 4;
+#pragma unroll
+    for (int j = 0; j < ZP; ++j)
+#pragma unroll
+      for (int i = 0; i < 4; ++i) part[j][i] = carry[j][i] = 0.f;
+  }
+  __device__ __forceinline__ __amdgpu_buffer_rsrc_t rsrc_r() const {
+    return __builtin_amdgcn_make_buffer_rsrc((void*)rp, 0, r_bytes, 0x00020000);
+  }
+  __device__ __forceinline__ void reduce_z(const vf32x4 (&r)[ZT], float (&zr)[ZP][4], int lane) const {
+    const int v = lane & 15;
+    const bool odd = v & 1;
+#pragma unroll
+    for (int i = 0; i < 4; ++i) {
+      auto low = [&](int zt) {
+        const float h = r[zt][i];
+        const float lf = vox_dpp_row_ror1(h), lfp = vox_dpp_row_ror1(r[zt > 0 ? zt - 1 : 0][i]);
+        const float rt = vox_dpp_row_rol1(h), rtn = vox_dpp_row_rol1(r[zt < ZT - 1 ? zt + 1 : zt][i]);
+        const float left = v == 0 ? (zt > 0 ? lfp : h) : lf;
+        const float right = v == 15 ? (zt < ZT - 1 ? rtn : h) : rt;
+        const float u = 0.75f * h + 0.25f * (odd ? right : left);
+        return u + vox_dpp_swap1(u);
+      };
+#pragma unroll
+      for (int j = 0; j < ZP; ++j) {
+        const float la = low(2 * j), lb = low(2 * j + 1);
+        zr[j][i] = __int_as_float(__builtin_amdgcn_ds_bpermute(src4, __float_as_int(odd ? lb : la)));
+      }
+    }
+  }
+  __device__ __forceinline__ void plane(const vf32x4 (&r)[ZT], int x, bool active, int lane) {
+    float zr[ZP][4];
+    reduce_z(r, zr, lane);
+    const bool even = !(x & 1), first = x == xs;
+    const __amdgpu_buffer_rsrc_t rs = __builtin_amdgcn_make_buffer_rsrc((void*)(first ? sp : rp), 0, first ? s_bytes : r_bytes, 0x00020000);
+    const bool st = active && even && rowok && (!first || xs > 0);
+    const unsigned base = first ? sbase : rbase + (unsigned)(x / 2 - 1) * cs_s, cs = first ? cs_s : cs_r;
+#pragma unroll
+    for (int j = 0; j < ZP; ++j)
+#pragma unroll
+      for (int i = 0; i < 4; ++i) {
+        const float q = part[j][i] + 0.25f * zr[j][i];
+        __builtin_amdgcn_raw_buffer_store_b32(__float_as_uint(q), rs, st ? base + (unsigned)i * cs + 64u * j : OOB, 0, 0);
+      }
+    if (active) {
+#pragma unroll
+      for (int j = 0; j < ZP; ++j)
+#pragma unroll
+        for (int i = 0; i < 4; ++i) {
+          const float z25 = 0.25f * zr[j][i];
+          const float head = even ? (x == 0 ? z25 : carry[j][i]) : part[j][i];
+          part[j][i] = head + 0.75f * zr[j][i];
+          carry[j][i] = z25;
+        }
+    }
+  }
+  __device__ __forceinline__ void finish() {
+    const bool last = xe >= X;
+    const __amdgpu_buffer_rsrc_t rs = rsrc_r();
+    const __amdgpu_buffer_rsrc_t rs1 = __builtin_amdgcn_make_buffer_rsrc((void*)(sp + s_which), 0, s_bytes, 0x00020000);
+    const unsigned base = rbase + (unsigned)(xe / 2 - 1) * cs_s;
+#pragma unroll
+    for (int j = 0; j < ZP; ++j)
+#pragma unroll
+      for (int i = 0; i < 4; ++i) {
+        const float q = part[j][i] + (last ? carry[j][i] : 0.f);
+        __builtin_amdgcn_raw_buffer_store_b32(__float_as_uint(q), rs, rowok ? base + (unsigned)i * cs_r + 64u * j : OOB, 0, 0);
+        __builtin_amdgcn_raw_buffer_store_b32(__float_as_uint(carry[j][i]), rs1, rowok && !last ? sbase + (unsigned)i * cs_s + 64u * j : OOB, 0, 0);
+      }
+  }
+};
+
+__global__ void __launch_bounds__(256)
+vox_up2_finish_kernel(const float* __restrict__ R, const float* __restrict__ S, float* __restrict__ dx, long NC, int Xh, int Y, int Zh,
+                      int segh, int nseg, long total) {
+  const long idx = (long)blockIdx.x * 256 + threadIdx.x;
+  if (idx >= total) return;
+  const int zq = Zh / 4, Yh = Y / 2;
+  const int k4 = (int)(idx % zq);
+  long t = idx / zq;
+  const int yl = (int)(t % Yh); t /= Yh;
+  const int i = (int)(t % Xh);
+  const long nc = t / Xh;
+  const int seg = i / segh;
+  const bool from_prev = nseg > 1 && seg > 0 && i == seg * segh, from_next = nseg > 1 && seg < nseg - 1 && i == (seg + 1) * segh - 1;
+  const long plane = (long)Y * Zh;
+  const float* r = R + (nc * Xh + i) * plane + k4 * 4;
+  const long s1 = ((long)(seg * 2 - 1) * NC + nc) * plane + k4 * 4;
+  const long s0 = ((long)(seg * 2 + 2) * NC + nc) * plane + k4 * 4;
+  auto row = [&](int y) {
+    y = y < 0 ? 0 : (y > Y - 1 ? Y - 1 : y);
+    float4 a = *(const float4*)(r + (long)y * Zh);
+    if (from_prev) { const float4 b = *(const float4*)(S + s1 + (long)y * Zh); a.x += b.x; a.y += b.y; a.z += b.z; a.w += b.w; }
+    if (from_next) { const float4 b = *(const float4*)(S + s0 + (long)y * Zh); a.x += b.x; a.y += b.y; a.z += b.z; a.w += b.w; }
+    return a;
+  };
+  const float4 a = row(2 * yl - 1), b = row(2 * yl), c = row(2 * yl + 1), d = row(2 * yl + 2);
+  float4 o;
+  o.x = 0.75f * (b.x + c.x) + 0.25f * (a.x + d.x);
+  o.y = 0.75f * (b.y + c.y) + 0.25f * (a.y + d.y);
+  o.z = 0.75f * (b.z + c.z) + 0.25f * (a.z + d.z);
+  o.w = 0.75f * (b.w + c.w) + 0.25f * (a.w + d.w);
+  *(float4*)(dx + ((nc * Xh + i) * Yh + yl) * Zh + k4 * 4) = o;
+}
+
+template <int CK, int Z, int TY, bool GENERIC, bool UP2 = false>
 __global__ void __launch_bounds__(64 * TY)
 vox_bf3_kernel(const VoxArgs a, const float* __restrict__ in, const vu32x4* __restrict__ wp, const float* __restrict__ bias,
                float* __restrict__ out, int act, float slope, int xseg, int accum) {
   static_assert(CK == 8 && TY == 8, "8 reduction channels (one channel group), 8 rows per workgroup");
+  static_assert(!(UP2 && GENERIC), "the upsample-adjoint epilogue has no activation");
   constexpr int CG = 1, TPS = 4, NSTEP = (27 + TPS - 1) / TPS, ZT = Z / 16;
   constexpr int ROWS = TY + 2, COLS = Z + 2;
   constexpr int PLANE = 2 * CG * ROWS * COLS;
@@ -443,7 +587,13 @@
   stage_load(xs - 1); stage_store((xs - 1 + 3) % 3);
   stage_load(xs); stage_store(xs % 3);
   stage_load(xs + 1);
-  vox_dummy_stores<4 * ZT>(rs_out);
+  std::conditional_t<UP2, VoxUp2<Z>, char> up2;
+  if constexpr (UP2) {
+    up2.init(out, a.N, a.Cout, a.X, a.Y, n, seg, xs, xe, co0, y0 + wave, lane);
+    vox_dummy_stores<VoxUp2<Z>::NSTORE>(up2.rsrc_r());
+  } else {
+    vox_dummy_stores<4 * ZT>(rs_out);
+  }
   __syncthreads();
   for (int x = xs; x < xe; ++x) {
     stage_store((x + 1) % 3);
@@ -454,6 +604,7 @@
 #pragma unroll
     for (int s = 0; s < NSTEP; ++s) fb[s] = (fdx[s] < 0 ? P[0] : (fdx[s] == 0 ? P[1] : P[2])) + foff[s];
     const int gy = y0 + wave;
+    vf32x4 up2_r[UP2 ? ZT : 1];
 #pragma unroll
     for (int zt = 0; zt < ZT; ++zt) {
       vf32x4 acc = {0.f, 0.f, 0.f, 0.f};
@@ -464,6 +615,10 @@
         acc = __builtin_amdgcn_mfma_f32_16x16x32_bf16(wl[s], bh, acc, 0, 0, 0);
         acc = __builtin_amdgcn_mfma_f32_16x16x32_bf16(wh[s], bl, acc, 0, 0, 0);
         acc = __builtin_amdgcn_mfma_f32_16x16x32_bf16(wh[s], bh, acc, 0, 0, 0);
+      }
+      if constexpr (UP2) {
+        up2_r[zt] = acc;
+        continue;
       }
       const unsigned ooff = (unsigned)(((long)x * YZ + (long)gy * Z + zt * 16 + v) * 4);
 #pragma unroll
@@ -484,7 +639,12 @@
         msq[i] += r * r;
       }
     }
+    if constexpr (UP2) up2.plane(up2_r, x, true, lane);
     __syncthreads();
+  }
+  if constexpr (UP2) {
+    up2.finish();
+    return;
   }
   if (a.moments) {
 #pragma unroll
@@ -506,11 +666,12 @@
 }
 
 constexpr int VOX_PS_TY = 8;
-template <int Z, int TY, bool CO8, bool GENERIC>
+template <int Z, int TY, bool CO8, bool GENERIC, bool UP2 = false>
 __global__ void __launch_bounds__(64 * TY, 1)
 vox_bf3_ps_kernel(const VoxArgs a, const float* __restrict__ in, const vu32x4* __restrict__ wp, const float* __restrict__ bias,
                   float* __restrict__ out, int act, float slope, int xseg, int accum) {
   static_assert(TY == VOX_PS_TY, "one workgroup of eight waves per CU");
+  static_assert(!(UP2 && (GENERIC || CO8)), "the upsample-adjoint epilogue: no activation, row blocks of 16 produced channels");
   constexpr int CK = 16, CG = 2, PSTEPS = 5, ZT = Z / 16, NF = CO8 ? 2 * PSTEPS : 3 * PSTEPS, NACC = CO8 ? 2 : 3;
   constexpr int ROWS = TY + 2, COLS = Z + 2;
   constexpr int PLANE = 2 * CG * ROWS * COLS;
@@ -609,7 +770,13 @@
 
   stage_load(xs - 1); stage_store((xs - 1) & 1);
   stage_load(xs);
-  vox_dummy_stores<4 * ZT>(rs_out);
+  std::conditional_t<UP2, VoxUp2<Z>, char> up2;
+  if constexpr (UP2) {
+    up2.init(out, a.N, a.Cout, a.X, a.Y, n, seg, xs, xe, co0, y0 + wave, lane);
+    vox_dummy_stores<VoxUp2<Z>::NSTORE>(up2.rsrc_r());
+  } else {
+    vox_dummy_stores<4 * ZT>(rs_out);
+  }
   __syncthreads();
   const int gy = y0 + wave;
   for (int p = xs - 1; p <= xe; ++p) {
@@ -672,8 +839,9 @@
     }
     const int xo = p - 1;
     const bool xok = xo >= xs && xo < xe;
-#pragma unroll
-    for (int zt = 0; zt < ZT; ++zt) {
+    if constexpr (UP2) up2.plane(acc[0], xo, xok, lane);
+#pragma unroll
+    for (int zt = 0; zt < (UP2 ? 0 : ZT); ++zt) {
       const unsigned ooff = (unsigned)(((long)xo * YZ + (long)gy * Z + zt * 16 + v) * 4);
 #pragma unroll
       for (int i = 0; i < 4; ++i) {
@@ -710,6 +878,10 @@
       }
     }
     __syncthreads();
+  }
+  if constexpr (UP2) {
+    up2.finish();
+    return;
   }
   if (a.moments) {
 #pragma unroll
@@ -1634,6 +1806,73 @@
   return vox_conv_dispatch(d, d->Cout, d->Cin, dy, wp, nullptr, dx, MUVO_ACT_NONE, 0.f, st, bf3, nullptr, nullptr);
 }
 
+static int vox_up2_enabled() {
+  static const int v = getenv("MUVO_VOX_UP2") ? atoi(getenv("MUVO_VOX_UP2")) : 1;
+  return v;
+}
+bool vox_dgrad_up2_shape_ok(const muvo_conv_desc* d) {
+  if (!vox_up2_enabled() || !vox_geometry_ok(d) || !vox_bf3_shape_ok(d, 1)) return false;
+  if ((d->Cout != 8 && d->Cout != 16) || (d->Cin != 16 && d->Cin != 32)) return false;
+  return d->in_sz[0] % 2 == 0 && d->in_sz[1] % 2 == 0;
+}
+static int vox_up2_xseg(const VoxArgs& a) {
+  const int xseg = vox_xseg(a, 1, 0);
+  return xseg + (xseg & 1);
+}
+static void vox_up2_sizes(const muvo_conv_desc* d, long* r_floats, long* s_floats, int* xseg_out) {
+  const VoxArgs a = vox_args(d, d->Cout, d->Cin, 8, d->in_sz[2], 0, nullptr);
+  const int xseg = vox_up2_xseg(a), nseg = cdiv(a.X, xseg);
+  const long plane = (long)a.N * d->Cin * a.Y * (d->in_sz[2] / 2);
+  *r_floats = plane * (a.X / 2);
+  *s_floats = nseg > 1 ? plane * 2 * nseg : 0;
+  if (xseg_out) *xseg_out = xseg;
+}
+long vox_dgrad_up2_ws_floats(const muvo_conv_desc* d) {
+  if (!vox_dgrad_up2_shape_ok(d)) return 0;
+  long r, s;
+  vox_up2_sizes(d, &r, &s, nullptr);
+  return r + s;
+}
+int vox_dgrad_up2(const muvo_conv_desc* d, const float* dy, const float* wp, float* dx_low, float* ws, long ws_floats, hipStream_t st) {
+  MUVO_CHECK_ARG(vox_dgrad_up2_shape_ok(d), "vox_dgrad_up2: shape not served (Cin=%d Cout=%d %dx%dx%d)", d->Cin, d->Cout, d->in_sz[0],
+                 d->in_sz[1], d->in_sz[2]);
+  long r_floats, s_floats;
+  int xseg;
+  vox_up2_sizes(d, &r_floats, &s_floats, &xseg);
+  MUVO_CHECK_ARG(ws != nullptr && ws_floats >= r_floats + s_floats, "vox_dgrad_up2: workspace of %ld floats, %ld needed", ws_floats,
+                 r_floats + s_floats);
+  const int Z = d->in_sz[2], C = d->Cin;
+  constexpr int TY = 8;
+  static_assert(VOX_PS_TY == TY, "both forms walk tiles of 8 rows");
+  VoxArgs a = vox_args(d, d->Cout, C, TY, Z, 0, nullptr);
+  const dim3 grid((unsigned)((long)a.N * a.ytiles * cdiv(a.X, xseg)), C / 16);
+  const int rc = vox_with_z(Z, [&](auto z) -> int {
+    constexpr int ZC = decltype(z)::value;
+    if (d->Cout == 8) {
+      constexpr size_t lds = (size_t)3 * 2 * (TY + 2) * (ZC + 2) * 16;
+      static bool lds_raised = false;
+      if (int e = vox_raise_lds(lds_raised, "vox_bf3 (up2)", lds, vox_bf3_kernel<8, ZC, TY, false, true>)) return e;
+      hipLaunchKernelGGL((vox_bf3_kernel<8, ZC, TY, false, true>), grid, dim3(64 * TY), lds, st, a, dy, (const vu32x4*)wp, nullptr, ws,
+                         MUVO_ACT_NONE, 0.f, xseg, 0);
+    } else {
+      constexpr size_t lds = (size_t)2 * 2 * 2 * (TY + 2) * (ZC + 2) * 16;
+      static bool lds_raised = false;
+      if (int e = vox_raise_lds(lds_raised, "vox_bf3_ps (up2)", lds, vox_bf3_ps_kernel<ZC, TY, false, false, true>)) return e;
+      hipLaunchKernelGGL((vox_bf3_ps_kernel<ZC, TY, false, false, true>), grid, dim3(64 * TY), lds, st, a, dy, (const vu32x4*)wp, nullptr, ws,
+                         MUVO_ACT_NONE, 0.f, xseg, 0);
+    }
+    MUVO_CHECK_LAUNCH("vox_bf3 (up2)");
+    return MUVO_OK;
+  });
+  if (rc) return rc;
+  const int Xh = a.X / 2, Zh = Z / 2;
+  const long total = (long)a.N * C * Xh * (a.Y / 2) * (Zh / 4);
+  hipLaunchKernelGGL(vox_up2_finish_kernel, dim3((unsigned)cdiv(total, 256)), dim3(256), 0, st, ws, ws + r_floats, dx_low, (long)a.N * C, Xh,
+                     a.Y, Zh, xseg / 2, cdiv(a.X, xseg), total);
+  MUVO_CHECK_LAUNCH("vox_up2_finish_kernel");
+  return MUVO_OK;
+}
+
 template <int RQB, int CQR, int Z, int TYB>
 static int launch_vox_wgrad(const muvo_conv_desc* d, const float* x, const float* dz, float* dw, float* dbias,
                             hipStream_t st) {
diff --git a/muvo_amd/models/common.py b/muvo_amd/models/common.py
--- a/muvo_amd/models/common.py
+++ b/muvo_amd/models/common.py
@@ -122,9 +122,12 @@
         self.conv_act = nn.Sequential(hnn.Conv3d(in_channels, out_channels, 3, 1, 1), hnn.Placeholder())
         self.adaptive_norm = AdaptiveInstanceNorm3d(latent_n_channels, out_channels)
 
-    def forward(self, x, w, lazy=None, next_conv=None):
-        moments = ops.conv_moments_buffer(x, self.conv_act[0].geom)
-        x = self.conv_act[0](x, act=ops.ACT_LEAKY, slope=0.2, act_bwd_fused=True, moments=moments, lazy=lazy)
+    def forward(self, x, w, lazy=None, next_conv=None, up2_src=None):
+        if up2_src is not None:
+            moments = ops.conv_moments_buffer(ops.upsampled_x2_shape(up2_src.shape), self.conv_act[0].geom, up2_src.device)
+        else:
+            moments = ops.conv_moments_buffer(x, self.conv_act[0].geom)
+        x = self.conv_act[0](x, act=ops.ACT_LEAKY, slope=0.2, act_bwd_fused=True, moments=moments, lazy=lazy, up2_src=up2_src)
         if next_conv is not None and ops.conv_affine_supported(x, next_conv.geom, moments):
             an = self.adaptive_norm
             y, raw, aff = ops.adain_lazy(x, _style(an, w), an.epsilon, ops.ACT_LEAKY, 0.2, moments)
@@ -238,8 +241,9 @@
 
     def forward(self, x, w, head_conv=None):
         if self.upsample:
-            x = ops.upsample3d_x2(x)
-        y, lazy = self.conv1(x, w, next_conv=self.conv2.conv_act[0])
+            y, lazy = self.conv1(None, w, next_conv=self.conv2.conv_act[0], up2_src=x)
+        else:
+            y, lazy = self.conv1(x, w, next_conv=self.conv2.conv_act[0])
         if head_conv is not None:
             return self.conv2.forward_with_head(y, w, head_conv, lazy=lazy)
         return self.conv2(y, w, lazy=lazy)
diff --git a/muvo_amd/nn.py b/muvo_amd/nn.py
--- a/muvo_amd/nn.py
+++ b/muvo_amd/nn.py
@@ -25,8 +25,8 @@
         if bias:
             _uniform_(self.bias, 1.0 / math.sqrt(fan_in))
 
-    def forward(self, x, act=ops.ACT_NONE, slope=0.0, act_bwd_fused=False, moments=None, lazy=None):
-        return ops.conv(x, self.weight, self.bias, self.geom, self._packed, act, slope, act_bwd_fused, moments, lazy)
+    def forward(self, x, act=ops.ACT_NONE, slope=0.0, act_bwd_fused=False, moments=None, lazy=None, up2_src=None):
+        return ops.conv(x, self.weight, self.bias, self.geom, self._packed, act, slope, act_bwd_fused, moments, lazy, up2_src)
 
 
 class Conv2d(_ConvNd):
diff --git a/muvo_amd/ops.py b/muvo_amd/ops.py
--- a/muvo_amd/ops.py
+++ b/muvo_amd/ops.py
@@ -73,6 +73,7 @@
     'muvo_panel_image', 'muvo_panel_logits', 'muvo_panel_labels', 'muvo_panel_fill', 'muvo_panel_bars', 'muvo_panel_scatter',
     'muvo_panel_voxel_top_logits', 'muvo_panel_voxel_top_grid',
     'muvo_icp_state_doubles', 'muvo_icp_ws_doubles', 'muvo_icp_init', 'muvo_icp_iterate',
+    'muvo_conv_dgrad_up2_ws_floats', 'muvo_conv_dgrad_up2',
 ]
 
 
@@ -97,6 +98,7 @@
                 L.muvo_chamfer_loss_ws_doubles.restype = C.c_int64
                 L.muvo_icp_state_doubles.restype = C.c_int64
                 L.muvo_icp_ws_doubles.restype = C.c_int64
+                L.muvo_conv_dgrad_up2_ws_floats.restype = C.c_int64
                 for name in EXPORTS:
                     getattr(L, name)
                 _lib = L
@@ -977,7 +979,14 @@
 
 class ConvFn(torch.autograd.Function):
     @staticmethod
-    def forward(ctx, x, weight, bias, geom, packed, act, slope, act_bwd_fused=False, moments=None, aff_src=None, aff=None):
+    def forward(ctx, x, weight, bias, geom, packed, act, slope, act_bwd_fused=False, moments=None, aff_src=None, aff=None,
+                up2_src=None):
+        ctx.up2 = None
+        if up2_src is not None:
+            assert x is None and aff is None and up2_src.dim() == 5
+            up2_src = up2_src.contiguous()
+            ctx.up2 = up2_src.shape
+            x = _upsample3d_x2_fwd(up2_src)
         ctx.aff = aff
         if aff is not None:
             x = aff_src
@@ -991,6 +1000,7 @@
         ctx.weight, ctx.bias = weight, bias
         ctx.stem = bool(plan.supports('muvo_stem_conv_supported') and get_conv_mode() != CONV_F32 and bias is None
                         and act == ACT_NONE and moments is None and aff is None and not x_ph and not ctx.needs_input_grad[0]
+                        and up2_src is None
                         and hf is None and weight.is_contiguous())
         if ctx.stem:
             return ConvFn._stem_forward(ctx, plan, x, weight)
@@ -1061,7 +1071,10 @@
 
     @staticmethod
     def backward(ctx, dy):
-        return ConvFn._backward(ctx, dy, None)
+        g = ConvFn._backward(ctx, dy, None)
+        if ctx.up2 is not None:
+            return (None,) + g[1:] + (g[0],)
+        return g + (None,)
 
     @staticmethod
     def _backward(ctx, dy, head):
@@ -1070,7 +1083,8 @@
         if getattr(ctx, 'stem', False):
             ConvFn._stem_backward(ctx, plan, x, dy)
             return (None,) * 11
-        need_dx, need_dw = ctx.needs_input_grad[0], ctx.weight.requires_grad
+        up2 = getattr(ctx, 'up2', None) is not None
+        need_dx, need_dw = ctx.needs_input_grad[11 if up2 else 0], ctx.weight.requires_grad
         fused_dy = plan.dy_planes and need_dx and need_dw
         dy_ws = _DyWorkspace(wgrad_stream(x.device) if need_dw else None, x.device)
         dz, planes = ConvFn._resolve_dy(ctx, plan, x, y, dy, head, fused_dy, dy_ws)
@@ -1131,11 +1145,21 @@
     @staticmethod
     def _data_grad(ctx, plan, x, dz, planes, fused_dy, dy_ws):
         wp = _packed_weight(plan, ctx.packed, ctx.weight, 1)
-        dx = torch.empty(x.shape, device=dz.device, dtype=torch.float32)
         e1 = _bracket(plan, 'dgrad') if KERNEL_TIMING is not None else None
         if planes is None and (plan.ws_dgrad_dy > 0 or plan.ws_wgrad_dy > 0):
             planes = dy_ws.get(plan.dy_planes_floats)
-        _ck(lib().muvo_conv_dgrad(C.byref(plan.desc), _f(dz), _f(wp), _f(dx), _p(planes), 1 if fused_dy else 0, _st()))
+        L, d = lib(), C.byref(plan.desc)
+        up2 = getattr(ctx, 'up2', None)
+        nws = L.muvo_conv_dgrad_up2_ws_floats(d) if (up2 is not None and not fused_dy) else 0
+        if nws > 0:
+            dx = torch.empty(up2, device=dz.device, dtype=torch.float32)
+            ws = torch.empty(nws, device=dz.device, dtype=torch.float32)
+            _ck(L.muvo_conv_dgrad_up2(d, _f(dz), _f(wp), _f(dx), _f(ws), _i64(nws), _st()))
+        else:
+            dx = torch.empty(x.shape, device=dz.device, dtype=torch.float32)
+            _ck(L.muvo_conv_dgrad(d, _f(dz), _f(wp), _f(dx), _p(planes), 1 if fused_dy else 0, _st()))
+            if up2 is not None:
+                dx = _upsample3d_x2_bwd(dx, up2)
         if e1 is not None:
             e1.record()
         return dx, planes
@@ -1166,7 +1190,10 @@
                 e1.record()
 
 
-def conv(x, weight, bias, geom, packed, act=ACT_NONE, slope=0.0, act_bwd_fused=False, moments=None, lazy=None):
+def conv(x, weight, bias, geom, packed, act=ACT_NONE, slope=0.0, act_bwd_fused=False, moments=None, lazy=None, up2_src=None):
+    if up2_src is not None:
+        assert lazy is None
+        return ConvFn.apply(None, weight, bias, geom, packed, act, slope, act_bwd_fused, moments, None, None, up2_src)
     if lazy is not None:
         return ConvFn.apply(x, weight, bias, geom, packed, act, slope, act_bwd_fused, moments, lazy[0], lazy[1])
     y = ConvFn.apply(x, weight, bias, geom, packed, act, slope, act_bwd_fused, moments)
@@ -1188,14 +1215,15 @@
 CONV_MOMENTS = os.environ.get('MUVO_CONV_MOMENTS', '1') != '0'
 
 
-def conv_moments_buffer(x, geom):
+def conv_moments_buffer(x, geom, device=None):
     if not CONV_MOMENTS or not geom.plan_for(x).supports('muvo_conv_forward_moments_supported'):
         return None
-    n = x.shape[0]
+    n = getattr(x, 'shape', x)[0]
+    device = x.device if device is None else device
     cache = geom.__dict__.setdefault('_moments', {})
-    buf = cache.get((n, x.device))
+    buf = cache.get((n, device))
     if buf is None:
-        buf = cache[(n, x.device)] = torch.zeros(n, geom.cout, 2, device=x.device, dtype=torch.float64)
+        buf = cache[(n, device)] = torch.zeros(n, geom.cout, 2, device=device, dtype=torch.float64)
         _MOMENT_BUFS.append(weakref.ref(buf))
     return buf
 
@@ -1792,23 +1820,35 @@
     return GlobalAvgPoolFn.apply(x)
 
 
+def upsampled_x2_shape(shape):
+    n, c, d, h, w = shape
+    return (n, c, 2 * d, 2 * h, 2 * w)
+
+
+def _upsample3d_x2_fwd(x):
+    n, c, d, h, w = x.shape
+    y = torch.empty(upsampled_x2_shape(x.shape), device=x.device, dtype=torch.float32)
+    _ck(lib().muvo_upsample3d_x2_fwd(_f(x), _f(y), _i64(n * c), d, h, w, _st()))
+    return y
+
+
+def _upsample3d_x2_bwd(dy, shape):
+    n, c, d, h, w = shape
+    dx = torch.empty(shape, device=dy.device, dtype=torch.float32)
+    _ck(lib().muvo_upsample3d_x2_bwd(_f(dy), _f(dx), _i64(n * c), d, h, w, _st()))
+    return dx
+
+
 class Upsample3dFn(torch.autograd.Function):
     @staticmethod
     def forward(ctx, x):
         x = x.contiguous()
-        n, c, d, h, w = x.shape
-        y = torch.empty(n, c, 2 * d, 2 * h, 2 * w, device=x.device, dtype=torch.float32)
-        _ck(lib().muvo_upsample3d_x2_fwd(_f(x), _f(y), _i64(n * c), d, h, w, _st()))
         ctx.shape = x.shape
-        return y
+        return _upsample3d_x2_fwd(x)
 
     @staticmethod
     def backward(ctx, dy):
-        dy = dy.contiguous()
-        n, c, d, h, w = ctx.shape
-        dx = torch.empty(ctx.shape, device=dy.device, dtype=torch.float32)
-        _ck(lib().muvo_upsample3d_x2_bwd(_f(dy), _f(dx), _i64(n * c), d, h, w, _st()))
-        return dx
+        return _upsample3d_x2_bwd(dy.contiguous(), ctx.shape)
 
 
 def upsample3d_x2(x):
```

New measurement: 25.83, median of 6. Within noise of the previous version (+0.8%).
